# xyfJASON/ctrlora

Measured on AMD Instinct MI355X. Metric: 512x512 LoRA-finetune images/sec, higher is better.
Workload: dtype bf16; 1 GPU; ctrlora_finetune_sd15_rank128.yaml, canny-style latent hint, 512x512 (latent 64x64), per-GPU batch 8, bf16 storage / fp32 accumulate, synthetic latents + random-init weights, LoRA+zero-conv+norm trainables, fused AdamW; global_batch=8, parallelism=dp1, lora_rank=128, launch=hipGraph replay, gemm_launch_table_entries=215

## Files before the change

ctrlora_amd/build.py:

```python
from __future__ import annotations

import os
import subprocess
import sys
from concurrent.futures import ThreadPoolExecutor

HERE = os.path.dirname(os.path.abspath(__file__))
ROOT = os.path.dirname(HERE)
CSRC = os.path.join(HERE, "csrc")
OBJ = os.path.join(ROOT, "build", "obj")
LIB = os.path.join(HERE, "libctrlora_hip.so")
SOURCES = ["gemm.hip", "gemm_xs.hip", "gemm_w4.hip", "wgrad.hip", "norm.hip", "norm_coop.hip", "elementwise.hip", "attention_fwd.hip", "attention_bwd.hip", "attention_tr.hip", "attention_fwd40.hip", "attention_causal.hip", "capi.hip"]
FLAGS = ["--offload-arch=gfx950", "-O3", "-std=c++17", "-fPIC", "-Wno-unused-value"]


def _headers_mtime() -> float:
    hs = [os.path.join(CSRC, f) for f in os.listdir(CSRC) if f.endswith(".h")]
    hs.append(os.path.join(ROOT, "include", "ctrlora_hip.h"))
    return max(os.path.getmtime(h) for h in hs)


def _compile(src: str, force: bool) -> str:
    obj = os.path.join(OBJ, src.replace(".hip", ".o"))
    spath = os.path.join(CSRC, src)
    if (not force and os.path.exists(obj)
            and os.path.getmtime(obj) >= max(os.path.getmtime(spath), _headers_mtime())):
        return obj
    cmd = ["hipcc", *FLAGS, "-c", spath, "-o", obj]
    r = subprocess.run(cmd, capture_output=True, text=True)
    if r.returncode != 0:
        raise RuntimeError(f"hipcc failed for {src}:\n{r.stderr[-4000:]}")
    return obj


def build(force: bool = False, verbose: bool = True) -> str:
    os.makedirs(OBJ, exist_ok=True)
    with ThreadPoolExecutor(max_workers=6) as ex:
        objs = list(ex.map(lambda s: _compile(s, force), SOURCES))
    if force or not os.path.exists(LIB) or os.path.getmtime(LIB) < max(os.path.getmtime(o) for o in objs):
        r = subprocess.run(["hipcc", "--offload-arch=gfx950", "-shared", "-fPIC", *objs, "-o", LIB],
                           capture_output=True, text=True)
        if r.returncode != 0:
            raise RuntimeError(f"link failed:\n{r.stderr[-4000:]}")
        if verbose:
            print(f"[ctrlora_amd.build] linked {LIB}")
    elif verbose:
        print(f"[ctrlora_amd.build] up to date: {LIB}")
    return LIB


if __name__ == "__main__":
    build(force="--force" in sys.argv)
```

ctrlora_amd/csrc/attention.h:

```cpp
#pragma once
#include "common.h"

namespace cl {

struct AttnFwdArgs {
  const void* Q; long ldq;
  const void* K; long ldk;
  const void* Vt; int nkv_pad;
  void* O; long ldo;
  float* LSE; int lse_stride;
  int B, H, N, Nkv, DH;
  float scale;
  int q_prescaled;
};

struct AttnIpArgs {
  const void* K2; long ldk2;
  const void* V2; long ldv2;
  int Nip;
  float ip_scale;
};

struct AttnBwdArgs {
  const void* Q; long ldq; const void* K; long ldk; const void* V; long ldv;
  const void* O; long ldo; const void* dO; long lddo;
  const void* Qt; const void* dOt; int n_pad;
  const void* Kt; int nkv_pad;
  const float* LSE; float* Delta; int lse_stride;
  void* dQ; long lddq; void* dK; long lddk; void* dV; long lddv;
  int B, H, N, Nkv, DH;
  float scale;
  int q_prescaled;
  void* row_ws;
};

int attn_fwd(const AttnFwdArgs& a, int dtype, hipStream_t st);
int attn_bwd(const AttnBwdArgs& a, int dtype, hipStream_t st);
int attn_fwd_tr(const AttnFwdArgs& a, const void* V, long ldv, hipStream_t st);
int attn_fwd_ip(const AttnFwdArgs& a, const AttnIpArgs& ip, int dtype, hipStream_t st);
int attn_fwd_tr_ip(const AttnFwdArgs& a, const void* V, long ldv, const AttnIpArgs& ip, hipStream_t st);
int attn_bwd_tr(const AttnBwdArgs& a, hipStream_t st);
extern int g_attn_fuse_delta;
extern int g_attn_variant_dkv4;
extern int g_attn_variant;
bool attn_fwd40_applies(const AttnFwdArgs& a);
int attn_fwd40(const AttnFwdArgs& a, const void* V, long ldv, hipStream_t st);
int attn_delta(const AttnBwdArgs& a, hipStream_t st);
int attn_causal_fwd(int dtype, const void* Q, long ldq, const void* K, long ldk, const void* V, long ldv, void* O, long ldo, int B, int H,
                    int N, int dh, float scale, hipStream_t st);

enum { ATTN_FAM_TR = 1, ATTN_FAM_TR_IP = 2, ATTN_FAM_HYB = 3, ATTN_FAM_FWD40 = 4, ATTN_FAM_FOLD = 5, ATTN_FAM_TRANSPOSED = 6,
       ATTN_FAM_CAUSAL = 7 };
enum { ATTN_BIT_TAIL = 1, ATTN_BIT_TQ = 2, ATTN_BIT_TK = 4, ATTN_BIT_PRIO = 8 };
struct AttnLaunchRec {
  int kind;
  int family;
  int dtype, dh;
  int fwd_frags, dq_frags, dkv_frags;
  int bits;
  int lookahead, remap;
  int delta_launch, dkv_ran;
  int grid_fwd, grid_dq, grid_dkv;
  int tile;
};
extern AttnLaunchRec g_attn_last;
inline void attn_rec_begin() { g_attn_last = AttnLaunchRec{}; }
inline void attn_rec(int kind, int family, int dtype, int dh) {
  g_attn_last.kind = kind; g_attn_last.family = family; g_attn_last.dtype = dtype; g_attn_last.dh = dh; g_attn_last.tile = 64;
}

}
```

ctrlora_amd/csrc/attention_tr.hip:

```cpp
#include <type_traits>
#include "attn_common.h"
#include "attn_tr_util.h"

#ifndef ATTN_BWD_ABL
#define ATTN_BWD_ABL 0
#endif
#if ATTN_BWD_ABL == 2
#define BWD_MMA(a, b, c) asm volatile("" ::"v"(a), "v"(b))
#else
#define BWD_MMA(a, b, c) Mma<bf16_t>::run(a, b, c)
#endif
#if ATTN_BWD_ABL == 3
#define BWD_RD128 abl_rd128
#define BWD_TRF abl_trf
#else
#define BWD_RD128 lds_read_b128_off
#define BWD_TRF tr_frag_off
#endif
#if ATTN_BWD_ABL == 5
#define BWD_PACK(p) abl_pack(p)
#else
#define BWD_PACK(p) PFrag<bf16_t>::make(p)
#endif
#if ATTN_BWD_ABL == 1
#define BWD_EXP2(x) (x)
#else
#define BWD_EXP2(x) __builtin_amdgcn_exp2f(x)
#endif

namespace cl {
#if ATTN_BWD_ABL == 3
template <int OFF> __device__ __forceinline__ u32x4_t abl_rd128(uint32_t a) { u32x4_t v = {0x3c003c00u, 0x3c003c00u, 0x3c003c00u, 0x3c003c00u}; asm volatile("" : "+v"(v) : "v"(a)); return v; }
template <int ROWB, int STEP, int OFF> __device__ __forceinline__ u32x4_t abl_trf(uint32_t a) { u32x4_t v = {0x3c003c00u, 0x3c003c00u, 0x3c003c00u, 0x3c003c00u}; asm volatile("" : "+v"(v) : "v"(a)); return v; }
#endif
#if ATTN_BWD_ABL == 5
__device__ __forceinline__ u32x4_t abl_pack(const f32x4_t* p) {
  return u32x4_t{__float_as_uint(p[0][0]), __float_as_uint(p[0][2]), __float_as_uint(p[1][0]), __float_as_uint(p[1][2])};
}
#endif

namespace {

template <int DH> struct TileDma {
  static constexpr int TI = Geo<DH>::TI, NJ = (TI + 3) / 4, CPR = Geo<DH>::CPR, CPRP = Geo<DH>::CPRP;
  int r[NJ], cc16[NJ];
  bool real[NJ];
  __device__ __forceinline__ void init(int wave, int lane) {
#pragma unroll
    for (int j = 0; j < NJ; ++j) {
      const int c = (wave + 4 * j) * 64 + lane;
      r[j] = c / CPRP;
      const int col = c - r[j] * CPRP;
      real[j] = col < CPR;
      cc16[j] = (real[j] ? col : 0) * 16;
    }
  }
  __device__ __forceinline__ void offsets(long ld_bytes, int (&off)[NJ]) const {
#pragma unroll
    for (int j = 0; j < NJ; ++j) off[j] = r[j] * (int)ld_bytes + cc16[j];
  }
  __device__ __forceinline__ void issue_with_pad(const char* base, long ld_bytes, const int (&off)[NJ], int row0, char* dst,
                                                 int wave, const char* pad, int pad_stride) const {
    const char* tb = base + (long)row0 * ld_bytes;
    const char* pb = pad + (long)row0 * pad_stride;
#pragma unroll
    for (int j = 0; j < NJ; ++j)
      if (wave + 4 * j < TI) {
        const char* src = real[j] ? tb + off[j] : pb + r[j] * pad_stride;
        glds16(src, dst + (wave + 4 * j) * 1024);
      }
  }
  __device__ __forceinline__ void issue(const char* base, long ld_bytes, const int (&off)[NJ], int row0, int nrows,
                                        char* dst, int wave) const {
    const char* tb = base + (long)row0 * ld_bytes;
    if (row0 + 64 <= nrows) {
#pragma unroll
      for (int j = 0; j < NJ; ++j)
        if (wave + 4 * j < TI && real[j]) glds16(tb + off[j], dst + (wave + 4 * j) * 1024);
    } else {
#pragma unroll
      for (int j = 0; j < NJ; ++j)
        if (wave + 4 * j < TI && real[j]) {
          const int rr = min(row0 + r[j], nrows - 1);
          glds16(base + (long)rr * ld_bytes + cc16[j], dst + (wave + 4 * j) * 1024);
        }
    }
  }
};

__device__ __forceinline__ void split3_bf16(float x, uint32_t& w0, uint32_t& w1) {
  const uint32_t hi = pack2bf(x, 0.f) & 0xffffu;
  const float r1 = x - __uint_as_float(hi << 16);
  const uint32_t mid = pack2bf(r1, 0.f) & 0xffffu;
  const float r2 = r1 - __uint_as_float(mid << 16);
  const uint32_t lo = pack2bf(r2, 0.f) & 0xffffu;
  w0 = hi | (mid << 16); w1 = lo;
}
__device__ __forceinline__ u32x4_t ones3_chunk() { return u32x4_t{0x3F803F80u, 0x00003F80u, 0u, 0u}; }
template <int DH> __device__ __forceinline__ void init_pads_ones3(char* tiles, int ntile, int tid, int nthreads) {
  using G = Geo<DH>;
  for (int i = tid; i < ntile * 64; i += nthreads)
    *reinterpret_cast<uint4*>(tiles + (long)i * G::ROWB + G::CPR * 16) = make_uint4(0x3F803F80u, 0x00003F80u, 0u, 0u);
}

}

template <int DH, int QW, bool TAIL>
__global__ __launch_bounds__(256, 2) void attn_fwd_tr_kernel(AttnFwdArgs p, const void* __restrict__ V, long ldv) {
  using G = Geo<DH>;
  constexpr int CPR = G::CPR, KSTEPS = G::KSTEPS, DN = G::DN, ROWB = G::ROWB, TILE = G::TILE;
  constexpr int STAGE = 2 * TILE;
  extern __shared__ __attribute__((aligned(16))) char smem[];

  const int tid = threadIdx.x, lane = tid & 63;
  const int wave = __builtin_amdgcn_readfirstlane(tid >> 6);
  const int g = lane >> 4, lq = lane & 15;
  const int b = blockIdx.z, h = blockIdx.y;
  const int q0 = blockIdx.x * (64 * QW) + wave * (16 * QW);
  const float sl2 = p.q_prescaled ? 1.0f : p.scale * 1.4426950408889634f;

  u32x4_t qf[QW][KSTEPS];
#pragma unroll
  for (int f = 0; f < QW; ++f) {
    const int row = min(q0 + f * 16 + lq, p.N - 1);
    const char* qp = (const char*)p.Q + (((long)b * p.N + row) * p.ldq + (long)h * DH) * 2;
#pragma unroll
    for (int ks = 0; ks < KSTEPS; ++ks) {
      const int c = 4 * ks + g;
      qf[f][ks] = (c < CPR) ? *reinterpret_cast<const u32x4_t*>(qp + c * 16) : u32x4_t{0u, 0u, 0u, 0u};
    }
  }
  const char* kbase = (const char*)p.K + ((long)b * p.Nkv * p.ldk + (long)h * DH) * 2;
  const char* vbase = (const char*)V + ((long)b * p.Nkv * ldv + (long)h * DH) * 2;

  f32x4_t ot[DN][QW];
#pragma unroll
  for (int i = 0; i < DN; ++i)
#pragma unroll
    for (int f = 0; f < QW; ++f) ot[i][f] = f32x4_t{0.f, 0.f, 0.f, 0.f};
  float m_run[QW], l_run[QW];
#pragma unroll
  for (int f = 0; f < QW; ++f) { m_run[f] = -1e30f; l_run[f] = 0.f; }

  const uint32_t lds0 = (uint32_t)(uintptr_t)smem;
  uint32_t krow[KSTEPS];
#pragma unroll
  for (int ks = 0; ks < KSTEPS; ++ks) krow[ks] = lq * ROWB + min(4 * ks + g, CPR - 1) * 16;
  const uint32_t troff = (4 * g + ((lane >> 2) & 3)) * ROWB + (lane & 3) * 8;
  const int ntiles = (p.Nkv + 63) / 64;
  TileDma<DH> dma; dma.init(wave, lane);
  int koff[TileDma<DH>::NJ], voff[TileDma<DH>::NJ];
  dma.offsets(p.ldk * 2, koff); dma.offsets(ldv * 2, voff);
  init_pads<DH>(smem, 4, 0u, 0u, tid, 256);
  dma.issue(kbase, p.ldk * 2, koff, 0, p.Nkv, smem, wave);
  dma.issue(vbase, ldv * 2, voff, 0, p.Nkv, smem + TILE, wave);
  for (int t = 0; t < ntiles; ++t) {
    const int buf = t & 1;
    asm volatile("s_waitcnt vmcnt(0)" ::: "memory");
    __syncthreads();
    if (t + 1 < ntiles) {
      dma.issue(kbase, p.ldk * 2, koff, (t + 1) * 64, p.Nkv, smem + (buf ^ 1) * STAGE, wave);
      dma.issue(vbase, ldv * 2, voff, (t + 1) * 64, p.Nkv, smem + (buf ^ 1) * STAGE + TILE, wave);
    }
    const uint32_t kt = lds0 + buf * STAGE, vt = kt + TILE;

    f32x4_t st[4][QW];
    uint32_t kr[KSTEPS];
#pragma unroll
    for (int ks = 0; ks < KSTEPS; ++ks) kr[ks] = kt + krow[ks];
    static_for<0, 4>([&](auto KF_) {
      constexpr int kf = decltype(KF_)::value;
      u32x4_t ka[KSTEPS];
#pragma unroll
      for (int ks = 0; ks < KSTEPS; ++ks) ka[ks] = lds_read_b128_off<kf * 16 * ROWB>(kr[ks]);
      lds_wait();
#pragma unroll
      for (int f = 0; f < QW; ++f) {
        st[kf][f] = f32x4_t{0.f, 0.f, 0.f, 0.f};
#pragma unroll
        for (int ks = 0; ks < KSTEPS; ++ks) Mma<bf16_t>::run(ka[ks], qf[f][ks], st[kf][f]);
      }
    });
    const int kv0 = t * 64;
    {
#pragma unroll
      for (int f = 0; f < QW; ++f) {
        float mx = -INFINITY;
#pragma unroll
        for (int kf = 0; kf < 4; ++kf)
#pragma unroll
          for (int r = 0; r < 4; ++r) {
            if constexpr (TAIL) { if (kv0 + kf * 16 + 4 * g + r >= p.Nkv) st[kf][f][r] = -INFINITY; }
            mx = fmaxf(mx, st[kf][f][r]);
          }
        mx = fmaxf(mx, __shfl_xor(mx, 16, 64));
        mx = fmaxf(mx, __shfl_xor(mx, 32, 64));
        const float m_new = fmaxf(m_run[f], mx * sl2);
        const float alpha = __builtin_amdgcn_exp2f(m_run[f] - m_new);
        m_run[f] = m_new;
        float ls = 0.f;
#pragma unroll
        for (int kf = 0; kf < 4; ++kf)
#pragma unroll
          for (int r = 0; r < 4; ++r) {
            const float e = __builtin_amdgcn_exp2f(__builtin_fmaf(st[kf][f][r], sl2, -m_new));
            st[kf][f][r] = e;
            ls += e;
          }
        l_run[f] = l_run[f] * alpha + ls;
#pragma unroll
        for (int i = 0; i < DN; ++i) ot[i][f] *= alpha;
      }
    }
    u32x4_t pb[2][QW];
#pragma unroll
    for (int s = 0; s < 2; ++s)
#pragma unroll
      for (int f = 0; f < QW; ++f) {
        f32x4_t tmp[2] = {st[2 * s][f], st[2 * s + 1][f]};
        pb[s][f] = PFrag<bf16_t>::make(tmp);
      }
    const uint32_t tb = vt + troff;
    static_for<0, DN>([&](auto I_) {
      constexpr int i = decltype(I_)::value;
      u32x4_t va[2];
      va[0] = tr_frag_off<ROWB, 0, i * 32>(tb);
      va[1] = tr_frag_off<ROWB, 1, i * 32>(tb);
      lds_wait();
#pragma unroll
      for (int s = 0; s < 2; ++s)
#pragma unroll
        for (int f = 0; f < QW; ++f) Mma<bf16_t>::run(va[s], pb[s][f], ot[i][f]);
    });
  }

#pragma unroll
  for (int f = 0; f < QW; ++f) {
    float l = l_run[f];
    l += __shfl_xor(l, 16, 64);
    l += __shfl_xor(l, 32, 64);
    const float inv = 1.0f / l;
    const int row = q0 + f * 16 + lq;
    if (row < p.N) {
      bf16_t* op = reinterpret_cast<bf16_t*>(p.O) + ((long)b * p.N + row) * p.ldo + (long)h * DH;
#pragma unroll
      for (int i = 0; i < DN; ++i) {
        const int d0 = i * 16 + 4 * g;
        if (d0 < DH) {
          float v[4] = {ot[i][f][0] * inv, ot[i][f][1] * inv, ot[i][f][2] * inv, ot[i][f][3] * inv};
          store4(op + d0, v);
        }
      }
      if (p.LSE && g == 0) p.LSE[((long)b * p.H + h) * p.lse_stride + row] = m_run[f] + __builtin_amdgcn_logf(l);
    }
  }
}

template <int DH, int QW>
__global__ __launch_bounds__(256, 2) void attn_fwd_tr_ip_kernel(AttnFwdArgs p, const void* __restrict__ V, long ldv,
                                                                AttnIpArgs ip) {
  using G = Geo<DH>;
  constexpr int CPR = G::CPR, KSTEPS = G::KSTEPS, DN = G::DN, ROWB = G::ROWB, TILE = G::TILE;
  constexpr int STAGE = 2 * TILE;
  extern __shared__ __attribute__((aligned(16))) char smem[];

  const int tid = threadIdx.x, lane = tid & 63;
  const int wave = __builtin_amdgcn_readfirstlane(tid >> 6);
  const int g = lane >> 4, lq = lane & 15;
  const int b = blockIdx.z, h = blockIdx.y;
  const int q0 = blockIdx.x * (64 * QW) + wave * (16 * QW);
  const float sl2 = p.q_prescaled ? 1.0f : p.scale * 1.4426950408889634f;

  u32x4_t qf[QW][KSTEPS];
#pragma unroll
  for (int f = 0; f < QW; ++f) {
    const int row = min(q0 + f * 16 + lq, p.N - 1);
    const char* qp = (const char*)p.Q + (((long)b * p.N + row) * p.ldq + (long)h * DH) * 2;
#pragma unroll
    for (int ks = 0; ks < KSTEPS; ++ks) {
      const int c = 4 * ks + g;
      qf[f][ks] = (c < CPR) ? *reinterpret_cast<const u32x4_t*>(qp + c * 16) : u32x4_t{0u, 0u, 0u, 0u};
    }
  }
  const char* kbase = (const char*)p.K + ((long)b * p.Nkv * p.ldk + (long)h * DH) * 2;
  const char* vbase = (const char*)V + ((long)b * p.Nkv * ldv + (long)h * DH) * 2;

  f32x4_t ot[DN][QW];
#pragma unroll
  for (int i = 0; i < DN; ++i)
#pragma unroll
    for (int f = 0; f < QW; ++f) ot[i][f] = f32x4_t{0.f, 0.f, 0.f, 0.f};
  float m_run[QW], l_run[QW];
#pragma unroll
  for (int f = 0; f < QW; ++f) { m_run[f] = -1e30f; l_run[f] = 0.f; }

  const uint32_t lds0 = (uint32_t)(uintptr_t)smem;
  uint32_t krow[KSTEPS];
#pragma unroll
  for (int ks = 0; ks < KSTEPS; ++ks) krow[ks] = lq * ROWB + min(4 * ks + g, CPR - 1) * 16;
  const uint32_t troff = (4 * g + ((lane >> 2) & 3)) * ROWB + (lane & 3) * 8;
  auto qk = [&](uint32_t kt, f32x4_t (&st)[4][QW]) {
    static_for<0, 4>([&](auto KF_) {
      constexpr int kf = decltype(KF_)::value;
      u32x4_t ka[KSTEPS];
#pragma unroll
      for (int ks = 0; ks < KSTEPS; ++ks) ka[ks] = lds_read_b128_off<kf * 16 * ROWB>(kt + krow[ks]);
      lds_wait();
#pragma unroll
      for (int f = 0; f < QW; ++f) {
        st[kf][f] = f32x4_t{0.f, 0.f, 0.f, 0.f};
#pragma unroll
        for (int ks = 0; ks < KSTEPS; ++ks) Mma<bf16_t>::run(ka[ks], qf[f][ks], st[kf][f]);
      }
    });
  };
  auto pv = [&](uint32_t vt, f32x4_t (&st)[4][QW]) {
    u32x4_t pb[2][QW];
#pragma unroll
    for (int s = 0; s < 2; ++s)
#pragma unroll
      for (int f = 0; f < QW; ++f) {
        f32x4_t tmp[2] = {st[2 * s][f], st[2 * s + 1][f]};
        pb[s][f] = PFrag<bf16_t>::make(tmp);
      }
    const uint32_t tb = vt + troff;
    static_for<0, DN>([&](auto I_) {
      constexpr int i = decltype(I_)::value;
      u32x4_t va[2];
      va[0] = tr_frag_off<ROWB, 0, i * 32>(tb);
      va[1] = tr_frag_off<ROWB, 1, i * 32>(tb);
      lds_wait();
#pragma unroll
      for (int s = 0; s < 2; ++s)
#pragma unroll
        for (int f = 0; f < QW; ++f) Mma<bf16_t>::run(va[s], pb[s][f], ot[i][f]);
    });
  };

  const int ntiles = (p.Nkv + 63) / 64;
  TileDma<DH> dma; dma.init(wave, lane);
  int koff[TileDma<DH>::NJ], voff[TileDma<DH>::NJ];
  dma.offsets(p.ldk * 2, koff); dma.offsets(ldv * 2, voff);
  init_pads<DH>(smem, 4, 0u, 0u, tid, 256);
  dma.issue(kbase, p.ldk * 2, koff, 0, p.Nkv, smem, wave);
  dma.issue(vbase, ldv * 2, voff, 0, p.Nkv, smem + TILE, wave);
  for (int t = 0; t < ntiles; ++t) {
    const int buf = t & 1;
    asm volatile("s_waitcnt vmcnt(0)" ::: "memory");
    __syncthreads();
    if (t + 1 < ntiles) {
      dma.issue(kbase, p.ldk * 2, koff, (t + 1) * 64, p.Nkv, smem + (buf ^ 1) * STAGE, wave);
      dma.issue(vbase, ldv * 2, voff, (t + 1) * 64, p.Nkv, smem + (buf ^ 1) * STAGE + TILE, wave);
    } else {
      const char* k2 = (const char*)ip.K2 + ((long)b * ip.Nip * ip.ldk2 + (long)h * DH) * 2;
      const char* v2 = (const char*)ip.V2 + ((long)b * ip.Nip * ip.ldv2 + (long)h * DH) * 2;
      dma.offsets(ip.ldk2 * 2, koff); dma.offsets(ip.ldv2 * 2, voff);
      dma.issue(k2, ip.ldk2 * 2, koff, 0, ip.Nip, smem + (buf ^ 1) * STAGE, wave);
      dma.issue(v2, ip.ldv2 * 2, voff, 0, ip.Nip, smem + (buf ^ 1) * STAGE + TILE, wave);
    }
    const uint32_t kt = lds0 + buf * STAGE, vt = kt + TILE;
    f32x4_t st[4][QW];
    qk(kt, st);
    const int kv0 = t * 64;
#pragma unroll
    for (int f = 0; f < QW; ++f) {
      float mx = -INFINITY;
#pragma unroll
      for (int kf = 0; kf < 4; ++kf)
#pragma unroll
        for (int r = 0; r < 4; ++r) {
          if (kv0 + kf * 16 + 4 * g + r >= p.Nkv) st[kf][f][r] = -INFINITY;
          mx = fmaxf(mx, st[kf][f][r]);
        }
      mx = fmaxf(mx, __shfl_xor(mx, 16, 64));
      mx = fmaxf(mx, __shfl_xor(mx, 32, 64));
      const float m_new = fmaxf(m_run[f], mx * sl2);
      const float alpha = __builtin_amdgcn_exp2f(m_run[f] - m_new);
      m_run[f] = m_new;
      float ls = 0.f;
#pragma unroll
      for (int kf = 0; kf < 4; ++kf)
#pragma unroll
        for (int r = 0; r < 4; ++r) {
          const float e = __builtin_amdgcn_exp2f(__builtin_fmaf(st[kf][f][r], sl2, -m_new));
          st[kf][f][r] = e;
          ls += e;
        }
      l_run[f] = l_run[f] * alpha + ls;
#pragma unroll
      for (int i = 0; i < DN; ++i) ot[i][f] *= alpha;
    }
    pv(vt, st);
  }

#pragma unroll
  for (int f = 0; f < QW; ++f) {
    float l = l_run[f];
    l += __shfl_xor(l, 16, 64);
    l += __shfl_xor(l, 32, 64);
    const float inv = 1.0f / l;
#pragma unroll
    for (int i = 0; i < DN; ++i) ot[i][f] *= inv;
  }
  asm volatile("s_waitcnt vmcnt(0)" ::: "memory");
  __syncthreads();
  {
    const uint32_t kt = lds0 + (ntiles & 1) * STAGE, vt = kt + TILE;
    f32x4_t st[4][QW];
    qk(kt, st);
#pragma unroll
    for (int f = 0; f < QW; ++f) {
      float mx = -INFINITY;
#pragma unroll
      for (int kf = 0; kf < 4; ++kf)
#pragma unroll
        for (int r = 0; r < 4; ++r) {
          if (kf * 16 + 4 * g + r >= ip.Nip) st[kf][f][r] = -INFINITY;
          mx = fmaxf(mx, st[kf][f][r]);
        }
      mx = fmaxf(mx, __shfl_xor(mx, 16, 64));
      mx = fmaxf(mx, __shfl_xor(mx, 32, 64));
      const float m2 = mx * sl2;
      float ls = 0.f;
#pragma unroll
      for (int kf = 0; kf < 4; ++kf)
#pragma unroll
        for (int r = 0; r < 4; ++r) {
          const float e = __builtin_amdgcn_exp2f(__builtin_fmaf(st[kf][f][r], sl2, -m2));
          st[kf][f][r] = e;
          ls += e;
        }
      ls += __shfl_xor(ls, 16, 64);
      ls += __shfl_xor(ls, 32, 64);
      const float c = ip.ip_scale / ls;
#pragma unroll
      for (int kf = 0; kf < 4; ++kf) st[kf][f] *= c;
    }
    pv(vt, st);
  }

#pragma unroll
  for (int f = 0; f < QW; ++f) {
    const int row = q0 + f * 16 + lq;
    if (row < p.N) {
      bf16_t* op = reinterpret_cast<bf16_t*>(p.O) + ((long)b * p.N + row) * p.ldo + (long)h * DH;
#pragma unroll
      for (int i = 0; i < DN; ++i) {
        const int d0 = i * 16 + 4 * g;
        if (d0 < DH) {
          float v[4] = {ot[i][f][0], ot[i][f][1], ot[i][f][2], ot[i][f][3]};
          store4(op + d0, v);
        }
      }
    }
  }
}



template <int DH, int LA = 3>
__global__ __launch_bounds__(512, 2) void attn_fwd_hyb_kernel(AttnFwdArgs p, const void* __restrict__ V, long ldv,
                                                              int nqb, int remap) {
  using G = Geo<DH>;
  constexpr int CPR = G::CPR, DN = G::DN, ROWB = G::ROWB, TILE = G::TILE;
  constexpr int STAGE = 2 * TILE, QW = 2;
  constexpr int NK = (DH + 15) / 16;
  constexpr bool ONES = (DH % 16) != 0;
  constexpr bool PADONES = ONES && G::CPRP > G::CPR;
  static_assert(!ONES || PADONES, "spare V^T rows come from the padded LDS pitch");
  static_assert(2 * NK <= G::CPRP, "K fragment reads stay inside the LDS row");
  constexpr int LROW = DH % 16;
  constexpr float RESCALE_THR = 6.0f;
  extern __shared__ __attribute__((aligned(16))) char smem[];

  const int tid = threadIdx.x, lane = tid & 63;
  const int wave = __builtin_amdgcn_readfirstlane(tid >> 6);
  const int grp = wave >> 2;
  const int g = lane >> 4, lq = lane & 15, l31 = lane & 31, hi = lane >> 5;
  int bh, qb;
  {
    const int id = blockIdx.x;
    if (remap) { const int xcd = id & 7, slot = id >> 3; bh = xcd + 8 * (slot / nqb); qb = slot - (slot / nqb) * nqb; }
    else { bh = id / nqb; qb = id - bh * nqb; }
  }
  const int b = bh / p.H, h = bh - b * p.H;
  const int q0 = qb * 256 + wave * 32;
  const float sl2 = p.q_prescaled ? 1.0f : p.scale * 1.4426950408889634f;

  for (int i = tid; i < (16 * ROWB + 64) / 4; i += 512) reinterpret_cast<uint32_t*>(smem + 3 * STAGE)[i] = 0u;
  init_pads<DH>(smem, 6, 0u, 0x3F803F80u, tid, 512);

  u32x4_t qh[NK];
  {
    const char* qp = (const char*)p.Q + (((long)b * p.N + q0 + l31) * p.ldq + (long)h * DH) * 2;
#pragma unroll
    for (int j = 0; j < NK; ++j) {
      const int c = 2 * j + hi;
      qh[j] = (c < CPR) ? *reinterpret_cast<const u32x4_t*>(qp + c * 16) : u32x4_t{0u, 0u, 0u, 0u};
    }
  }
  const char* kbase = (const char*)p.K + ((long)b * p.Nkv * p.ldk + (long)h * DH) * 2;
  const char* vbase = (const char*)V + ((long)b * p.Nkv * ldv + (long)h * DH) * 2;

  f32x4_t ot[DN][QW];
#pragma unroll
  for (int i = 0; i < DN; ++i)
#pragma unroll
    for (int f = 0; f < QW; ++f) ot[i][f] = f32x4_t{0.f, 0.f, 0.f, 0.f};
  float m_run = -1e30f, l_run = 0.f;
  f32x16_t st[2];
  u32x4_t pb[2][QW];

  constexpr int CPRP = G::CPRP, NJ = (CPRP + 7) / 8;
  int koff[NJ], voff[NJ];
  bool real[NJ];
#pragma unroll
  for (int j = 0; j < NJ; ++j) {
    const int c = (wave + 8 * j) * 64 + lane, r = c / CPRP, col = c - r * CPRP;
    real[j] = col < CPR;
    const int cc = (real[j] ? col : 0) * 16;
    koff[j] = r * (int)(p.ldk * 2) + cc;
    voff[j] = r * (int)(ldv * 2) + cc;
  }
  auto issue = [&](int t, int stage) {
    const char* kb = kbase + (long)t * 64 * p.ldk * 2;
    const char* vb = vbase + (long)t * 64 * ldv * 2;
    char* dst = smem + stage * STAGE;
#pragma unroll
    for (int j = 0; j < NJ; ++j)
      if (wave + 8 * j < CPRP && real[j]) {
        glds16(kb + koff[j], dst + (wave + 8 * j) * 1024);
        glds16(vb + voff[j], dst + TILE + (wave + 8 * j) * 1024);
      }
  };

  const uint32_t lds0 = (uint32_t)(uintptr_t)smem;
  const int kr = (l31 & 19) | ((l31 & 4) << 1) | ((l31 & 8) >> 1);
  const uint32_t krow = kr * ROWB + hi * 16;
  const uint32_t troff = (4 * g + ((lane >> 2) & 3)) * ROWB + (lane & 3) * 8;
  const int nt = p.Nkv / 64;

  auto phaseM = [&](auto PREVc, uint32_t kt, uint32_t vt) {
    constexpr bool PREV = decltype(PREVc)::value;
    constexpr int NV = PREV ? DN : 0, NG = NV + 2;
    u32x4_t va[LA][2], ka[LA][NK];
    auto cnt_of = [](int j) constexpr { return j < NV ? 4 : NK; };
    auto read_group = [&](auto Jc) {
      constexpr int J = decltype(Jc)::value;
      if constexpr (J < NV) {
        va[J % LA][0] = tr_frag<ROWB, 0>(vt + troff + J * 32);
        va[J % LA][1] = tr_frag<ROWB, 1>(vt + troff + J * 32);
      } else if constexpr (J < NG) {
        constexpr int s = J - NV;
        static_for<0, NK>([&](auto Kc) {
          constexpr int j = decltype(Kc)::value;
          ka[s % LA][j] = lds_read_b128_off<s * 32 * ROWB + j * 32>(kt + krow);
        });
      }
    };
    static_for<0, LA - 1>([&](auto Jc) { read_group(Jc); });
    __builtin_amdgcn_s_setprio(1);
    static_for<0, NG>([&](auto Jc) {
      constexpr int J = decltype(Jc)::value;
      read_group(std::integral_constant<int, J + LA - 1>{});
      constexpr int pending = [&]() constexpr { int n = 0; for (int k = J + 1; k < J + LA && k < NG; ++k) n += cnt_of(k); return n; }();
      lgkm_wait<(pending > 15 ? 15 : pending)>();
      if constexpr (J < NV) {
        pin(va[J % LA][0]); pin(va[J % LA][1]);
#pragma unroll
        for (int f = 0; f < QW; ++f) Mma<bf16_t>::run(va[J % LA][0], pb[0][f], ot[J][f]);
#pragma unroll
        for (int f = 0; f < QW; ++f) Mma<bf16_t>::run(va[J % LA][1], pb[1][f], ot[J][f]);
      } else {
        constexpr int s = J - NV;
#pragma unroll
        for (int j = 0; j < NK; ++j) pin(ka[s % LA][j]);
        f32x16_t acc = {0.f, 0.f, 0.f, 0.f, 0.f, 0.f, 0.f, 0.f, 0.f, 0.f, 0.f, 0.f, 0.f, 0.f, 0.f, 0.f};
#pragma unroll
        for (int j = 0; j < NK; ++j)
          acc = __builtin_amdgcn_mfma_f32_32x32x16_bf16(__builtin_bit_cast(bf16x8_t, ka[s % LA][j]),
                                                        __builtin_bit_cast(bf16x8_t, qh[j]), acc, 0, 0, 0);
        st[s] = acc;
      }
      __builtin_amdgcn_sched_barrier(0);
    });
    __builtin_amdgcn_s_setprio(0);
  };

  auto phaseV = [&]() {
    float mx = st[0][0];
#pragma unroll
    for (int s = 0; s < 2; ++s)
#pragma unroll
      for (int r = 0; r < 16; ++r) mx = fmaxf(mx, st[s][r]);
    const bool need = mx * sl2 > m_run + RESCALE_THR;
    if (__any(need)) {
      mx = fmaxf(mx, __shfl_xor(mx, 32, 64));
      const float m_new = fmaxf(m_run, mx * sl2);
      const float alpha = __builtin_amdgcn_exp2f(m_run - m_new);
      m_run = m_new;
      l_run *= alpha;
#pragma unroll
      for (int f = 0; f < QW; ++f) {
        const float af = __shfl(alpha, 16 * f + lq, 64);
#pragma unroll
        for (int i = 0; i < DN; ++i) ot[i][f] *= af;
      }
    }
    float ls = 0.f;
#pragma unroll
    for (int s = 0; s < 2; ++s) {
      uint32_t pk[8];
#pragma unroll
      for (int k = 0; k < 8; ++k) {
        const f32x2_t x = f32x2_t{st[s][2 * k], st[s][2 * k + 1]} * sl2 - m_run;
        const float e0 = __builtin_amdgcn_exp2f(x.x), e1 = __builtin_amdgcn_exp2f(x.y);
        if constexpr (!ONES) ls += e0 + e1;
        pk[k] = pack2bf(e0, e1);
      }
      const auto s0 = __builtin_amdgcn_permlane16_swap(pk[0], pk[2], false, false);
      const auto s1 = __builtin_amdgcn_permlane16_swap(pk[1], pk[3], false, false);
      const auto s2 = __builtin_amdgcn_permlane16_swap(pk[4], pk[6], false, false);
      const auto s3 = __builtin_amdgcn_permlane16_swap(pk[5], pk[7], false, false);
      pb[s][0] = u32x4_t{s0[0], s1[0], s2[0], s3[0]};
      pb[s][1] = u32x4_t{s0[1], s1[1], s2[1], s3[1]};
    }
    if constexpr (!ONES) l_run += ls;
  };

  issue(0, 0);
  issue(1, 1);
  asm volatile("s_waitcnt vmcnt(0)" ::: "memory");
  __syncthreads();
  int sk = 0;
  if (grp == 1) __builtin_amdgcn_s_setprio(1);
  auto pv_tail = [&](uint32_t vt) {
    u32x4_t va[2];
#pragma unroll
    for (int i = 0; i < DN; ++i) {
      va[0] = tr_frag<ROWB, 0>(vt + troff + i * 32); va[1] = tr_frag<ROWB, 1>(vt + troff + i * 32);
      lds_wait();
#pragma unroll
      for (int s = 0; s < 2; ++s)
#pragma unroll
        for (int f = 0; f < QW; ++f) Mma<bf16_t>::run(va[s], pb[s][f], ot[i][f]);
    }
  };
  if (grp == 0) {
    int sp = 2;
    for (int u = 0; u < nt; ++u) {
      const int sn = (sk == 2) ? 0 : sk + 1;
      if (u >= 1 && u + 1 < nt) issue(u + 1, sn);
      if (u == 0) phaseM(std::false_type{}, lds0 + sk * STAGE, 0u);
      else phaseM(std::true_type{}, lds0 + sk * STAGE, lds0 + sp * STAGE + TILE);
      __builtin_amdgcn_s_barrier();
      phaseV();
      asm volatile("s_waitcnt vmcnt(0)" ::: "memory");
      __builtin_amdgcn_s_barrier();
      sp = sk; sk = sn;
    }
    pv_tail(lds0 + sp * STAGE + TILE);
    __builtin_amdgcn_s_barrier();
  } else {
    int sp = 2;
    __builtin_amdgcn_s_barrier();
    for (int u = 0; u < nt; ++u) {
      const int sn = (sk == 2) ? 0 : sk + 1, sn2 = (sn == 2) ? 0 : sn + 1;
      if (u == 0) phaseM(std::false_type{}, lds0 + sk * STAGE, 0u);
      else phaseM(std::true_type{}, lds0 + sk * STAGE, lds0 + sp * STAGE + TILE);
      __builtin_amdgcn_s_setprio(1);
      asm volatile("s_waitcnt vmcnt(0)" ::: "memory");
      __builtin_amdgcn_s_barrier();
      if (u + 2 < nt) issue(u + 2, sn2);
      phaseV();
      __builtin_amdgcn_s_barrier();
      sp = sk; sk = sn;
    }
    pv_tail(lds0 + sp * STAGE + TILE);
  }

  float l_full = l_run;
  if constexpr (!ONES) l_full += __shfl_xor(l_full, 32, 64);
#pragma unroll
  for (int f = 0; f < QW; ++f) {
    float l;
    if constexpr (ONES) l = __shfl(ot[DN - 1][f][LROW & 3], lq + 16 * (LROW >> 2), 64);
    else l = __shfl(l_full, 16 * f + lq, 64);
    const float m = __shfl(m_run, 16 * f + lq, 64);
    const float inv = 1.0f / l;
    const int row = q0 + f * 16 + lq;
    bf16_t* op = reinterpret_cast<bf16_t*>(p.O) + ((long)b * p.N + row) * p.ldo + (long)h * DH;
#pragma unroll
    for (int i = 0; i < DN; ++i) {
      const int d0 = i * 16 + 4 * g;
      if (d0 < DH) {
        float v[4] = {ot[i][f][0] * inv, ot[i][f][1] * inv, ot[i][f][2] * inv, ot[i][f][3] * inv};
        store4(op + d0, v);
      }
    }
    if (p.LSE && g == 0) p.LSE[((long)b * p.H + h) * p.lse_stride + row] = m + __builtin_amdgcn_logf(l);
  }
}

template <int DH, int KF, bool TAIL, bool PRIO = false, bool FOLD = false>
__global__ __launch_bounds__(256, (DH <= 80 && KF <= 2 ? 2 : 1)) void attn_bwd_dkv_tr_kernel(AttnBwdArgs p) {
  using G = Geo<DH>;
  constexpr int CPR = G::CPR, KSTEPS = G::KSTEPS, DN = G::DN, ROWB = G::ROWB, TILE = G::TILE, TI = G::TI;
  static_assert(!FOLD || (DH == 40 && !TAIL), "the fold uses the pad chunk of the 96-byte pitch, whole tiles only");
  constexpr int CIN = FOLD ? G::CPRP : CPR;
  constexpr bool PIPE = FOLD;
  constexpr int STAGE = 2 * TILE + 512;
  extern __shared__ __attribute__((aligned(16))) char smem[];

  const int tid = threadIdx.x, lane = tid & 63;
  const int wave = __builtin_amdgcn_readfirstlane(tid >> 6);
  const int g = lane >> 4, lq = lane & 15;
  const int b = blockIdx.z, h = blockIdx.y;
  const int kv_w = blockIdx.x * (64 * KF) + wave * (16 * KF);
  const float sl2 = p.q_prescaled ? 1.0f : p.scale * 1.4426950408889634f;
  const float kscale = p.q_prescaled ? 0.6931471805599453f : p.scale;

  u32x4_t kb[KF][KSTEPS], vb[KF][KSTEPS];
#pragma unroll
  for (int kf = 0; kf < KF; ++kf) {
    const int kr = min(kv_w + kf * 16 + lq, p.Nkv - 1);
    const char* kp = (const char*)p.K + (((long)b * p.Nkv + kr) * p.ldk + (long)h * DH) * 2;
    const char* vp = (const char*)p.V + (((long)b * p.Nkv + kr) * p.ldv + (long)h * DH) * 2;
#pragma unroll
    for (int ks = 0; ks < KSTEPS; ++ks) {
      const int c = 4 * ks + g;
      kb[kf][ks] = (c < CPR) ? *reinterpret_cast<const u32x4_t*>(kp + c * 16) : u32x4_t{0u, 0u, 0u, 0u};
      vb[kf][ks] = (c < CPR) ? *reinterpret_cast<const u32x4_t*>(vp + c * 16) : u32x4_t{0u, 0u, 0u, 0u};
      if constexpr (FOLD) {
        if (c == CPR) { kb[kf][ks] = ones3_chunk(); vb[kf][ks] = ones3_chunk(); }
      }
    }
  }
  const char* qbase = (const char*)p.Q + ((long)b * p.N * p.ldq + (long)h * DH) * 2;
  const char* dobase = (const char*)p.dO + ((long)b * p.N * p.lddo + (long)h * DH) * 2;
  const float* lse = p.LSE + ((long)b * p.H + h) * p.lse_stride;
  const float* dlt = p.Delta + ((long)b * p.H + h) * p.lse_stride;

  f32x4_t dvt[KF][DN], dkt[KF][DN];
#pragma unroll
  for (int kf = 0; kf < KF; ++kf)
#pragma unroll
    for (int i = 0; i < DN; ++i) { dvt[kf][i] = f32x4_t{0.f, 0.f, 0.f, 0.f}; dkt[kf][i] = f32x4_t{0.f, 0.f, 0.f, 0.f}; }

  TileDma<DH> dma; dma.init(wave, lane);
  int qoff[TileDma<DH>::NJ], dooff[TileDma<DH>::NJ];
  dma.offsets(p.ldq * 2, qoff); dma.offsets(p.lddo * 2, dooff);
  const char* rowpad = FOLD ? (const char*)p.row_ws + ((long)b * p.H + h) * p.lse_stride * 32 : nullptr;
  auto issue = [&](int t, int buf) {
    char* base = smem + buf * STAGE;
    if constexpr (FOLD) {
      dma.issue_with_pad(qbase, p.ldq * 2, qoff, t * 64, base, wave, rowpad, 32);
      dma.issue_with_pad(dobase, p.lddo * 2, dooff, t * 64, base + TILE, wave, rowpad + 16, 32);
      return;
    }
    dma.issue(qbase, p.ldq * 2, qoff, t * 64, p.N, base, wave);
    dma.issue(dobase, p.lddo * 2, dooff, t * 64, p.N, base + TILE, wave);
    if (wave == (TI & 3) && lane < 32) {
      const float* src = lane < 16 ? lse + t * 64 + lane * 4 : dlt + t * 64 + (lane - 16) * 4;
      glds16(src, base + 2 * TILE);
    }
  };

  const uint32_t lds0 = (uint32_t)(uintptr_t)smem;
  uint32_t rrow[KSTEPS];
#pragma unroll
  for (int ks = 0; ks < KSTEPS; ++ks) rrow[ks] = lq * ROWB + min(4 * ks + g, CIN - 1) * 16;
  const uint32_t troff = (4 * g + ((lane >> 2) & 3)) * ROWB + (lane & 3) * 8;
  const int ntiles = (p.N + 63) / 64;
  if constexpr (!FOLD) {
    init_pads<DH>(smem, 2, 0u, 0u, tid, 256);
    init_pads<DH>(smem + STAGE, 2, 0u, 0u, tid, 256);
  }
  const int dma_per_tile = 2 * ((TI - wave + 3) / 4);
  issue(0, 0);
  if constexpr (PIPE) { if (ntiles > 1) issue(1, 1); }
  int buf = 0;
  for (int t = 0; t < ntiles; ++t) {
#if ATTN_BWD_ABL == 4
    if constexpr (!PIPE) { asm volatile("s_waitcnt vmcnt(0)" ::: "memory"); __syncthreads(); }
#else
    if constexpr (PIPE) {
      if (t + 1 >= ntiles) asm volatile("s_waitcnt vmcnt(0)" ::: "memory");
      else if (dma_per_tile == 4) asm volatile("s_waitcnt vmcnt(4)" ::: "memory");
      else asm volatile("s_waitcnt vmcnt(2)" ::: "memory");
    } else {
      asm volatile("s_waitcnt vmcnt(0)" ::: "memory");
    }
    __syncthreads();
#endif
    const uint32_t aQ = lds0 + buf * STAGE, adO = aQ + TILE, aL = adO + TILE;
    const int q0 = t * 64;
    uint32_t rb[KSTEPS];
#pragma unroll
    for (int ks = 0; ks < KSTEPS; ++ks) rb[ks] = aQ + rrow[ks];
    const uint32_t tb = aQ + troff;
    u32x4_t qa[2][KSTEPS], da[2][KSTEPS];
    if constexpr (PIPE) {
#pragma unroll
      for (int ks = 0; ks < KSTEPS; ++ks) { qa[0][ks] = BWD_RD128<0>(rb[ks]); da[0][ks] = BWD_RD128<TILE>(rb[ks]); }
    }
    if constexpr (PIPE) {
      if (t + 2 < ntiles) issue(t + 2, buf == 0 ? 2 : buf - 1);
    } else {
      if (t + 1 < ntiles) issue(t + 1, buf ^ 1);
    }

    f32x4_t ps[KF][4], ds[KF][4];
    u32x4_t oa[2][2], qt[2][2];
    static_for<0, 4>([&](auto QF_) {
      constexpr int qf = decltype(QF_)::value;
      constexpr int cur = PIPE ? (qf & 1) : 0;
      u32x4_t l4 = {0u, 0u, 0u, 0u}, d4 = {0u, 0u, 0u, 0u};
      if constexpr (PIPE) {
        if constexpr (qf + 1 < 4) {
#pragma unroll
          for (int ks = 0; ks < KSTEPS; ++ks) {
            qa[cur ^ 1][ks] = BWD_RD128<(qf + 1) * 16 * ROWB>(rb[ks]);
            da[cur ^ 1][ks] = BWD_RD128<TILE + (qf + 1) * 16 * ROWB>(rb[ks]);
          }
          lgkm_wait<2 * KSTEPS>();
        } else {
          oa[0][0] = BWD_TRF<ROWB, 0, TILE>(tb); oa[0][1] = BWD_TRF<ROWB, 1, TILE>(tb);
          qt[0][0] = BWD_TRF<ROWB, 0, 0>(tb); qt[0][1] = BWD_TRF<ROWB, 1, 0>(tb);
          lgkm_wait<8>();
        }
      } else {
#pragma unroll
        for (int ks = 0; ks < KSTEPS; ++ks) {
          qa[0][ks] = BWD_RD128<qf * 16 * ROWB>(rb[ks]);
          da[0][ks] = BWD_RD128<TILE + qf * 16 * ROWB>(rb[ks]);
        }
        if constexpr (!FOLD) {
          l4 = lds_read_b128(aL + (qf * 16 + 4 * g) * 4);
          d4 = lds_read_b128(aL + 256 + (qf * 16 + 4 * g) * 4);
        }
        lds_wait();
      }
      const float lv[4] = {__uint_as_float(l4.x), __uint_as_float(l4.y), __uint_as_float(l4.z), __uint_as_float(l4.w)};
      const float dv[4] = {__uint_as_float(d4.x), __uint_as_float(d4.y), __uint_as_float(d4.z), __uint_as_float(d4.w)};
      const int qrow = q0 + qf * 16 + 4 * g;
#pragma unroll
      for (int kf = 0; kf < KF; ++kf) {
        f32x4_t sc = {0.f, 0.f, 0.f, 0.f}, dp = {0.f, 0.f, 0.f, 0.f};
        if constexpr (PRIO) __builtin_amdgcn_s_setprio(1);
#pragma unroll
        for (int ks = 0; ks < KSTEPS; ++ks) { BWD_MMA(qa[cur][ks], kb[kf][ks], sc); BWD_MMA(da[cur][ks], vb[kf][ks], dp); }
        if constexpr (PRIO) __builtin_amdgcn_s_setprio(0);
#pragma unroll
        for (int h2 = 0; h2 < 2; ++h2) {
          f32x2_t pr, dsv;
          if constexpr (FOLD) {
            pr = f32x2_t{BWD_EXP2(sc[2 * h2]), BWD_EXP2(sc[2 * h2 + 1])};
            dsv = pr * f32x2_t{dp[2 * h2], dp[2 * h2 + 1]};
          } else {
            const f32x2_t s2 = {sc[2 * h2], sc[2 * h2 + 1]}, l2 = {lv[2 * h2], lv[2 * h2 + 1]};
            const f32x2_t x = s2 * sl2 - l2;
            pr = f32x2_t{__builtin_amdgcn_exp2f(x.x), __builtin_amdgcn_exp2f(x.y)};
            const f32x2_t dd = f32x2_t{dp[2 * h2], dp[2 * h2 + 1]} - f32x2_t{dv[2 * h2], dv[2 * h2 + 1]};
            dsv = pr * dd;
          }
          if constexpr (TAIL) {
            if (qrow + 2 * h2 >= p.N) { pr.x = 0.f; dsv.x = 0.f; }
            if (qrow + 2 * h2 + 1 >= p.N) { pr.y = 0.f; dsv.y = 0.f; }
          }
          ps[kf][qf][2 * h2] = pr.x; ps[kf][qf][2 * h2 + 1] = pr.y;
          ds[kf][qf][2 * h2] = dsv.x; ds[kf][qf][2 * h2 + 1] = dsv.y;
        }
      }
    });
    u32x4_t pb[KF][2], sb[KF][2];
#pragma unroll
    for (int kf = 0; kf < KF; ++kf)
#pragma unroll
      for (int s2 = 0; s2 < 2; ++s2) { pb[kf][s2] = BWD_PACK(&ps[kf][2 * s2]); sb[kf][s2] = BWD_PACK(&ds[kf][2 * s2]); }
    static_for<0, DN>([&](auto I_) {
      constexpr int i = decltype(I_)::value;
      constexpr int cur = PIPE ? (i & 1) : 0;
      if constexpr (PIPE) {
        if constexpr (i + 1 < DN) {
          oa[cur ^ 1][0] = BWD_TRF<ROWB, 0, TILE + (i + 1) * 32>(tb); oa[cur ^ 1][1] = BWD_TRF<ROWB, 1, TILE + (i + 1) * 32>(tb);
          lgkm_wait<4>();
          qt[cur ^ 1][0] = BWD_TRF<ROWB, 0, (i + 1) * 32>(tb); qt[cur ^ 1][1] = BWD_TRF<ROWB, 1, (i + 1) * 32>(tb);
        } else {
          lgkm_wait<0>();
        }
      } else {
        oa[0][0] = BWD_TRF<ROWB, 0, TILE + i * 32>(tb); oa[0][1] = BWD_TRF<ROWB, 1, TILE + i * 32>(tb);
        qt[0][0] = BWD_TRF<ROWB, 0, i * 32>(tb); qt[0][1] = BWD_TRF<ROWB, 1, i * 32>(tb);
        lds_wait();
      }
      if constexpr (PRIO) __builtin_amdgcn_s_setprio(1);
#pragma unroll
      for (int kf = 0; kf < KF; ++kf)
#pragma unroll
        for (int s2 = 0; s2 < 2; ++s2) { BWD_MMA(oa[cur][s2], pb[kf][s2], dvt[kf][i]); BWD_MMA(qt[cur][s2], sb[kf][s2], dkt[kf][i]); }
      if constexpr (PRIO) __builtin_amdgcn_s_setprio(0);
    });
    if constexpr (PIPE) buf = buf == 2 ? 0 : buf + 1;
    else buf ^= 1;
  }
#pragma unroll
  for (int kf = 0; kf < KF; ++kf) {
    const int kr = kv_w + kf * 16 + lq;
    if (kr < p.Nkv) {
      bf16_t* dkp = reinterpret_cast<bf16_t*>(p.dK) + ((long)b * p.Nkv + kr) * p.lddk + (long)h * DH;
      bf16_t* dvp = reinterpret_cast<bf16_t*>(p.dV) + ((long)b * p.Nkv + kr) * p.lddv + (long)h * DH;
#pragma unroll
      for (int i = 0; i < DN; ++i) {
        const int d0 = i * 16 + 4 * g;
        if (d0 < DH) {
          float a[4] = {dkt[kf][i][0] * kscale, dkt[kf][i][1] * kscale, dkt[kf][i][2] * kscale, dkt[kf][i][3] * kscale};
          float c[4] = {dvt[kf][i][0], dvt[kf][i][1], dvt[kf][i][2], dvt[kf][i][3]};
          store4(dkp + d0, a);
          store4(dvp + d0, c);
        }
      }
    }
  }
}

template <int DH, int QF, bool TAIL, bool DELTA = false, bool PRIO = false, bool FOLD = false>
__global__ __launch_bounds__(256, 2) void attn_bwd_dq_tr_kernel(AttnBwdArgs p) {
  using G = Geo<DH>;
  constexpr int CPR = G::CPR, KSTEPS = G::KSTEPS, DN = G::DN, ROWB = G::ROWB, TILE = G::TILE;
  static_assert(!FOLD || (DH == 40 && !TAIL && DELTA), "fold: d_head 40, whole key tiles, fused delta");
  constexpr int CIN = FOLD ? G::CPRP : CPR;
  constexpr bool PIPE = FOLD;
  constexpr int STAGE = 2 * TILE;
  extern __shared__ __attribute__((aligned(16))) char smem[];

  const int tid = threadIdx.x, lane = tid & 63;
  const int wave = __builtin_amdgcn_readfirstlane(tid >> 6);
  const int g = lane >> 4, lq = lane & 15;
  const int b = blockIdx.z, h = blockIdx.y;
  const int q_w = blockIdx.x * (64 * QF) + wave * (16 * QF);
  const float sl2 = p.q_prescaled ? 1.0f : p.scale * 1.4426950408889634f;

  u32x4_t qb[QF][KSTEPS], ob[QF][KSTEPS];
  float lse_q[QF], dlt_q[QF];
#pragma unroll
  for (int f = 0; f < QF; ++f) {
    const int qr = min(q_w + f * 16 + lq, p.N - 1);
    const char* qp = (const char*)p.Q + (((long)b * p.N + qr) * p.ldq + (long)h * DH) * 2;
    const char* op = (const char*)p.dO + (((long)b * p.N + qr) * p.lddo + (long)h * DH) * 2;
#pragma unroll
    for (int ks = 0; ks < KSTEPS; ++ks) {
      const int c = 4 * ks + g;
      qb[f][ks] = (c < CPR) ? *reinterpret_cast<const u32x4_t*>(qp + c * 16) : u32x4_t{0u, 0u, 0u, 0u};
      ob[f][ks] = (c < CPR) ? *reinterpret_cast<const u32x4_t*>(op + c * 16) : u32x4_t{0u, 0u, 0u, 0u};
    }
    lse_q[f] = p.LSE[((long)b * p.H + h) * p.lse_stride + qr];
    if constexpr (DELTA) {
      const char* orow = (const char*)p.O + (((long)b * p.N + qr) * p.ldo + (long)h * DH) * 2;
      float acc = 0.f;
#pragma unroll
      for (int ks = 0; ks < KSTEPS; ++ks) {
        const int c = 4 * ks + g;
        if (c < CPR) {
          const u32x4_t ov = *reinterpret_cast<const u32x4_t*>(orow + c * 16);
          const u32x4_t dv = ob[f][ks];
#pragma unroll
          for (int j = 0; j < 4; ++j) {
            acc += __uint_as_float(ov[j] << 16) * __uint_as_float(dv[j] << 16);
            acc += __uint_as_float(ov[j] & 0xffff0000u) * __uint_as_float(dv[j] & 0xffff0000u);
          }
        }
      }
      acc += __shfl_xor(acc, 16, 64);
      acc += __shfl_xor(acc, 32, 64);
      dlt_q[f] = acc;
      if (g == 0 && q_w + f * 16 + lq < p.N) p.Delta[((long)b * p.H + h) * p.lse_stride + qr] = acc;
    } else {
      dlt_q[f] = p.Delta[((long)b * p.H + h) * p.lse_stride + qr];
    }
    if constexpr (FOLD) {
      uint32_t l0, l1, d0, d1;
      split3_bf16(-lse_q[f], l0, l1);
      split3_bf16(-dlt_q[f], d0, d1);
      if (g == 1) {
        qb[f][1] = u32x4_t{l0, l1, 0u, 0u};
        ob[f][1] = u32x4_t{d0, d1, 0u, 0u};
      }
      if (g == 0 && q_w + f * 16 + lq < p.N) {
        uint4* rp = reinterpret_cast<uint4*>((char*)p.row_ws + (((long)b * p.H + h) * p.lse_stride + qr) * 32);
        rp[0] = make_uint4(l0, l1, 0u, 0u);
        rp[1] = make_uint4(d0, d1, 0u, 0u);
      }
    }
  }
  const char* kbase = (const char*)p.K + ((long)b * p.Nkv * p.ldk + (long)h * DH) * 2;
  const char* vbase = (const char*)p.V + ((long)b * p.Nkv * p.ldv + (long)h * DH) * 2;

  f32x4_t dqt[QF][DN];
#pragma unroll
  for (int f = 0; f < QF; ++f)
#pragma unroll
    for (int i = 0; i < DN; ++i) dqt[f][i] = f32x4_t{0.f, 0.f, 0.f, 0.f};

  const uint32_t lds0 = (uint32_t)(uintptr_t)smem;
  uint32_t rrow[KSTEPS];
#pragma unroll
  for (int ks = 0; ks < KSTEPS; ++ks) rrow[ks] = lq * ROWB + min(4 * ks + g, CIN - 1) * 16;
  const uint32_t troff = (4 * g + ((lane >> 2) & 3)) * ROWB + (lane & 3) * 8;
  const int ntiles = (p.Nkv + 63) / 64;
  TileDma<DH> dma; dma.init(wave, lane);
  int koff[TileDma<DH>::NJ], voff[TileDma<DH>::NJ];
  dma.offsets(p.ldk * 2, koff); dma.offsets(p.ldv * 2, voff);
  if constexpr (FOLD) init_pads_ones3<DH>(smem, 6, tid, 256);
  else init_pads<DH>(smem, 4, 0u, 0u, tid, 256);
  constexpr int TI = G::TI;
  const int dma_per_tile = 2 * ((TI - wave + 3) / 4);
  auto issue_kv = [&](int t, int st_) {
    dma.issue(kbase, p.ldk * 2, koff, t * 64, p.Nkv, smem + st_ * STAGE, wave);
    dma.issue(vbase, p.ldv * 2, voff, t * 64, p.Nkv, smem + st_ * STAGE + TILE, wave);
  };
  issue_kv(0, 0);
  if constexpr (PIPE) { if (ntiles > 1) issue_kv(1, 1); }
  int buf = 0;
  for (int t = 0; t < ntiles; ++t) {
#if ATTN_BWD_ABL == 4
    if constexpr (!PIPE) { asm volatile("s_waitcnt vmcnt(0)" ::: "memory"); __syncthreads(); }
#else
    if constexpr (PIPE) {
      if (t + 1 >= ntiles) asm volatile("s_waitcnt vmcnt(0)" ::: "memory");
      else if (dma_per_tile == 4) asm volatile("s_waitcnt vmcnt(4)" ::: "memory");
      else asm volatile("s_waitcnt vmcnt(2)" ::: "memory");
    } else {
      asm volatile("s_waitcnt vmcnt(0)" ::: "memory");
    }
    __syncthreads();
#endif
    const uint32_t aK = lds0 + buf * STAGE, aV = aK + TILE;
    const int kv0 = t * 64;
    uint32_t rb[KSTEPS];
#pragma unroll
    for (int ks = 0; ks < KSTEPS; ++ks) rb[ks] = aK + rrow[ks];
    const uint32_t tb = aK + troff;
    u32x4_t ka[2][KSTEPS], va[2][KSTEPS], kc[2][2];
    if constexpr (PIPE) {
#pragma unroll
      for (int ks = 0; ks < KSTEPS; ++ks) { ka[0][ks] = BWD_RD128<0>(rb[ks]); va[0][ks] = BWD_RD128<TILE>(rb[ks]); }
    }
    if constexpr (PIPE) {
      if (t + 2 < ntiles) issue_kv(t + 2, buf == 0 ? 2 : buf - 1);
    } else {
      if (t + 1 < ntiles) issue_kv(t + 1, buf ^ 1);
    }

    f32x4_t dst[QF][4];
    static_for<0, 4>([&](auto KF_) {
      constexpr int kf = decltype(KF_)::value;
      constexpr int cur = PIPE ? (kf & 1) : 0;
      if constexpr (PIPE) {
        if constexpr (kf + 1 < 4) {
#pragma unroll
          for (int ks = 0; ks < KSTEPS; ++ks) {
            ka[cur ^ 1][ks] = BWD_RD128<(kf + 1) * 16 * ROWB>(rb[ks]);
            va[cur ^ 1][ks] = BWD_RD128<TILE + (kf + 1) * 16 * ROWB>(rb[ks]);
          }
          lgkm_wait<2 * KSTEPS>();
        } else {
          kc[0][0] = BWD_TRF<ROWB, 0, 0>(tb); kc[0][1] = BWD_TRF<ROWB, 1, 0>(tb);
          lgkm_wait<4>();
        }
      } else {
#pragma unroll
        for (int ks = 0; ks < KSTEPS; ++ks) {
          ka[0][ks] = BWD_RD128<kf * 16 * ROWB>(rb[ks]);
          va[0][ks] = BWD_RD128<TILE + kf * 16 * ROWB>(rb[ks]);
        }
        lds_wait();
      }
#pragma unroll
      for (int f = 0; f < QF; ++f) {
        f32x4_t sc = {0.f, 0.f, 0.f, 0.f}, dp = {0.f, 0.f, 0.f, 0.f};
        if constexpr (PRIO) __builtin_amdgcn_s_setprio(1);
#pragma unroll
        for (int ks = 0; ks < KSTEPS; ++ks) { BWD_MMA(ka[cur][ks], qb[f][ks], sc); BWD_MMA(va[cur][ks], ob[f][ks], dp); }
        if constexpr (PRIO) __builtin_amdgcn_s_setprio(0);
#pragma unroll
        for (int h2 = 0; h2 < 2; ++h2) {
          f32x2_t dsv;
          if constexpr (FOLD) {
            const f32x2_t pr = {BWD_EXP2(sc[2 * h2]), BWD_EXP2(sc[2 * h2 + 1])};
            dsv = pr * f32x2_t{dp[2 * h2], dp[2 * h2 + 1]};
          } else {
            const f32x2_t x = f32x2_t{sc[2 * h2], sc[2 * h2 + 1]} * sl2 - lse_q[f];
            const f32x2_t pr = {__builtin_amdgcn_exp2f(x.x), __builtin_amdgcn_exp2f(x.y)};
            dsv = pr * (f32x2_t{dp[2 * h2], dp[2 * h2 + 1]} - dlt_q[f]);
          }
          if constexpr (TAIL) {
            if (kv0 + kf * 16 + 4 * g + 2 * h2 >= p.Nkv) dsv.x = 0.f;
            if (kv0 + kf * 16 + 4 * g + 2 * h2 + 1 >= p.Nkv) dsv.y = 0.f;
          }
          dst[f][kf][2 * h2] = dsv.x; dst[f][kf][2 * h2 + 1] = dsv.y;
        }
      }
    });
    u32x4_t sb[QF][2];
#pragma unroll
    for (int f = 0; f < QF; ++f)
#pragma unroll
      for (int s2 = 0; s2 < 2; ++s2) sb[f][s2] = BWD_PACK(&dst[f][2 * s2]);
    static_for<0, DN>([&](auto I_) {
      constexpr int i = decltype(I_)::value;
      constexpr int cur = PIPE ? (i & 1) : 0;
      if constexpr (PIPE) {
        if constexpr (i + 1 < DN) {
          kc[cur ^ 1][0] = BWD_TRF<ROWB, 0, (i + 1) * 32>(tb); kc[cur ^ 1][1] = BWD_TRF<ROWB, 1, (i + 1) * 32>(tb);
          lgkm_wait<4>();
        } else {
          lgkm_wait<0>();
        }
      } else {
        kc[0][0] = BWD_TRF<ROWB, 0, i * 32>(tb); kc[0][1] = BWD_TRF<ROWB, 1, i * 32>(tb);
        lds_wait();
      }
      if constexpr (PRIO) __builtin_amdgcn_s_setprio(1);
#pragma unroll
      for (int f = 0; f < QF; ++f)
#pragma unroll
        for (int s2 = 0; s2 < 2; ++s2) BWD_MMA(kc[cur][s2], sb[f][s2], dqt[f][i]);
      if constexpr (PRIO) __builtin_amdgcn_s_setprio(0);
    });
    if constexpr (PIPE) buf = buf == 2 ? 0 : buf + 1;
    else buf ^= 1;
  }
#pragma unroll
  for (int f = 0; f < QF; ++f) {
    const int qrow = q_w + f * 16 + lq;
    if (qrow < p.N) {
      bf16_t* dqp = reinterpret_cast<bf16_t*>(p.dQ) + ((long)b * p.N + qrow) * p.lddq + (long)h * DH;
#pragma unroll
      for (int i = 0; i < DN; ++i) {
        const int d0 = i * 16 + 4 * g;
        if (d0 < DH) {
          float a[4] = {dqt[f][i][0] * p.scale, dqt[f][i][1] * p.scale, dqt[f][i][2] * p.scale, dqt[f][i][3] * p.scale};
          store4(dqp + d0, a);
        }
      }
    }
  }
}

template <typename K>
static int set_lds(K kern, int bytes) {
  if (bytes > 65536 &&
      hipFuncSetAttribute(reinterpret_cast<const void*>(kern), hipFuncAttributeMaxDynamicSharedMemorySize, bytes) != hipSuccess)
    return CL_ELAUNCH;
  return CL_OK;
}

AttnLaunchRec g_attn_last{};
int g_attn_variant_dkv4 = 0;
int g_attn_variant = 0;

template <int DH, int LA>
static int launch_fwd_hyb_t(const AttnFwdArgs& a, const void* V, long ldv, hipStream_t st) {
  constexpr int LDS = 3 * 2 * Geo<DH>::TILE + 16 * Geo<DH>::ROWB + 64;
  static bool done = false;
  if (!done) {
    if (set_lds(&attn_fwd_hyb_kernel<DH, LA>, LDS)) return CL_ELAUNCH;
    done = true;
  }
  const int nqb = a.N / 256;
  const long grid = (long)nqb * a.H * a.B;
  const int remap = ((a.B * a.H) % 8 == 0) ? 1 : 0;
  hipLaunchKernelGGL((attn_fwd_hyb_kernel<DH, LA>), dim3((unsigned)grid), dim3(512), LDS, st, a, V, ldv, nqb, remap);
  attn_rec(1, ATTN_FAM_HYB, CL_BF16, DH);
  g_attn_last.fwd_frags = 4; g_attn_last.lookahead = LA; g_attn_last.remap = remap; g_attn_last.grid_fwd = (int)grid;
  CL_CHECK_LAUNCH();
  return CL_OK;
}

template <int DH>
static bool launch_fwd_pp(const AttnFwdArgs& a, const void* V, long ldv, hipStream_t st, int* rc) {
  if constexpr (DH == 40 || DH == 80) {
    const long grid = (long)(a.N / 256) * a.H * a.B;
    if (g_attn_variant == 1 || a.N % 256 || a.Nkv % 64 || a.Nkv < 128 || grid < 256) return false;
    *rc = g_attn_variant == 13 ? launch_fwd_hyb_t<DH, 3>(a, V, ldv, st) : launch_fwd_hyb_t<DH, 2>(a, V, ldv, st);
    return true;
  }
  return false;
}

template <int DH, bool TAIL>
static int launch_fwd_tr(const AttnFwdArgs& a, const void* V, long ldv, hipStream_t st) {
  constexpr int LDS = 2 * 2 * Geo<DH>::TILE + 64 + 16 * Geo<DH>::ROWB;
  constexpr int QW = DH <= 80 ? 2 : 1;
  static bool done = false;
  if (!done) {
    if (set_lds(&attn_fwd_tr_kernel<DH, QW, TAIL>, LDS) || set_lds(&attn_fwd_tr_kernel<DH, 1, TAIL>, LDS)) return CL_ELAUNCH;
    done = true;
  }
  const long blocks128 = (long)((a.N + 127) / 128) * a.H * a.B;
  if (QW == 2 && blocks128 >= 512) {
    dim3 grid((a.N + 127) / 128, a.H, a.B);
    hipLaunchKernelGGL((attn_fwd_tr_kernel<DH, QW, TAIL>), grid, dim3(256), LDS, st, a, V, ldv);
    g_attn_last.fwd_frags = QW; g_attn_last.grid_fwd = (int)(grid.x * grid.y * grid.z);
  } else {
    dim3 grid((a.N + 63) / 64, a.H, a.B);
    hipLaunchKernelGGL((attn_fwd_tr_kernel<DH, 1, TAIL>), grid, dim3(256), LDS, st, a, V, ldv);
    g_attn_last.fwd_frags = 1; g_attn_last.grid_fwd = (int)(grid.x * grid.y * grid.z);
  }
  attn_rec(1, ATTN_FAM_TR, CL_BF16, DH);
  g_attn_last.bits = TAIL ? ATTN_BIT_TAIL : 0;
  CL_CHECK_LAUNCH();
  return CL_OK;
}

template <int DH>
static int launch_fwd_tr_t(const AttnFwdArgs& a, const void* V, long ldv, hipStream_t st) {
  int rc = CL_OK;
  if (launch_fwd_pp<DH>(a, V, ldv, st, &rc)) return rc;
  return (a.Nkv % 64) ? launch_fwd_tr<DH, true>(a, V, ldv, st) : launch_fwd_tr<DH, false>(a, V, ldv, st);
}

int attn_fwd_tr(const AttnFwdArgs& a, const void* V, long ldv, hipStream_t st) {
  attn_rec_begin();
  if ((a.ldq * 2) % 16 || (a.ldk * 2) % 16 || (ldv * 2) % 16 || (a.ldo * 2) % 16 || a.Nkv < 1 || a.N < 1) return CL_EINVAL;
  if (a.LSE && (a.lse_stride % 64 || a.lse_stride < a.N)) return CL_EINVAL;
  if (g_attn_variant == 0 && attn_fwd40_applies(a)) return attn_fwd40(a, V, ldv, st);
  switch (a.DH) {
    case 8: return launch_fwd_tr_t<8>(a, V, ldv, st);
    case 16: return launch_fwd_tr_t<16>(a, V, ldv, st);
    case 32: return launch_fwd_tr_t<32>(a, V, ldv, st);
    case 40: return launch_fwd_tr_t<40>(a, V, ldv, st);
    case 80: return launch_fwd_tr_t<80>(a, V, ldv, st);
    case 160: return launch_fwd_tr_t<160>(a, V, ldv, st);
    default: return CL_EINVAL;
  }
}

template <int DH>
static int launch_fwd_tr_ip(const AttnFwdArgs& a, const void* V, long ldv, const AttnIpArgs& ip, hipStream_t st) {
  constexpr int LDS = 2 * 2 * Geo<DH>::TILE + 64 + 16 * Geo<DH>::ROWB;
  constexpr int QW = DH <= 80 ? 2 : 1;
  static bool done = false;
  if (!done) {
    if (set_lds(&attn_fwd_tr_ip_kernel<DH, QW>, LDS) || set_lds(&attn_fwd_tr_ip_kernel<DH, 1>, LDS)) return CL_ELAUNCH;
    done = true;
  }
  const long blocks128 = (long)((a.N + 127) / 128) * a.H * a.B;
  if (QW == 2 && blocks128 >= 512) {
    dim3 grid((a.N + 127) / 128, a.H, a.B);
    hipLaunchKernelGGL((attn_fwd_tr_ip_kernel<DH, QW>), grid, dim3(256), LDS, st, a, V, ldv, ip);
    g_attn_last.fwd_frags = QW; g_attn_last.grid_fwd = (int)(grid.x * grid.y * grid.z);
  } else {
    dim3 grid((a.N + 63) / 64, a.H, a.B);
    hipLaunchKernelGGL((attn_fwd_tr_ip_kernel<DH, 1>), grid, dim3(256), LDS, st, a, V, ldv, ip);
    g_attn_last.fwd_frags = 1; g_attn_last.grid_fwd = (int)(grid.x * grid.y * grid.z);
  }
  attn_rec(1, ATTN_FAM_TR_IP, CL_BF16, DH);
  CL_CHECK_LAUNCH();
  return CL_OK;
}

int attn_fwd_tr_ip(const AttnFwdArgs& a, const void* V, long ldv, const AttnIpArgs& ip, hipStream_t st) {
  attn_rec_begin();
  if ((a.ldq * 2) % 16 || (a.ldk * 2) % 16 || (ldv * 2) % 16 || (a.ldo * 2) % 16 || a.Nkv < 1 || a.N < 1) return CL_EINVAL;
  if ((ip.ldk2 * 2) % 16 || (ip.ldv2 * 2) % 16 || ip.Nip < 1 || ip.Nip > 64 || !ip.K2 || !ip.V2 || a.LSE) return CL_EINVAL;
  switch (a.DH) {
    case 8: return launch_fwd_tr_ip<8>(a, V, ldv, ip, st);
    case 16: return launch_fwd_tr_ip<16>(a, V, ldv, ip, st);
    case 32: return launch_fwd_tr_ip<32>(a, V, ldv, ip, st);
    case 40: return launch_fwd_tr_ip<40>(a, V, ldv, ip, st);
    case 80: return launch_fwd_tr_ip<80>(a, V, ldv, ip, st);
    case 160: return launch_fwd_tr_ip<160>(a, V, ldv, ip, st);
    default: return CL_EINVAL;
  }
}

int g_attn_fuse_delta = 1;

template <int DH, bool TQ, bool TK>
static int launch_bwd_tr(const AttnBwdArgs& a, hipStream_t st) {
  constexpr int KF = DH <= 40 ? 2 : 1;
  constexpr int LDS_DKV = 2 * (2 * Geo<DH>::TILE + 512) + 64 + 16 * Geo<DH>::ROWB;
  constexpr int LDS_DQ = 2 * 2 * Geo<DH>::TILE + 64 + 16 * Geo<DH>::ROWB;
  constexpr int LDS_DKV3 = 3 * (2 * Geo<DH>::TILE + 512) + 64 + 16 * Geo<DH>::ROWB;
  constexpr int LDS_DQ3 = 3 * 2 * Geo<DH>::TILE + 64 + 16 * Geo<DH>::ROWB;
  static bool done = false;
  if (!done) {
    if (set_lds(&attn_bwd_dkv_tr_kernel<DH, KF, TQ>, LDS_DKV) || set_lds(&attn_bwd_dkv_tr_kernel<DH, 1, TQ>, LDS_DKV) ||
        set_lds(&attn_bwd_dq_tr_kernel<DH, KF, TK>, LDS_DQ) || set_lds(&attn_bwd_dq_tr_kernel<DH, 1, TK>, LDS_DQ) ||
        set_lds(&attn_bwd_dq_tr_kernel<DH, KF, TK, true>, LDS_DQ) || set_lds(&attn_bwd_dq_tr_kernel<DH, 1, TK, true>, LDS_DQ) ||
        set_lds(&attn_bwd_dq_tr_kernel<DH, KF, TK, true, true>, LDS_DQ) || set_lds(&attn_bwd_dkv_tr_kernel<DH, KF, TQ, true>, LDS_DKV))
      return CL_ELAUNCH;
    done = true;
  }
  const bool fused_delta = g_attn_fuse_delta != 0;
  if (!fused_delta) {
    const int rc = attn_delta(a, st);
    if (rc) return rc;
  }
  const bool prio = g_attn_variant == 11;
  attn_rec(2, ATTN_FAM_TR, CL_BF16, DH);
  g_attn_last.bits = (TQ ? ATTN_BIT_TQ : 0) | (TK ? ATTN_BIT_TK : 0);
  g_attn_last.delta_launch = fused_delta ? 0 : 1;
  if constexpr (DH == 40 && !TQ && !TK) {
    const long qb2 = (long)(a.N / 128) * a.H * a.B, kb2 = (long)(a.Nkv / 128) * a.H * a.B;
    if (a.q_prescaled && a.row_ws && fused_delta && g_attn_variant == 0 && a.N % 128 == 0 && a.Nkv % 128 == 0 &&
        qb2 >= 512 && (!a.dK || kb2 >= 512)) {
      static bool done_f = false;
      if (!done_f) {
        if (set_lds(&attn_bwd_dq_tr_kernel<DH, KF, TK, true, false, true>, LDS_DQ3) ||
            set_lds(&attn_bwd_dkv_tr_kernel<DH, KF, TQ, false, true>, LDS_DKV3))
          return CL_ELAUNCH;
        done_f = true;
      }
      hipLaunchKernelGGL((attn_bwd_dq_tr_kernel<DH, KF, TK, true, false, true>), dim3(a.N / 128, a.H, a.B), dim3(256), LDS_DQ3, st, a);
      g_attn_last.family = ATTN_FAM_FOLD; g_attn_last.dq_frags = KF; g_attn_last.grid_dq = (int)qb2;
      if (a.dK) {
        if (g_attn_variant_dkv4 && a.Nkv % 256 == 0) {
          static bool done4 = false;
          if (!done4) { if (set_lds(&attn_bwd_dkv_tr_kernel<DH, 4, TQ, false, true>, LDS_DKV3)) return CL_ELAUNCH; done4 = true; }
          hipLaunchKernelGGL((attn_bwd_dkv_tr_kernel<DH, 4, TQ, false, true>), dim3(a.Nkv / 256, a.H, a.B), dim3(256), LDS_DKV3, st, a);
          g_attn_last.dkv_frags = 4; g_attn_last.grid_dkv = (a.Nkv / 256) * a.H * a.B;
        } else {
          hipLaunchKernelGGL((attn_bwd_dkv_tr_kernel<DH, KF, TQ, false, true>), dim3(a.Nkv / 128, a.H, a.B), dim3(256), LDS_DKV3, st, a);
          g_attn_last.dkv_frags = KF; g_attn_last.grid_dkv = (int)kb2;
        }
        g_attn_last.dkv_ran = 1;
      }
      CL_CHECK_LAUNCH();
      return CL_OK;
    }
  }
  auto launch_dq = [&]() {
    const long qb2 = (long)((a.N + 64 * KF - 1) / (64 * KF)) * a.H * a.B;
    if (KF == 2 && qb2 >= 512) {
      dim3 grid((a.N + 127) / 128, a.H, a.B);
      if (fused_delta && prio) hipLaunchKernelGGL((attn_bwd_dq_tr_kernel<DH, KF, TK, true, true>), grid, dim3(256), LDS_DQ, st, a);
      else if (fused_delta) hipLaunchKernelGGL((attn_bwd_dq_tr_kernel<DH, KF, TK, true>), grid, dim3(256), LDS_DQ, st, a);
      else hipLaunchKernelGGL((attn_bwd_dq_tr_kernel<DH, KF, TK>), grid, dim3(256), LDS_DQ, st, a);
      g_attn_last.dq_frags = KF; g_attn_last.grid_dq = (int)(grid.x * grid.y * grid.z);
      if (fused_delta && prio) g_attn_last.bits |= ATTN_BIT_PRIO;
    } else {
      dim3 grid((a.N + 63) / 64, a.H, a.B);
      if (fused_delta) hipLaunchKernelGGL((attn_bwd_dq_tr_kernel<DH, 1, TK, true>), grid, dim3(256), LDS_DQ, st, a);
      else hipLaunchKernelGGL((attn_bwd_dq_tr_kernel<DH, 1, TK>), grid, dim3(256), LDS_DQ, st, a);
      g_attn_last.dq_frags = 1; g_attn_last.grid_dq = (int)(grid.x * grid.y * grid.z);
    }
  };
  if (fused_delta) launch_dq();
  if (a.dK) {
    const long blocks2 = (long)((a.Nkv + 64 * KF - 1) / (64 * KF)) * a.H * a.B;
    if (KF == 2 && blocks2 >= 512) {
      dim3 grid((a.Nkv + 127) / 128, a.H, a.B);
      if (prio) hipLaunchKernelGGL((attn_bwd_dkv_tr_kernel<DH, KF, TQ, true>), grid, dim3(256), LDS_DKV, st, a);
      else hipLaunchKernelGGL((attn_bwd_dkv_tr_kernel<DH, KF, TQ>), grid, dim3(256), LDS_DKV, st, a);
      g_attn_last.dkv_frags = KF; g_attn_last.grid_dkv = (int)(grid.x * grid.y * grid.z);
      if (prio) g_attn_last.bits |= ATTN_BIT_PRIO;
    } else {
      dim3 grid((a.Nkv + 63) / 64, a.H, a.B);
      hipLaunchKernelGGL((attn_bwd_dkv_tr_kernel<DH, 1, TQ>), grid, dim3(256), LDS_DKV, st, a);
      g_attn_last.dkv_frags = 1; g_attn_last.grid_dkv = (int)(grid.x * grid.y * grid.z);
    }
    g_attn_last.dkv_ran = 1;
  }
  if (!fused_delta) launch_dq();
  CL_CHECK_LAUNCH();
  return CL_OK;
}

template <int DH>
static int launch_bwd_tr_t(const AttnBwdArgs& a, hipStream_t st) {
  const bool tq = a.N % 64, tk = a.Nkv % 64;
  if (tq) return tk ? launch_bwd_tr<DH, true, true>(a, st) : launch_bwd_tr<DH, true, false>(a, st);
  return tk ? launch_bwd_tr<DH, false, true>(a, st) : launch_bwd_tr<DH, false, false>(a, st);
}

int attn_bwd_tr(const AttnBwdArgs& a, hipStream_t st) {
  attn_rec_begin();
  if ((a.ldq * 2) % 16 || (a.ldk * 2) % 16 || (a.ldv * 2) % 16 || (a.lddo * 2) % 16 || (a.ldo * 2) % 16) return CL_EINVAL;
  if ((a.lddq * 2) % 16 || a.lse_stride % 64 || a.lse_stride < a.N) return CL_EINVAL;
  if ((a.dK == nullptr) != (a.dV == nullptr)) return CL_EINVAL;
  if (a.row_ws && (reinterpret_cast<uintptr_t>(a.row_ws) & 15)) return CL_EINVAL;
  if (a.dK && ((a.lddk * 2) % 16 || (a.lddv * 2) % 16)) return CL_EINVAL;
  switch (a.DH) {
    case 8: return launch_bwd_tr_t<8>(a, st);
    case 16: return launch_bwd_tr_t<16>(a, st);
    case 32: return launch_bwd_tr_t<32>(a, st);
    case 40: return launch_bwd_tr_t<40>(a, st);
    case 80: return launch_bwd_tr_t<80>(a, st);
    case 160: return launch_bwd_tr_t<160>(a, st);
    default: return CL_EINVAL;
  }
}

}
```

ctrlora_amd/csrc/capi.hip:

```cpp
#define CTRLORA_HIP_INTERNAL
#include "../../include/ctrlora_hip.h"
#include "attention.h"
#include "debug_hooks.h"
#include "elementwise.h"
#include "gemm.h"
#include "norm.h"

using namespace cl;

static inline hipStream_t S(void* s) { (void)hipGetLastError(); return reinterpret_cast<hipStream_t>(s); }

static GemmParams base_params() {
  GemmParams g{};
  g.alpha = 1.f; g.beta = 0.f; g.splitk = 1; g.mode = GEMM_LINEAR;
  return g;
}

extern "C" {

int cl_abi_version(void) { return CL_ABI_VERSION; }
int cl_last_hip_error(void) { return g_last_hip_error; }
const char* cl_last_hip_error_string(void) { return hipGetErrorString((hipError_t)g_last_hip_error); }

int cl_set_workspace(void* ptr, long bytes) {
  if (bytes < 0 || (bytes > 0 && !ptr) || (reinterpret_cast<uintptr_t>(ptr) & 15)) return CL_EINVAL;
  gemm_set_workspace(ptr, bytes);
  return CL_OK;
}
int cl_set_stream_workspace(void* stream, void* ptr, long bytes) {
  if (bytes <= 0 || !ptr || (reinterpret_cast<uintptr_t>(ptr) & 15)) return CL_EINVAL;
  return gemm_set_stream_workspace(S(stream), ptr, bytes);
}
int cl_gemm_force_config(int cfg) { g_gemm_force_cfg = cfg; return CL_OK; }
int cl_gemm_force_splitk(int splitk) { g_gemm_force_splitk = splitk < 0 ? 0 : splitk; return CL_OK; }
int cl_gemm_tune_set(int dtype, int mode, int M, int N, int K1, int K2, int geglu, int cfg, int splitk) {
  return gemm_tune_set(dtype, mode, M, N, K1, K2, geglu, cfg, splitk);
}
int cl_gemm_tune_clear(void) { gemm_tune_clear(); return CL_OK; }
int cl_gemm_tune_size(void) { return gemm_tune_size(); }
int cl_debug_attention_variant(int v) {
  switch (v) {
    case 0: case 1: case 11: case 13: case 14:
      g_attn_variant = v; g_attn_variant_dkv4 = 0; return CL_OK;
    case 21:
      g_attn_variant = 0; g_attn_variant_dkv4 = 1; return CL_OK;
    default: return CL_EINVAL;
  }
}
int cl_debug_attention_fuse_delta(int on) { g_attn_fuse_delta = on ? 1 : 0; return CL_OK; }
int cl_debug_attention_last_launch(int* out16) {
  static_assert(sizeof(AttnLaunchRec) == 16 * sizeof(int), "cl_debug_attention_last_launch: sixteen ints");
  if (!out16) return CL_EINVAL;
  const int* rec = reinterpret_cast<const int*>(&g_attn_last);
  for (int i = 0; i < 16; ++i) out16[i] = rec[i];
  return CL_OK;
}
int cl_debug_groupnorm_form(int three_pass, int one_pass) {
  g_gn_three_pass = three_pass ? 1 : 0; g_gn_one_pass = one_pass ? 1 : 0; return CL_OK;
}
int cl_debug_groupnorm_group(int mode) {
  if (mode != 0 && mode != 1 && mode != 2 && mode != 5 && mode != 6) return CL_EINVAL;
  g_gn_group = mode; return CL_OK;
}
int cl_debug_norm_last_launch(int* out12) {
  static_assert(sizeof(NormLaunchRec) == 12 * sizeof(int), "cl_debug_norm_last_launch: twelve ints");
  if (!out12) return CL_EINVAL;
  const int* rec = reinterpret_cast<const int*>(&g_norm_last);
  for (int i = 0; i < 12; ++i) out12[i] = rec[i];
  return CL_OK;
}

int cl_debug_groupnorm_coop(int on) { g_gn_coop = on ? 1 : 0; return CL_OK; }
int cl_debug_groupnorm_coop_timeouts(void) { return (int)gnc_timeouts(); }

int cl_debug_wgrad_ring(int slots) { if (slots != 3 && slots != 4 && slots != 6) return CL_EINVAL; g_wgrad_ring = slots; return CL_OK; }
int cl_debug_wgrad_last_launch(int* out32) {
  static_assert(sizeof(WgradLaunchRec) == 32 * sizeof(int), "cl_debug_wgrad_last_launch: thirty-two ints");
  if (!out32) return CL_EINVAL;
  const int* rec = reinterpret_cast<const int*>(&g_wgrad_last);
  for (int i = 0; i < 32; ++i) out32[i] = rec[i];
  return CL_OK;
}
int cl_debug_wgrad_last_problem(int i, long* out12) {
  static_assert(sizeof(WgradProbRec) == 12 * sizeof(long), "cl_debug_wgrad_last_problem: twelve longs");
  return wgrad_rec_problem(i, out12);
}
int cl_debug_ew_last_launch(int* out8) {
  static_assert(sizeof(EwLaunchRec) == 8 * sizeof(int), "cl_debug_ew_last_launch: eight ints");
  if (!out8) return CL_EINVAL;
  const int* rec = reinterpret_cast<const int*>(&g_ew_last);
  for (int i = 0; i < 8; ++i) out8[i] = rec[i];
  return CL_OK;
}
int cl_debug_gemm_xs_rules(int on) { g_gemm_xs_rules = on ? 1 : 0; return CL_OK; }
int cl_debug_gemm_tag(int on) { g_gemm_tag_on = on ? 1 : 0; return CL_OK; }
int cl_debug_gemm_tag_count(void) { return gemm_tag_count(); }
int cl_debug_gemm_tag_clear(void) { gemm_tag_clear(); return CL_OK; }
int cl_debug_gemm_config(int cfg, int* out10) { return gemm_config_get(cfg, out10); }
int cl_debug_gemm_tag_get(int i, long* out12) { return out12 ? gemm_tag_get(i, out12) : CL_EINVAL; }

int cl_gemm(const cl_gemm_params* p, int dtype, void* stream) {
  if (!p) return CL_EINVAL;
  GemmParams g{};
  g.A1 = p->A1; g.lda1 = p->lda1; g.K1 = p->K1; g.W1 = p->W1; g.ldw1 = p->ldw1;
  g.A2 = p->A2; g.lda2 = p->lda2; g.K2 = p->K2; g.W2 = p->W2; g.ldw2 = p->ldw2;
  g.M = p->M; g.N = p->N; g.mode = p->mode;
  g.B = p->B; g.Hin = p->Hin; g.Win = p->Win; g.Hout = p->Hout; g.Wout = p->Wout;
  g.zero_page = p->zero_page; g.bias = p->bias;
  g.rowbias = p->rowbias; g.ldrb = p->ldrb; g.rows_per_batch = p->rows_per_batch;
  g.residual = p->residual; g.ldr = p->ldr; g.alpha = p->alpha; g.beta = p->beta; g.act = p->act;
  g.C = p->C; g.ldc = p->ldc; g.out_f32 = p->out_f32; g.atomic = p->atomic; g.splitk = p->splitk < 1 ? 1 : p->splitk;
  g.a1_group_n = p->a1_group_n; g.a2_group_n = p->a2_group_n; g.alpha_n = p->alpha_n;
  g.ln_gamma = p->ln_gamma; g.ln_beta = p->ln_beta; g.ln_eps = p->ln_eps; g.ln_stats = p->ln_stats;
  return launch_gemm(g, dtype, S(stream));
}

int cl_lora_down(int dtype, const void* x, long ldx, const void* A, int r, void* t, long ldt, int M, int K,
                 void* stream) {
  GemmParams g = base_params();
  g.A1 = x; g.lda1 = ldx; g.K1 = K; g.W1 = A; g.ldw1 = K; g.M = M; g.N = r; g.C = t; g.ldc = ldt;
  return launch_gemm(g, dtype, S(stream));
}

int cl_lora_linear_fwd(int dtype, const void* x, long ldx, const void* W, const float* bias, const void* t,
                       long ldt, const void* Bup, int r, const void* residual, long ldr, int act, void* y,
                       long ldy, int M, int N, int K, void* stream) {
  GemmParams g = base_params();
  g.A1 = x; g.lda1 = ldx; g.K1 = K; g.W1 = W; g.ldw1 = K;
  if (r > 0) { g.A2 = t; g.lda2 = ldt; g.K2 = r; g.W2 = Bup; g.ldw2 = r; }
  g.M = M; g.N = N; g.bias = bias; g.act = act;
  if (residual) { g.residual = residual; g.ldr = ldr; g.beta = 1.f; }
  g.C = y; g.ldc = ldy;
  return launch_gemm(g, dtype, S(stream));
}

int cl_lora_linear_bwd_data(int dtype, const void* dy, long lddy, const void* Wt, const void* At, const void* Bt,
                            int r, void* u, long ldu, const void* accum, long ldacc, void* dx, long lddx, int M,
                            int N, int K, void* stream) {
  if (r > 0) {
    GemmParams g = base_params();
    g.A1 = dy; g.lda1 = lddy; g.K1 = N; g.W1 = Bt; g.ldw1 = N; g.M = M; g.N = r; g.C = u; g.ldc = ldu;
    const int rc = launch_gemm(g, dtype, S(stream));
    if (rc) return rc;
  }
  GemmParams g = base_params();
  g.A1 = dy; g.lda1 = lddy; g.K1 = N; g.W1 = Wt; g.ldw1 = N;
  if (r > 0) { g.A2 = u; g.lda2 = ldu; g.K2 = r; g.W2 = At; g.ldw2 = r; }
  g.M = M; g.N = K;
  if (accum) { g.residual = accum; g.ldr = ldacc; g.beta = 1.f; }
  g.C = dx; g.ldc = lddx;
  return launch_gemm(g, dtype, S(stream));
}

int cl_weight_grad(int dtype, const void* dyT, long lddyt, const void* xT, long ldxt, float* dW, long lddw, int N,
                   int K, int Mp, float scale, void* stream) {
  GemmParams g = base_params();
  g.A1 = dyT; g.lda1 = lddyt; g.K1 = Mp; g.W1 = xT; g.ldw1 = ldxt; g.M = N; g.N = K;
  g.alpha = scale; g.C = dW; g.ldc = lddw; g.out_f32 = 1; g.atomic = 1;
  const int kpb = dtype == CL_BF16 ? 32 : 16;
  const long tiles = (long)((N + 63) / 64) * ((K + 63) / 64);
  int sk = (int)(512 / (tiles > 0 ? tiles : 1));
  const int ksteps = Mp / kpb;
  if (sk > ksteps / 4) sk = ksteps / 4;
  if (sk < 1) sk = 1;
  if (sk > 64) sk = 64;
  g.splitk = sk;
  return launch_gemm(g, dtype, S(stream));
}

int cl_weight_grad_tn(int dtype, const void* dy, long lddy, const void* x, long ldx, float* dW, long lddw, int M,
                      int N, int K, float scale, const void* zero_page, void* stream) {
  wgrad_rec_begin();
  if (dtype != CL_BF16) return CL_EINVAL;
  return launch_wgrad_tn(dy, lddy, x, ldx, dW, lddw, M, N, K, scale, zero_page, S(stream));
}

int cl_weight_grad_tn_group(int dtype, int n, const cl_wgrad_desc* descs, const void* zero_page, void* stream) {
  wgrad_rec_begin();
  if (dtype != CL_BF16) return CL_EINVAL;
  if (n <= 0) return CL_OK;
  if (!descs || n > 4096) return CL_EINVAL;
  static_assert(sizeof(cl_wgrad_desc) == sizeof(WgradDesc), "descriptor layout");
  return launch_wgrad_tn_group(reinterpret_cast<const WgradDesc*>(descs), n, zero_page, S(stream));
}

int cl_conv3x3_fwd(int dtype, int mode, const void* x, long ldx, const void* Wp, const float* bias, const void* emb,
                   long ldemb, const void* residual, long ldr, void* y, long ldy, int B, int Hin, int Win, int Cin,
                   int Cout, const void* zero_page, void* stream) {
  GemmParams g = base_params();
  int Hout = Hin, Wout = Win;
  if (mode == GEMM_CONV_S2 || mode == GEMM_CONV_S2A) { Hout = Hin / 2; Wout = Win / 2; }
  else if (mode == GEMM_CONV_UP2 || mode == GEMM_CONV_T2) { Hout = 2 * Hin; Wout = 2 * Win; }
  else if (mode != GEMM_CONV_S1) return CL_EINVAL;
  g.mode = mode; g.A1 = x; g.lda1 = ldx; g.K1 = Cin; g.W1 = Wp; g.ldw1 = 9L * Cin;
  g.M = B * Hout * Wout; g.N = Cout; g.B = B; g.Hin = Hin; g.Win = Win; g.Hout = Hout; g.Wout = Wout;
  g.zero_page = zero_page; g.bias = bias;
  if (emb) { g.rowbias = emb; g.ldrb = ldemb; g.rows_per_batch = Hout * Wout; }
  if (residual) { g.residual = residual; g.ldr = ldr; g.beta = 1.f; }
  g.C = y; g.ldc = ldy;
  return launch_gemm(g, dtype, S(stream));
}

int cl_conv3x3_bwd_data(int dtype, int mode, const void* dy, long lddy, const void* Wd, const void* accum,
                        long ldacc, void* dx, long lddx, int B, int Hdy, int Wdy, int Cout, int Cin,
                        const void* zero_page, void* stream) {
  return cl_conv3x3_fwd(dtype, mode, dy, lddy, Wd, nullptr, nullptr, 0, accum, ldacc, dx, lddx, B, Hdy, Wdy, Cout,
                        Cin, zero_page, stream);
}

int cl_conv1x1_fwd(int dtype, const void* x, long ldx, const void* W, const float* bias, float scale,
                   const void* residual, long ldr, float beta, void* y, long ldy, int M, int Cin, int Cout,
                   void* stream) {
  GemmParams g = base_params();
  g.A1 = x; g.lda1 = ldx; g.K1 = Cin; g.W1 = W; g.ldw1 = Cin; g.M = M; g.N = Cout; g.bias = bias; g.alpha = scale;
  if (residual) { g.residual = residual; g.ldr = ldr; g.beta = beta; }
  g.C = y; g.ldc = ldy;
  return launch_gemm(g, dtype, S(stream));
}

long cl_groupnorm_ws_floats(int B, int HW, int C) { return gn_ws_floats(B, HW, C); }

int cl_groupnorm_silu_fwd(int dtype, const void* x, long ldx, void* y, long ldy, const float* gamma,
                          const float* beta, int B, int HW, int C, int groups, float eps, int silu, float* stats,
                          float* ws, void* stream) {
  GnArgs a{}; a.x = x; a.ldx = ldx; a.y = y; a.ldy = ldy; a.gamma = gamma; a.beta = beta; a.B = B; a.HW = HW; a.C = C;
  a.G = groups; a.eps = eps; a.silu = silu; a.stats = stats; a.ws = ws;
  return gn_fwd(a, dtype, S(stream));
}

int cl_groupnorm_silu_bwd(int dtype, const void* x, long ldx, const void* dy, long lddy, const void* accum,
                          long ldacc, void* dx, long lddx, const float* gamma, const float* beta, const float* stats,
                          int B, int HW, int C, int groups, int silu, float* dgamma, float* dbeta, float* ws,
                          void* stream) {
  GnBwdArgs a{}; a.x = x; a.ldx = ldx; a.dy = dy; a.lddy = lddy; a.accum = accum; a.ldacc = ldacc; a.dx = dx; a.lddx = lddx;
  a.gamma = gamma; a.beta = beta; a.stats = stats; a.B = B; a.HW = HW; a.C = C; a.G = groups; a.silu = silu;
  a.dgamma = dgamma; a.dbeta = dbeta; a.ws = ws;
  return gn_bwd(a, dtype, S(stream));
}

int cl_layernorm_fwd(int dtype, const void* x, long ldx, void* y, long ldy, const float* gamma, const float* beta,
                     int M, int D, float eps, float* stats, void* stream) {
  LnArgs a{}; a.x = x; a.ldx = ldx; a.y = y; a.ldy = ldy; a.gamma = gamma; a.beta = beta; a.M = M; a.D = D; a.eps = eps;
  a.stats = stats;
  return ln_fwd(a, dtype, S(stream));
}

int cl_layernorm_bwd(int dtype, const void* x, long ldx, const void* dy, long lddy, const void* accum, long ldacc,
                     void* dx, long lddx, const float* gamma, const float* stats, int M, int D, float* dgamma,
                     float* dbeta, void* stream) {
  LnBwdArgs a{}; a.x = x; a.ldx = ldx; a.dy = dy; a.lddy = lddy; a.accum = accum; a.ldacc = ldacc; a.dx = dx; a.lddx = lddx;
  a.gamma = gamma; a.stats = stats; a.M = M; a.D = D; a.dgamma = dgamma; a.dbeta = dbeta;
  return ln_bwd(a, dtype, S(stream));
}

int cl_attention_fwd(int dtype, const void* Q, long ldq, const void* K, long ldk, const void* Vt, int nkv_pad,
                     void* O, long ldo, float* LSE, int lse_stride, int B, int H, int N, int Nkv, int dh, float scale,
                     void* stream) {
  attn_rec_begin();
  AttnFwdArgs a{}; a.Q = Q; a.ldq = ldq; a.K = K; a.ldk = ldk; a.Vt = Vt; a.nkv_pad = nkv_pad; a.O = O; a.ldo = ldo;
  a.LSE = LSE; a.lse_stride = lse_stride; a.B = B; a.H = H; a.N = N; a.Nkv = Nkv; a.DH = dh; a.scale = scale;
  return attn_fwd(a, dtype, S(stream));
}

int cl_attention_bwd(int dtype, const void* Q, long ldq, const void* K, long ldk, const void* V, long ldv,
                     const void* O, long ldo, const void* dO, long lddo, const void* Qt, const void* dOt, int n_pad,
                     const void* Kt, int nkv_pad, const float* LSE, float* Delta, int lse_stride, void* dQ, long lddq,
                     void* dK, long lddk, void* dV, long lddv, int B, int H, int N, int Nkv, int dh, float scale,
                     void* stream) {
  attn_rec_begin();
  AttnBwdArgs a{}; a.Q = Q; a.ldq = ldq; a.K = K; a.ldk = ldk; a.V = V; a.ldv = ldv; a.O = O; a.ldo = ldo;
  a.dO = dO; a.lddo = lddo; a.Qt = Qt; a.dOt = dOt; a.n_pad = n_pad; a.Kt = Kt; a.nkv_pad = nkv_pad; a.LSE = LSE;
  a.Delta = Delta; a.lse_stride = lse_stride; a.dQ = dQ; a.lddq = lddq; a.dK = dK; a.lddk = lddk; a.dV = dV; a.lddv = lddv;
  a.B = B; a.H = H; a.N = N; a.Nkv = Nkv; a.DH = dh; a.scale = scale;
  return attn_bwd(a, dtype, S(stream));
}

int cl_attention_fwd_v2(int dtype, const void* Q, long ldq, const void* K, long ldk, const void* V, long ldv, void* O,
                        long ldo, float* LSE, int lse_stride, int B, int H, int N, int Nkv, int dh, float scale,
                        int flags, void* stream) {
  attn_rec_begin();
  if (dtype != CL_BF16 || (flags & ~CL_ATTN_Q_PRESCALED)) return CL_EINVAL;
  AttnFwdArgs a{}; a.Q = Q; a.ldq = ldq; a.K = K; a.ldk = ldk; a.O = O; a.ldo = ldo;
  a.LSE = LSE; a.lse_stride = lse_stride; a.B = B; a.H = H; a.N = N; a.Nkv = Nkv; a.DH = dh; a.scale = scale;
  a.q_prescaled = (flags & CL_ATTN_Q_PRESCALED) ? 1 : 0;
  return attn_fwd_tr(a, V, ldv, S(stream));
}

int cl_attention_fwd_ip(int dtype, const void* Q, long ldq, const void* K, long ldk, const void* V, long ldv,
                        const void* Kip, long ldkip, const void* Vip, long ldvip, void* O, long ldo, int B, int H, int N,
                        int Nkv, int Nip, int dh, float scale, float ip_scale, int flags, void* stream) {
  attn_rec_begin();
  if (flags & ~CL_ATTN_Q_PRESCALED) return CL_EINVAL;
  AttnFwdArgs a{}; a.Q = Q; a.ldq = ldq; a.K = K; a.ldk = ldk; a.O = O; a.ldo = ldo;
  a.B = B; a.H = H; a.N = N; a.Nkv = Nkv; a.DH = dh; a.scale = scale;
  a.q_prescaled = (flags & CL_ATTN_Q_PRESCALED) ? 1 : 0;
  AttnIpArgs ip{}; ip.K2 = Kip; ip.ldk2 = ldkip; ip.V2 = Vip; ip.ldv2 = ldvip; ip.Nip = Nip; ip.ip_scale = ip_scale;
  if (dtype == CL_BF16) return attn_fwd_tr_ip(a, V, ldv, ip, S(stream));
  if (ldv < 1 || ldv > 0x7fffffffL) return CL_EINVAL;
  a.Vt = V; a.nkv_pad = (int)ldv;
  return attn_fwd_ip(a, ip, dtype, S(stream));
}

int cl_attention_causal_fwd(int dtype, const void* Q, long ldq, const void* K, long ldk, const void* V, long ldv, void* O,
                            long ldo, int B, int H, int N, int dh, float scale, void* stream) {
  attn_rec_begin();
  return attn_causal_fwd(dtype, Q, ldq, K, ldk, V, ldv, O, ldo, B, H, N, dh, scale, S(stream));
}

int cl_attention_bwd_v2(int dtype, const void* Q, long ldq, const void* K, long ldk, const void* V, long ldv,
                        const void* O, long ldo, const void* dO, long lddo, const float* LSE, float* Delta,
                        int lse_stride, void* dQ, long lddq, void* dK, long lddk, void* dV, long lddv, int B, int H,
                        int N, int Nkv, int dh, float scale, int flags, void* row_ws, void* stream) {
  attn_rec_begin();
  if (dtype != CL_BF16 || (flags & ~CL_ATTN_Q_PRESCALED)) return CL_EINVAL;
  AttnBwdArgs a{}; a.Q = Q; a.ldq = ldq; a.K = K; a.ldk = ldk; a.V = V; a.ldv = ldv; a.O = O; a.ldo = ldo;
  a.dO = dO; a.lddo = lddo; a.LSE = LSE; a.Delta = Delta; a.lse_stride = lse_stride; a.dQ = dQ; a.lddq = lddq;
  a.dK = dK; a.lddk = lddk; a.dV = dV; a.lddv = lddv; a.B = B; a.H = H; a.N = N; a.Nkv = Nkv; a.DH = dh; a.scale = scale;
  a.q_prescaled = (flags & CL_ATTN_Q_PRESCALED) ? 1 : 0;
  a.row_ws = row_ws;
  return attn_bwd_tr(a, S(stream));
}

int cl_geglu_fwd(int dtype, const void* h, long ldh, void* out, long ldo, long M, int F, void* stream) { return geglu_fwd(dtype, h, ldh, out, ldo, M, F, S(stream)); }
int cl_geglu_bwd(int dtype, const void* h, long ldh, const void* dout, long lddo, void* dh, long lddh, long M, int F, void* stream) { return geglu_bwd(dtype, h, ldh, dout, lddo, dh, lddh, M, F, S(stream)); }
int cl_silu_fwd(int dtype, const void* x, void* y, long n, void* stream) { return silu_fwd(dtype, x, y, n, S(stream)); }
int cl_silu_bwd(int dtype, const void* x, const void* dy, void* dx, long n, void* stream) { return silu_bwd(dtype, x, dy, dx, n, S(stream)); }
int cl_axpby(int dtype, const void* x, long ldx, void* y, long ldy, long M, int C, float a, float b, void* stream) { return axpby(dtype, x, ldx, y, ldy, M, C, a, b, S(stream)); }
int cl_transpose(int in_dtype, int out_dtype, const void* in, long ldi, long bsi, void* out, long ldo, long bso, int Bt, int R, int C, int Rpad, void* stream) { return transpose(in_dtype, out_dtype, in, ldi, bsi, out, ldo, bso, Bt, R, C, Rpad, S(stream)); }
int cl_nchw_to_tok(int dtype, const float* in, void* out, long ldo, int B, int Cin, int Cpad, int HW, void* stream) { return nchw_to_tok(dtype, in, out, ldo, B, Cin, Cpad, HW, S(stream)); }
int cl_tok_to_nchw(int dtype, const void* in, long ldi, float* out, int B, int C, int HW, float alpha, float beta, void* stream) { return tok_to_nchw(dtype, in, ldi, out, B, C, HW, alpha, beta, S(stream)); }
int cl_colsum(int dtype, const void* in, long ldi, float* out, long ldo, int B, int HW, int C, float scale, void* stream) { return colsum(dtype, in, ldi, out, ldo, B, HW, C, scale, S(stream)); }
int cl_pool2x2(int dtype, const void* in, long ldi, void* out, long ldo, int B, int H, int W, int C, int accumulate, void* stream) { return pool2x2(dtype, in, ldi, out, ldo, B, H, W, C, accumulate, S(stream)); }
int cl_pack2d(int dtype, const float* in, long ldi, void* out, long ldo, long R, int C, int Cpad, void* stream) { return pack2d(dtype, in, ldi, out, ldo, R, C, Cpad, S(stream)); }
int cl_vit_patch_rows(int dtype, const float* pixels, void* out, long ldo, int B, int C, int S_, int P, int Kpad, void* stream) { return vit_patch_rows(dtype, pixels, out, ldo, B, C, S_, P, Kpad, S(stream)); }
int cl_vit_tokens(int dtype, const void* patch, long ldp, const float* cls, const float* pos, void* out, long ldo, int B, int T, int D, void* stream) { return vit_tokens(dtype, patch, ldp, cls, pos, out, ldo, B, T, D, S(stream)); }
int cl_clip_text_embed(int dtype, const long* ids, const float* tok, const float* pos, void* out, long ldo, int B, int T, int D, int vocab, void* stream) { return clip_text_embed(dtype, ids, tok, pos, out, ldo, B, T, D, vocab, S(stream)); }
int cl_gather_rows(int dtype, const void* src, long lds_, const long* rows, void* dst, long ldd, int R, int D, int nsrc, void* stream) { return gather_rows(dtype, src, lds_, rows, dst, ldd, R, D, nsrc, S(stream)); }
int cl_repack(int dtype, const float* flat, const long* desc, const int* tile_prefix, int ndesc, int total_tiles, void* stream) { return repack(dtype, flat, desc, tile_prefix, ndesc, total_tiles, S(stream)); }
int cl_timestep_embedding(int dtype, const long* t, const float* freqs, void* out, long ldo, int B, int half, void* stream) { return timestep_embed(dtype, t, freqs, out, ldo, B, half, S(stream)); }
int cl_qsample(const float* z, const float* noise, const long* t, const float* sqrt_ac, const float* sqrt_1mac, float* out, int B, long per_sample, void* stream) { return qsample(z, noise, t, sqrt_ac, sqrt_1mac, out, B, per_sample, S(stream)); }
int cl_qsample_blend(const float* x0, const float* noise, const long* t, const float* sqrt_ac, const float* sqrt_1mac, int T, const float* mask, int mask_per_batch, int mask_per_channel, const float* x, float* out, int B, int C, long HW, void* stream) { return qsample_blend(x0, noise, t, sqrt_ac, sqrt_1mac, T, mask, mask_per_batch, mask_per_channel, x, out, B, C, HW, S(stream)); }
int cl_posterior_sample_pair(const float* mom_a, const float* e_a, float* out_a, const float* mom_b, const float* e_b, float* out_b, int B, long per_sample, float scale, void* stream) { return posterior_sample_pair(mom_a, e_a, out_a, mom_b, e_b, out_b, B, per_sample, scale, S(stream)); }
int cl_mse_loss(const float* eps, const float* target, float* d_eps, float* loss, long n, float gscale, void* stream) { return mse_loss(eps, target, d_eps, loss, n, gscale, S(stream)); }
int cl_ddim_step(const float* x, const float* e_c, const float* e_u, const float* noise, const float* coef, int index, float scale, float* x_prev, float* pred_x0, long n, void* stream) { return ddim_step(x, e_c, e_u, noise, coef, index, scale, x_prev, pred_x0, n, S(stream)); }
int cl_adamw(float* p, const float* g, float* m, float* v, long n, float lr, float beta1, float beta2, float eps, float weight_decay, int step, float grad_scale, void* stream) { return adamw(p, g, m, v, n, lr, beta1, beta2, eps, weight_decay, step, grad_scale, S(stream)); }

int cl_p_losses_mse(const float* eps, const float* target, float* d_eps, const long* t, const float* lvlb, float* out, float* per_sample, float* scratch, int B, long per_sample_elems, float gscale, float w_simple, float w_elbo, void* stream) { return plosses_mse(eps, target, d_eps, t, lvlb, out, per_sample, scratch, B, per_sample_elems, gscale, w_simple, w_elbo, S(stream)); }
int cl_conv_tap_gather(int dtype, const void* x, long ldx, void* out, long ldo, int B, int Hin, int Win, int Hout, int Wout, int C, int tap, int stride, int pad, void* stream) { return conv_tap_gather(dtype, x, ldx, out, ldo, B, Hin, Win, Hout, Wout, C, tap, stride, pad, S(stream)); }
int cl_softmax_rows(int dtype, const float* Sm, long lds_, void* P, long ldp, long M, int N, float scale, void* stream) { return softmax_rows(dtype, Sm, lds_, P, ldp, M, N, scale, S(stream)); }
int cl_zero(void* p, long nbytes, void* stream) { return zero_bytes(p, nbytes, S(stream)); }
int cl_tick(int* counter, void* stream) { return tick(counter, S(stream)); }
int cl_adamw_dev(float* p, const float* g, float* m, float* v, long n, const float* hyper, int* step, void* stream) { return adamw_dev(p, g, m, v, n, hyper, step, S(stream)); }
long cl_grad_norm_scratch_floats(int nbuf) { return grad_norm_scratch_floats(nbuf); }
int cl_grad_norm(const float* const* bufs, const long* counts, int nbuf, const float* hyper, const float* max_norm, float* out, float* scratch, void* stream) { return grad_norm(bufs, counts, nbuf, hyper, max_norm, out, scratch, S(stream)); }
int cl_adamw_dev_clip(float* p, const float* g, float* m, float* v, long n, const float* hyper, int* step, const float* clip, void* stream) { return adamw_dev_clip(p, g, m, v, n, hyper, step, clip, S(stream)); }
int cl_ddim_set_t(const long* table, const int* cursor, int S_, long* ts, int n, void* stream) { return ddim_set_t(table, cursor, S_, ts, n, S(stream)); }
int cl_ddim_step_dev(const float* x, const float* e_c, const float* e_u, const float* noise, const float* coef, const int* cursor, int S_, float scale, float* x_prev, float* pred_x0, long n, void* stream) { return ddim_step_dev(x, e_c, e_u, noise, coef, cursor, S_, scale, x_prev, pred_x0, n, S(stream)); }
int cl_timestep_embedding_f(int dtype, const float* t, const float* freqs, void* out, long ldo, int B, int half, void* stream) { return timestep_embed_f(dtype, t, freqs, out, ldo, B, half, S(stream)); }
int cl_dpmpp_step(const float* x, const float* e_c, const float* e_u, const float* coef, int index, int S_, float scale, float* hist, float* x_next, float* pred_x0, long n, void* stream) { return dpmpp_step(x, e_c, e_u, coef, index, S_, scale, hist, x_next, pred_x0, n, S(stream)); }
int cl_dpmpp_step_dev(const float* x, const float* e_c, const float* e_u, const float* coef, const int* cursor, int S_, float scale, float* hist, float* x_next, float* pred_x0, long n, void* stream) { return dpmpp_step_dev(x, e_c, e_u, coef, cursor, S_, scale, hist, x_next, pred_x0, n, S(stream)); }
int cl_dpm_set_t(const float* coef, const int* cursor, int S_, float* ts, int n, void* stream) { return dpm_set_t(coef, cursor, S_, ts, n, S(stream)); }
int cl_plms_step(const float* x, const float* e_c, const float* e_u, const float* coef, int iter, int S_, int phase, float scale, float* hist, float* x_out, float* pred_x0, long n, void* stream) { return plms_step(x, e_c, e_u, coef, iter, S_, phase, scale, hist, x_out, pred_x0, n, S(stream)); }
int cl_plms_step_dev(const float* x, const float* e_c, const float* e_u, const float* coef, const int* cursor, int S_, float scale, float* hist, float* x_out, float* pred_x0, long n, void* stream) { return plms_step_dev(x, e_c, e_u, coef, cursor, S_, scale, hist, x_out, pred_x0, n, S(stream)); }

}
```

ctrlora_amd/csrc/debug_hooks.h:

```cpp
#pragma once
#ifdef __cplusplus
extern "C" {
#endif
int cl_debug_attention_variant(int variant);
int cl_debug_attention_fuse_delta(int on);
int cl_debug_attention_last_launch(int* out16);
int cl_debug_groupnorm_form(int three_pass, int one_pass);
int cl_debug_groupnorm_group(int mode);
int cl_debug_norm_last_launch(int* out12);
int cl_debug_wgrad_last_launch(int* out32);
int cl_debug_wgrad_last_problem(int i, long* out12);
int cl_debug_ew_last_launch(int* out8);
int cl_debug_groupnorm_coop(int on);
int cl_debug_groupnorm_coop_timeouts(void);
int cl_debug_gemm_tag(int on);
int cl_debug_gemm_xs_rules(int on);
int cl_debug_wgrad_ring(int slots);
int cl_debug_gemm_tag_count(void);
int cl_debug_gemm_tag_clear(void);
int cl_debug_gemm_tag_get(int i, long* out12);
int cl_debug_gemm_config(int cfg, int* out10);
#ifdef __cplusplus
}
#endif
```

ctrlora_amd/hip.py:

```python
from __future__ import annotations

import ctypes as C
import os
from typing import Optional

import torch

_HERE = os.path.dirname(os.path.abspath(__file__))
LIB_PATH = os.environ.get("CTRLORA_LIB") or os.path.join(_HERE, "libctrlora_hip.so")

BF16, F32 = 0, 1
LINEAR, CONV_S1, CONV_S2, CONV_UP2, CONV_T2, CONV_S2A, CONV_UP2P, CONV_T2P, CONV_S2K4 = 0, 1, 2, 3, 4, 5, 6, 7, 8
ACT_NONE, ACT_SILU, ACT_GEGLU, ACT_GEGLU_SPLIT, ACT_GELU = 0, 1, 2, 3, 4


class HipError(RuntimeError):
    pass


class WgradDesc(C.Structure):
    _fields_ = [("dy", C.c_void_p), ("lddy", C.c_long), ("x", C.c_void_p), ("ldx", C.c_long),
                ("dW", C.c_void_p), ("lddw", C.c_long), ("M", C.c_int), ("N", C.c_int), ("K", C.c_int),
                ("scale", C.c_float), ("tap", C.c_int), ("Hin", C.c_int), ("Win", C.c_int), ("Hout", C.c_int),
                ("Wout", C.c_int), ("stride", C.c_int), ("pad", C.c_int), ("reserved", C.c_int)]


class GemmParams(C.Structure):
    _fields_ = [
        ("A1", C.c_void_p), ("lda1", C.c_long), ("K1", C.c_int),
        ("W1", C.c_void_p), ("ldw1", C.c_long),
        ("A2", C.c_void_p), ("lda2", C.c_long), ("K2", C.c_int),
        ("W2", C.c_void_p), ("ldw2", C.c_long),
        ("M", C.c_int), ("N", C.c_int), ("mode", C.c_int),
        ("B", C.c_int), ("Hin", C.c_int), ("Win", C.c_int), ("Hout", C.c_int), ("Wout", C.c_int),
        ("zero_page", C.c_void_p), ("bias", C.c_void_p),
        ("rowbias", C.c_void_p), ("ldrb", C.c_long), ("rows_per_batch", C.c_int),
        ("residual", C.c_void_p), ("ldr", C.c_long),
        ("alpha", C.c_float), ("beta", C.c_float), ("act", C.c_int),
        ("C", C.c_void_p), ("ldc", C.c_long),
        ("out_f32", C.c_int), ("atomic", C.c_int), ("splitk", C.c_int),
        ("a1_group_n", C.c_int), ("a2_group_n", C.c_int), ("alpha_n", C.c_int),
        ("ln_gamma", C.c_void_p), ("ln_beta", C.c_void_p), ("ln_eps", C.c_float), ("ln_stats", C.c_void_p),
    ]


_lib = None

_P, _L, _I, _F = C.c_void_p, C.c_long, C.c_int, C.c_float
_SIGS = {
    "cl_abi_version": [],
    "cl_last_hip_error": [],
    "cl_set_workspace": [_P, _L],
    "cl_set_stream_workspace": [_P, _P, _L],
    "cl_gemm_force_config": [_I],
    "cl_gemm_force_splitk": [_I],
    "cl_gemm_tune_set": [_I] * 9,
    "cl_gemm_tune_clear": [],
    "cl_gemm_tune_size": [],
    "cl_gemm": [C.POINTER(GemmParams), _I, _P],
    "cl_lora_down": [_I, _P, _L, _P, _I, _P, _L, _I, _I, _P],
    "cl_lora_linear_fwd": [_I, _P, _L, _P, _P, _P, _L, _P, _I, _P, _L, _I, _P, _L, _I, _I, _I, _P],
    "cl_lora_linear_bwd_data": [_I, _P, _L, _P, _P, _P, _I, _P, _L, _P, _L, _P, _L, _I, _I, _I, _P],
    "cl_weight_grad": [_I, _P, _L, _P, _L, _P, _L, _I, _I, _I, _F, _P],
    "cl_weight_grad_tn_group": [_I, _I, _P, _P, _P],
    "cl_weight_grad_tn": [_I, _P, _L, _P, _L, _P, _L, _I, _I, _I, _F, _P, _P],
    "cl_conv3x3_fwd": [_I, _I, _P, _L, _P, _P, _P, _L, _P, _L, _P, _L, _I, _I, _I, _I, _I, _P, _P],
    "cl_conv3x3_bwd_data": [_I, _I, _P, _L, _P, _P, _L, _P, _L, _I, _I, _I, _I, _I, _P, _P],
    "cl_conv1x1_fwd": [_I, _P, _L, _P, _P, _F, _P, _L, _F, _P, _L, _I, _I, _I, _P],
    "cl_groupnorm_ws_floats": [_I, _I, _I],
    "cl_groupnorm_silu_fwd": [_I, _P, _L, _P, _L, _P, _P, _I, _I, _I, _I, _F, _I, _P, _P, _P],
    "cl_groupnorm_silu_bwd": [_I, _P, _L, _P, _L, _P, _L, _P, _L, _P, _P, _P, _I, _I, _I, _I, _I, _P, _P, _P, _P],
    "cl_layernorm_fwd": [_I, _P, _L, _P, _L, _P, _P, _I, _I, _F, _P, _P],
    "cl_layernorm_bwd": [_I, _P, _L, _P, _L, _P, _L, _P, _L, _P, _P, _I, _I, _P, _P, _P],
    "cl_attention_fwd": [_I, _P, _L, _P, _L, _P, _I, _P, _L, _P, _I, _I, _I, _I, _I, _I, _F, _P],
    "cl_attention_bwd": [_I, _P, _L, _P, _L, _P, _L, _P, _L, _P, _L, _P, _P, _I, _P, _I, _P, _P, _I, _P, _L, _P, _L,
                         _P, _L, _I, _I, _I, _I, _I, _F, _P],
    "cl_attention_fwd_v2": [_I, _P, _L, _P, _L, _P, _L, _P, _L, _P, _I, _I, _I, _I, _I, _I, _F, _I, _P],
    "cl_attention_fwd_ip": [_I, _P, _L, _P, _L, _P, _L, _P, _L, _P, _L, _P, _L, _I, _I, _I, _I, _I, _I, _F, _F, _I, _P],
    "cl_attention_bwd_v2": [_I, _P, _L, _P, _L, _P, _L, _P, _L, _P, _L, _P, _P, _I, _P, _L, _P, _L, _P, _L,
                            _I, _I, _I, _I, _I, _F, _I, _P, _P],
    "cl_attention_causal_fwd": [_I, _P, _L, _P, _L, _P, _L, _P, _L, _I, _I, _I, _I, _F, _P],
    "cl_geglu_fwd": [_I, _P, _L, _P, _L, _L, _I, _P],
    "cl_geglu_bwd": [_I, _P, _L, _P, _L, _P, _L, _L, _I, _P],
    "cl_silu_fwd": [_I, _P, _P, _L, _P],
    "cl_silu_bwd": [_I, _P, _P, _P, _L, _P],
    "cl_axpby": [_I, _P, _L, _P, _L, _L, _I, _F, _F, _P],
    "cl_transpose": [_I, _I, _P, _L, _L, _P, _L, _L, _I, _I, _I, _I, _P],
    "cl_nchw_to_tok": [_I, _P, _P, _L, _I, _I, _I, _I, _P],
    "cl_tok_to_nchw": [_I, _P, _L, _P, _I, _I, _I, _F, _F, _P],
    "cl_colsum": [_I, _P, _L, _P, _L, _I, _I, _I, _F, _P],
    "cl_pool2x2": [_I, _P, _L, _P, _L, _I, _I, _I, _I, _I, _P],
    "cl_pack2d": [_I, _P, _L, _P, _L, _L, _I, _I, _P],
    "cl_vit_patch_rows": [_I, _P, _P, _L, _I, _I, _I, _I, _I, _P],
    "cl_vit_tokens": [_I, _P, _L, _P, _P, _P, _L, _I, _I, _I, _P],
    "cl_clip_text_embed": [_I, _P, _P, _P, _P, _L, _I, _I, _I, _I, _P],
    "cl_gather_rows": [_I, _P, _L, _P, _P, _L, _I, _I, _I, _P],
    "cl_repack": [_I, _P, _P, _P, _I, _I, _P],
    "cl_timestep_embedding": [_I, _P, _P, _P, _L, _I, _I, _P],
    "cl_qsample": [_P, _P, _P, _P, _P, _P, _I, _L, _P],
    "cl_mse_loss": [_P, _P, _P, _P, _L, _F, _P],
    "cl_p_losses_mse": [_P, _P, _P, _P, _P, _P, _P, _P, _I, _L, _F, _F, _F, _P],
    "cl_zero": [_P, _L, _P],
    "cl_softmax_rows": [_I, _P, _L, _P, _L, _L, _I, _F, _P],
    "cl_conv_tap_gather": [_I, _P, _L, _P, _L, _I, _I, _I, _I, _I, _I, _I, _I, _I, _P],
    "cl_ddim_step": [_P, _P, _P, _P, _P, _I, _F, _P, _P, _L, _P],
    "cl_tick": [_P, _P],
    "cl_adamw_dev": [_P, _P, _P, _P, _L, _P, _P, _P],
    "cl_ddim_set_t": [_P, _P, _I, _P, _I, _P],
    "cl_ddim_step_dev": [_P, _P, _P, _P, _P, _P, _I, _F, _P, _P, _L, _P],
    "cl_adamw": [_P, _P, _P, _P, _L, _F, _F, _F, _F, _F, _I, _F, _P],
    "cl_timestep_embedding_f": [_I, _P, _P, _P, _L, _I, _I, _P],
    "cl_dpmpp_step": [_P, _P, _P, _P, _I, _I, _F, _P, _P, _P, _L, _P],
    "cl_dpmpp_step_dev": [_P, _P, _P, _P, _P, _I, _F, _P, _P, _P, _L, _P],
    "cl_dpm_set_t": [_P, _P, _I, _P, _I, _P],
    "cl_posterior_sample_pair": [_P, _P, _P, _P, _P, _P, _I, _L, _F, _P],
    "cl_plms_step": [_P, _P, _P, _P, _I, _I, _I, _F, _P, _P, _P, _L, _P],
    "cl_plms_step_dev": [_P, _P, _P, _P, _P, _I, _F, _P, _P, _P, _L, _P],
    "cl_qsample_blend": [_P, _P, _P, _P, _P, _I, _P, _I, _I, _P, _P, _I, _I, _L, _P],
    "cl_grad_norm_scratch_floats": [_I],
    "cl_grad_norm": [_P, _P, _I, _P, _P, _P, _P, _P],
    "cl_adamw_dev_clip": [_P, _P, _P, _P, _L, _P, _P, _P, _P],
}
_LONG_RESULT = ("cl_groupnorm_ws_floats", "cl_grad_norm_scratch_floats")
EXPORTED = tuple(_SIGS.keys())
_DEBUG_SIGS = {
    "cl_debug_attention_variant": [_I],
    "cl_debug_attention_fuse_delta": [_I],
    "cl_debug_attention_last_launch": [_P],
    "cl_debug_groupnorm_form": [_I, _I],
    "cl_debug_groupnorm_group": [_I],
    "cl_debug_norm_last_launch": [_P],
    "cl_debug_groupnorm_coop": [_I],
    "cl_debug_groupnorm_coop_timeouts": [],
    "cl_debug_gemm_tag": [_I],
    "cl_debug_gemm_xs_rules": [_I],
    "cl_debug_wgrad_ring": [_I],
    "cl_debug_wgrad_last_launch": [_P],
    "cl_debug_wgrad_last_problem": [_I, _P],
    "cl_debug_ew_last_launch": [_P],
    "cl_debug_gemm_tag_count": [],
    "cl_debug_gemm_tag_clear": [],
    "cl_debug_gemm_tag_get": [_I, _P],
    "cl_debug_gemm_config": [_I, _P],
}


def lib():
    global _lib
    if _lib is None:
        if not os.path.exists(LIB_PATH):
            raise HipError(f"{LIB_PATH} not found -- run `python -m ctrlora_amd.build` "
                           "(the CtrLoRA engine has no non-HIP fallback)")
        L = C.CDLL(LIB_PATH)
        for name, args in {**_SIGS, **_DEBUG_SIGS}.items():
            fn = getattr(L, name)
            fn.argtypes = args
            fn.restype = C.c_long if name in _LONG_RESULT else C.c_int
        _lib = L
        if os.environ.get("CTRLORA_ATTN_FUSE_DELTA", "1") == "0":
            L.cl_debug_attention_fuse_delta(0)
        gn3 = os.environ.get("CTRLORA_GN_THREE_PASS", "0") == "1"
        gn1 = os.environ.get("CTRLORA_GN_ONE_PASS", "1") != "0"
        if gn3 or not gn1:
            L.cl_debug_groupnorm_form(int(gn3), int(gn1))
        if os.environ.get("CTRLORA_GN_GROUP", "1") == "0":
            L.cl_debug_groupnorm_group(0)
        if os.environ.get("CTRLORA_GN_COOP", "0") == "1":
            L.cl_debug_groupnorm_coop(1)
        L.cl_debug_gemm_xs_rules(int(XS_ENABLED))
        if os.environ.get("CTRLORA_WGRAD_RING"):
            L.cl_debug_wgrad_ring(int(os.environ["CTRLORA_WGRAD_RING"]))
        if os.environ.get("CTRLORA_GEMM_TUNED", "1") != "0":
            load_gemm_table(os.environ.get("CTRLORA_GEMM_TABLE", GEMM_TABLE_PATH))
            if "CTRLORA_GEMM_TABLE" not in os.environ:
                if XS_ENABLED:
                    load_gemm_table(GEMM_XS_TABLE_PATH, clear=False)
                if R06_ENABLED and os.path.exists(GEMM_R06_TABLE_PATH):
                    load_gemm_table(GEMM_R06_TABLE_PATH, clear=False)
    return _lib


GEMM_TABLE_PATH = os.path.join(os.path.dirname(os.path.abspath(__file__)), "gemm_tuned_gfx950.json")
GEMM_XS_TABLE_PATH = os.path.join(os.path.dirname(os.path.abspath(__file__)), "gemm_tuned_gfx950_xs.json")
GEMM_R06_TABLE_PATH = os.path.join(os.path.dirname(os.path.abspath(__file__)), "gemm_tuned_gfx950_r06.json")
R06_ENABLED = os.environ.get("CTRLORA_GEMM_R06", "1") != "0"
XS_ENABLED = os.environ.get("CTRLORA_GEMM_XS", "1") != "0"


LN_PROLOGUE = os.environ.get("CTRLORA_LN_PROLOGUE", "1") != "0"


def xs_ln_ok(M: int, N: int, K: int, act: int = 0) -> bool:
    if not (XS_ENABLED and LN_PROLOGUE) or K not in (320, 640) or M < 128:
        return False
    if act == ACT_GEGLU_SPLIT:
        return N % 64 == 0 and xs_geglu_ok(M, K, 0)
    return act == ACT_NONE and N % 32 == 0


def gemm_tags():
    L = lib()
    out = []
    buf = (C.c_long * 12)()
    for i in range(int(L.cl_debug_gemm_tag_count())):
        _chk(L.cl_debug_gemm_tag_get(i, C.cast(buf, C.c_void_p)), "cl_debug_gemm_tag_get")
        v = list(buf)
        out.append(dict(dtype=v[0], mode=v[1], M=v[2], N=v[3], K1=v[4], K2=v[5], act=v[6], residual=v[7], tag=v[8],
                        workgroups=v[9], wg_size=v[10], launches=v[11]))
    return out


def xs_geglu_ok(M: int, K: int, r: int) -> bool:
    if not XS_ENABLED or r not in (0, 128):
        return False
    return (K == 320 and M >= 128) or (K == 640 and M >= 8192)


def load_gemm_table(path: str, clear: bool = True) -> int:
    import json
    L = lib()
    if clear:
        L.cl_gemm_tune_clear()
    if not path or not os.path.exists(path):
        return 0
    with open(path) as f:
        tab = json.load(f)
    for row in tab.get("entries", []):
        _chk(L.cl_gemm_tune_set(*[int(v) for v in row[:9]]), "cl_gemm_tune_set")
    return int(L.cl_gemm_tune_size())


def _chk(rc: int, what: str):
    if rc != 0:
        detail = "unsupported shape/alignment"
        if rc != 1:
            L = lib()
            L.cl_last_hip_error_string.restype = C.c_char_p
            detail = f"HIP launch error {L.cl_last_hip_error()}: {L.cl_last_hip_error_string().decode()}"
        raise HipError(f"{what} failed with code {rc} ({detail})")


def dt(t: torch.Tensor) -> int:
    if t.dtype == torch.bfloat16:
        return BF16
    if t.dtype == torch.float32:
        return F32
    raise HipError(f"unsupported dtype {t.dtype}")


def dt_of(dtype: torch.dtype) -> int:
    return BF16 if dtype == torch.bfloat16 else F32


def stream() -> int:
    return torch.cuda.current_stream().cuda_stream


def ptr(t: Optional[torch.Tensor]):
    return None if t is None else t.data_ptr()


def ld(t: Optional[torch.Tensor]) -> int:
    if t is None:
        return 0
    assert t.dim() == 2 and t.stride(1) == 1, (t.shape, t.stride())
    return t.stride(0)


ZERO_PAGE_BYTES = 16384
_zero_pages = {}
_workspace = None
WORKSPACE_BYTES = 64 << 20


_stream_ws = {}


def bind_stream_workspace(stream: "torch.cuda.Stream", nbytes: int = 32 << 20) -> None:
    key = stream.cuda_stream
    if key not in _stream_ws:
        buf = torch.empty(nbytes, dtype=torch.uint8, device=stream.device)
        _chk(lib().cl_set_stream_workspace(key, buf.data_ptr(), nbytes), "cl_set_stream_workspace")
        _stream_ws[key] = buf


_side_streams = {}


def side_stream(device) -> "torch.cuda.Stream":
    key = str(device)
    st = _side_streams.get(key)
    if st is None:
        st = torch.cuda.Stream(device=device)
        bind_stream_workspace(st)
        _side_streams[key] = st
    return st


def ensure_workspace(device) -> None:
    global _workspace
    if _workspace is None:
        _workspace = torch.empty(WORKSPACE_BYTES, dtype=torch.uint8, device=device)
        _chk(lib().cl_set_workspace(_workspace.data_ptr(), WORKSPACE_BYTES), "cl_set_workspace")


def zero_page(device) -> torch.Tensor:
    k = str(device)
    if k not in _zero_pages:
        _zero_pages[k] = torch.zeros(ZERO_PAGE_BYTES, dtype=torch.uint8, device=device)
    return _zero_pages[k]



def gemm(a1, w1, out, *, a2=None, w2=None, bias=None, rowbias=None, rows_per_batch=0, residual=None,
         alpha=1.0, beta=0.0, act=ACT_NONE, mode=LINEAR, conv=None, k1=None, out_f32=False, atomic=False,
         splitk=1, M=None, N=None, dtype=None, a1_group_n=0, a2_group_n=0, alpha_n=0, ln=None):
    p = GemmParams()
    if _workspace is None:
        ensure_workspace(a1.device)
    dty = dt(a1) if dtype is None else dtype
    p.A1 = a1.data_ptr(); p.lda1 = ld(a1); p.K1 = a1.shape[1] if k1 is None else k1
    p.W1 = w1.data_ptr(); p.ldw1 = ld(w1)
    if a2 is not None:
        p.A2 = a2.data_ptr(); p.lda2 = ld(a2); p.W2 = w2.data_ptr(); p.ldw2 = ld(w2)
        p.K2 = w2.shape[1] if a2_group_n else a2.shape[1]
    p.M = out.shape[0] if M is None else M
    p.N = out.shape[1] if N is None else N
    p.mode = mode
    if conv is not None:
        p.B, p.Hin, p.Win, p.Hout, p.Wout = conv
        p.zero_page = zero_page(a1.device).data_ptr()
    p.bias = ptr(bias)
    if rowbias is not None:
        p.rowbias = rowbias.data_ptr(); p.ldrb = ld(rowbias); p.rows_per_batch = rows_per_batch
    if residual is not None:
        p.residual = residual.data_ptr(); p.ldr = ld(residual)
    p.alpha = alpha; p.beta = beta; p.act = act
    p.C = out.data_ptr(); p.ldc = ld(out)
    p.out_f32 = int(out_f32); p.atomic = int(atomic); p.splitk = splitk
    p.a1_group_n = a1_group_n; p.a2_group_n = a2_group_n; p.alpha_n = alpha_n
    if ln is not None:
        p.ln_gamma = ln[0].data_ptr(); p.ln_beta = ln[1].data_ptr(); p.ln_eps = ln[2]; p.ln_stats = ptr(ln[3])
    _chk(lib().cl_gemm(C.byref(p), dty, stream()), "cl_gemm")
    return out


WGRAD_F32_DETERMINISTIC = os.environ.get("CTRLORA_WGRAD_F32_DETERMINISTIC", "0") == "1"


def weight_grad(dyT, xT, dW, scale=1.0):
    if WGRAD_F32_DETERMINISTIC and dyT.dtype == torch.float32:
        if dW.data_ptr() % 16 or ld(dW) % 8 or dW.shape[1] % 8:
            raise HipError(f"deterministic fp32 weight gradient: dW must be 16-byte aligned with a row stride and a width that are "
                           f"multiples of 8 (got offset {dW.data_ptr() % 16}, ld {ld(dW)}, width {dW.shape[1]})")
        gemm(dyT, xT, dW, residual=dW, alpha=scale, beta=1.0, out_f32=True)
        return
    _chk(lib().cl_weight_grad(dt(dyT), dyT.data_ptr(), ld(dyT), xT.data_ptr(), ld(xT), dW.data_ptr(), ld(dW),
                              dyT.shape[0], xT.shape[0], dyT.shape[1], scale, stream()), "cl_weight_grad")


def weight_grad_tn_group(problems):
    n = len(problems)
    if n == 0:
        return
    if _workspace is None:
        ensure_workspace(problems[0][0].device)
    arr = (WgradDesc * n)()
    for d, prob in zip(arr, problems):
        dy, x, dW, scale = prob[:4]
        d.dy = dy.data_ptr(); d.lddy = ld(dy); d.x = x.data_ptr(); d.ldx = ld(x)
        d.dW = dW.data_ptr(); d.lddw = ld(dW); d.M = dy.shape[0]; d.N = dy.shape[1]; d.K = x.shape[1]
        d.scale = scale
        d.tap = -1
        if len(prob) > 4 and prob[4] is not None:
            d.tap, d.Hin, d.Win, d.Hout, d.Wout, d.stride, d.pad = prob[4]
    _chk(lib().cl_weight_grad_tn_group(BF16, n, C.cast(arr, C.c_void_p), zero_page(problems[0][0].device).data_ptr(),
                                       stream()), "cl_weight_grad_tn_group")


def repack(dtype, flat, desc, tile_prefix, ndesc, total_tiles):
    _chk(lib().cl_repack(dt_of(dtype), flat.data_ptr(), desc.data_ptr(), tile_prefix.data_ptr(), ndesc, total_tiles,
                         stream()), "cl_repack")


def weight_grad_tn(dy, x, dW, scale=1.0):
    if _workspace is None:
        ensure_workspace(dy.device)
    _chk(lib().cl_weight_grad_tn(dt(dy), dy.data_ptr(), ld(dy), x.data_ptr(), ld(x), dW.data_ptr(), ld(dW),
                                 dy.shape[0], dy.shape[1], x.shape[1], scale, zero_page(dy.device).data_ptr(),
                                 stream()), "cl_weight_grad_tn")



def groupnorm_ws(B, HW, C_) -> int:
    return int(lib().cl_groupnorm_ws_floats(B, HW, C_))


def groupnorm_fwd(x, y, gamma, beta, B, HW, eps, silu, stats, ws, groups=32):
    _chk(lib().cl_groupnorm_silu_fwd(dt(x), x.data_ptr(), ld(x), y.data_ptr(), ld(y), gamma.data_ptr(),
                                     beta.data_ptr(), B, HW, x.shape[1], groups, eps, int(silu), stats.data_ptr(),
                                     ws.data_ptr(), stream()), "cl_groupnorm_silu_fwd")
    return y


def groupnorm_bwd(x, dy, dx, gamma, beta, stats, B, HW, silu, ws, accum=None, dgamma=None, dbeta=None, groups=32):
    _chk(lib().cl_groupnorm_silu_bwd(dt(x), x.data_ptr(), ld(x), dy.data_ptr(), ld(dy), ptr(accum), ld(accum),
                                     dx.data_ptr(), ld(dx), gamma.data_ptr(), beta.data_ptr(), stats.data_ptr(), B, HW,
                                     x.shape[1], groups, int(silu), ptr(dgamma), ptr(dbeta), ws.data_ptr(), stream()),
         "cl_groupnorm_silu_bwd")
    return dx


def layernorm_fwd(x, y, gamma, beta, eps=1e-5, stats=None):
    _chk(lib().cl_layernorm_fwd(dt(x), x.data_ptr(), ld(x), y.data_ptr(), ld(y), gamma.data_ptr(), beta.data_ptr(),
                                x.shape[0], x.shape[1], eps, ptr(stats), stream()), "cl_layernorm_fwd")
    return y


def layernorm_bwd(x, dy, dx, gamma, stats, accum=None, dgamma=None, dbeta=None):
    _chk(lib().cl_layernorm_bwd(dt(x), x.data_ptr(), ld(x), dy.data_ptr(), ld(dy), ptr(accum), ld(accum),
                                dx.data_ptr(), ld(dx), gamma.data_ptr(), stats.data_ptr(), x.shape[0], x.shape[1],
                                ptr(dgamma), ptr(dbeta), stream()), "cl_layernorm_bwd")
    return dx



def attention_fwd(q, k, vt, o, lse, B, H, N, Nkv, dh, scale):
    _chk(lib().cl_attention_fwd(dt(q), q.data_ptr(), ld(q), k.data_ptr(), ld(k), vt.data_ptr(), vt.shape[-1],
                                o.data_ptr(), ld(o), ptr(lse), 0 if lse is None else lse.shape[-1], B, H, N, Nkv, dh,
                                scale, stream()), "cl_attention_fwd")
    return o


def attention_bwd(q, k, v, o, do, qt, dot, kt, lse, delta, dq, dk, dv, B, H, N, Nkv, dh, scale):
    _chk(lib().cl_attention_bwd(dt(q), q.data_ptr(), ld(q), k.data_ptr(), ld(k), v.data_ptr(), ld(v), o.data_ptr(),
                                ld(o), do.data_ptr(), ld(do), qt.data_ptr(), dot.data_ptr(), qt.shape[-1],
                                kt.data_ptr(), kt.shape[-1], lse.data_ptr(), delta.data_ptr(), lse.shape[-1],
                                dq.data_ptr(), ld(dq), ptr(dk), ld(dk), ptr(dv), ld(dv), B, H, N, Nkv, dh, scale,
                                stream()), "cl_attention_bwd")


ATTN_Q_PRESCALED = 1


def attention_fwd_v2(q, k, v, o, lse, B, H, N, Nkv, dh, scale, q_prescaled=False):
    _chk(lib().cl_attention_fwd_v2(dt(q), q.data_ptr(), ld(q), k.data_ptr(), ld(k), v.data_ptr(), ld(v), o.data_ptr(),
                                   ld(o), ptr(lse), 0 if lse is None else lse.shape[-1], B, H, N, Nkv, dh, scale,
                                   ATTN_Q_PRESCALED if q_prescaled else 0, stream()), "cl_attention_fwd_v2")
    return o


def attention_fwd_ip(q, k, v, k_ip, v_ip, o, B, H, N, Nkv, Nip, dh, scale, ip_scale, q_prescaled=False):
    if dt(q) == BF16:
        lv, lvi = ld(v), ld(v_ip)
    else:
        lv, lvi = v.shape[-1], v_ip.shape[-1]
    _chk(lib().cl_attention_fwd_ip(dt(q), q.data_ptr(), ld(q), k.data_ptr(), ld(k), v.data_ptr(), lv, k_ip.data_ptr(),
                                   ld(k_ip), v_ip.data_ptr(), lvi, o.data_ptr(), ld(o), B, H, N, Nkv, Nip, dh, scale,
                                   ip_scale, ATTN_Q_PRESCALED if q_prescaled else 0, stream()), "cl_attention_fwd_ip")
    return o


def attention_bwd_v2(q, k, v, o, do, lse, delta, dq, dk, dv, B, H, N, Nkv, dh, scale, q_prescaled=False, row_ws=None):
    assert row_ws is None or row_ws.numel() * row_ws.element_size() >= B * H * lse.shape[-1] * 32
    _chk(lib().cl_attention_bwd_v2(dt(q), q.data_ptr(), ld(q), k.data_ptr(), ld(k), v.data_ptr(), ld(v), o.data_ptr(),
                                   ld(o), do.data_ptr(), ld(do), lse.data_ptr(), delta.data_ptr(), lse.shape[-1],
                                   dq.data_ptr(), ld(dq), ptr(dk), ld(dk), ptr(dv), ld(dv), B, H, N, Nkv, dh, scale,
                                   ATTN_Q_PRESCALED if q_prescaled else 0, ptr(row_ws), stream()), "cl_attention_bwd_v2")



def _transposed(x, B, rows, inner, pad, out=None):
    if out is None:
        out = torch.empty((B, inner, pad), dtype=x.dtype, device=x.device)
    assert tuple(out.shape) == (B, inner, pad) and out.dtype == x.dtype
    return transpose(x, out, B, rows, inner, pad, ldi=x.stride(0))


def attention(q, k, v, o, lse, B, H, N, Nkv, dh, scale, *, q_prescaled=False, ip=None, vt=None):
    assert ip is None or lse is None
    if dt(q) == BF16:
        if ip is None:
            return attention_fwd_v2(q, k, v, o, lse, B, H, N, Nkv, dh, scale, q_prescaled=q_prescaled)
        k_ip, v_ip, Nip, ip_scale = ip
        return attention_fwd_ip(q, k, v, k_ip, v_ip, o, B, H, N, Nkv, Nip, dh, scale, ip_scale, q_prescaled=q_prescaled)
    assert not q_prescaled, "the fp32 kernels scale the scores themselves"
    vt = _transposed(v, B, Nkv, H * dh, (Nkv + 63) // 64 * 64, vt)
    if ip is None:
        return attention_fwd(q, k, vt, o, lse, B, H, N, Nkv, dh, scale)
    k_ip, v_ip, Nip, ip_scale = ip
    vt_ip = _transposed(v_ip, B, Nip, H * dh, 64)
    return attention_fwd_ip(q, k, vt, k_ip, vt_ip, o, B, H, N, Nkv, Nip, dh, scale, ip_scale)


def attention_causal(q, k, v, o, B, H, N, dh, scale):
    assert dt(q) == dt(k) == dt(v) == dt(o)
    _chk(lib().cl_attention_causal_fwd(dt(q), q.data_ptr(), ld(q), k.data_ptr(), ld(k), v.data_ptr(), ld(v), o.data_ptr(), ld(o),
                                       B, H, N, dh, float(scale), stream()), "cl_attention_causal_fwd")
    return o


def attention_backward(q, k, v, o, do, lse, delta, dq, dk, dv, B, H, N, Nkv, dh, scale, *, q_prescaled=False):
    if dt(q) == BF16:
        row_ws = torch.empty(lse.numel() * 8, dtype=torch.float32, device=q.device) if (q_prescaled and dh == 40) else None
        return attention_bwd_v2(q, k, v, o, do, lse, delta, dq, dk, dv, B, H, N, Nkv, dh, scale, q_prescaled=q_prescaled,
                                row_ws=row_ws)
    assert not q_prescaled, "the fp32 kernels scale the scores themselves"
    inner, npad, kpad = H * dh, (N + 63) // 64 * 64, (Nkv + 63) // 64 * 64
    qt = _transposed(q, B, N, inner, npad)
    dot = _transposed(do, B, N, inner, npad)
    kt = _transposed(k, B, Nkv, inner, kpad)
    attention_bwd(q, k, v, o, do, qt, dot, kt, lse, delta, dq, dk, dv, B, H, N, Nkv, dh, scale)



def geglu_fwd(h, out):
    _chk(lib().cl_geglu_fwd(dt(h), h.data_ptr(), ld(h), out.data_ptr(), ld(out), h.shape[0], out.shape[1], stream()),
         "cl_geglu_fwd")
    return out


def geglu_bwd(h, dout, dh):
    _chk(lib().cl_geglu_bwd(dt(h), h.data_ptr(), ld(h), dout.data_ptr(), ld(dout), dh.data_ptr(), ld(dh), h.shape[0],
                            dout.shape[1], stream()), "cl_geglu_bwd")
    return dh


def silu_fwd(x, y):
    _chk(lib().cl_silu_fwd(dt(x), x.data_ptr(), y.data_ptr(), x.numel(), stream()), "cl_silu_fwd")
    return y


def silu_bwd(x, dy, dx):
    _chk(lib().cl_silu_bwd(dt(x), x.data_ptr(), dy.data_ptr(), dx.data_ptr(), x.numel(), stream()), "cl_silu_bwd")
    return dx


def axpby(x, y, a=1.0, b=1.0):
    _chk(lib().cl_axpby(dt(x), x.data_ptr(), ld(x), y.data_ptr(), ld(y), x.shape[0], x.shape[1], a, b, stream()),
         "cl_axpby")
    return y


def transpose(src, dst, Bt, R, C_, Rpad, ldi=None, bsi=None):
    ldi = src.stride(-2) if ldi is None else ldi
    bsi = R * ldi if bsi is None else bsi
    _chk(lib().cl_transpose(dt(src), dt(dst), src.data_ptr(), ldi, bsi, dst.data_ptr(), Rpad, C_ * Rpad, Bt, R, C_,
                            Rpad, stream()), "cl_transpose")
    return dst


def nchw_to_tok(x_nchw, out, Cpad=None):
    B, Cin, H, W = x_nchw.shape
    x_nchw = x_nchw.contiguous()
    _chk(lib().cl_nchw_to_tok(dt(out), x_nchw.data_ptr(), out.data_ptr(), ld(out), B, Cin,
                              out.shape[1] if Cpad is None else Cpad, H * W, stream()), "cl_nchw_to_tok")
    return out


def tok_to_nchw(tok, out_nchw, alpha=1.0, beta=0.0):
    B, C_, H, W = out_nchw.shape
    _chk(lib().cl_tok_to_nchw(dt(tok), tok.data_ptr(), ld(tok), out_nchw.data_ptr(), B, C_, H * W, alpha, beta,
                              stream()), "cl_tok_to_nchw")
    return out_nchw


def colsum(x, out_f32, B, HW, scale=1.0):
    _chk(lib().cl_colsum(dt(x), x.data_ptr(), ld(x), out_f32.data_ptr(), ld(out_f32), B, HW, x.shape[1], scale,
                         stream()), "cl_colsum")
    return out_f32


def pool2x2(src, dst, B, H, W, accumulate=False):
    _chk(lib().cl_pool2x2(dt(src), src.data_ptr(), ld(src), dst.data_ptr(), ld(dst), B, H, W, dst.shape[1],
                          int(accumulate), stream()), "cl_pool2x2")
    return dst


def pack2d(src_f32, dst, Cpad=None):
    R, C_ = src_f32.shape
    _chk(lib().cl_pack2d(dt(dst), src_f32.data_ptr(), ld(src_f32), dst.data_ptr(), ld(dst), R, C_,
                         dst.shape[1] if Cpad is None else Cpad, stream()), "cl_pack2d")
    return dst


def vit_patch_rows(pixels, out, P):
    B, C_, S, S2 = pixels.shape
    assert S == S2 and pixels.dtype == torch.float32 and pixels.is_contiguous() and out.shape[0] == B * (S // P) ** 2
    _chk(lib().cl_vit_patch_rows(dt(out), pixels.data_ptr(), out.data_ptr(), ld(out), B, C_, S, P, out.shape[1], stream()),
         "cl_vit_patch_rows")
    return out


def clip_text_embed(ids, tok, pos, out):
    B, T = ids.shape
    vocab, D = tok.shape
    assert ids.dtype == torch.long and ids.is_contiguous() and tok.is_contiguous() and pos.is_contiguous()
    assert out.shape == (B * T, D) and pos.shape[0] >= T and pos.shape[1] == D and tok.dtype == pos.dtype == torch.float32
    if not ids.is_cuda:
        if ids.numel() and (int(ids.min()) < 0 or int(ids.max()) >= vocab):
            raise HipError(f"cl_clip_text_embed: token id outside [0, {vocab})")
        ids = ids.to(out.device)
    _chk(lib().cl_clip_text_embed(dt(out), ids.data_ptr(), tok.data_ptr(), pos.data_ptr(), out.data_ptr(), ld(out), B, T, D, vocab,
                                  stream()), "cl_clip_text_embed")
    return out


def gather_rows(src, rows, dst):
    R, D = dst.shape
    assert rows.dtype == torch.long and rows.is_cuda and rows.is_contiguous() and rows.numel() == R and src.shape[1] == D
    assert src.dtype == dst.dtype
    _chk(lib().cl_gather_rows(dt(dst), src.data_ptr(), ld(src), rows.data_ptr(), dst.data_ptr(), ld(dst), R, D, src.shape[0], stream()),
         "cl_gather_rows")
    return dst


def vit_tokens(patch, cls, pos, out, B):
    T, D = pos.shape
    assert out.shape == (B * T, D) and patch.shape == (B * (T - 1), D) and cls.is_contiguous() and pos.is_contiguous()
    _chk(lib().cl_vit_tokens(dt(out), patch.data_ptr(), ld(patch), cls.data_ptr(), pos.data_ptr(), out.data_ptr(), ld(out), B, T, D,
                             stream()), "cl_vit_tokens")
    return out


def timestep_embedding(t_long, freqs, out):
    _chk(lib().cl_timestep_embedding(dt(out), t_long.data_ptr(), freqs.data_ptr(), out.data_ptr(), ld(out),
                                     t_long.shape[0], freqs.shape[0], stream()), "cl_timestep_embedding")
    return out


def timestep_embedding_f(t_f32, freqs, out):
    assert t_f32.dtype == torch.float32 and t_f32.is_contiguous()
    _chk(lib().cl_timestep_embedding_f(dt(out), t_f32.data_ptr(), freqs.data_ptr(), out.data_ptr(), ld(out),
                                       t_f32.shape[0], freqs.shape[0], stream()), "cl_timestep_embedding_f")
    return out


def qsample(z, noise, t, sqrt_ac, sqrt_1mac, out):
    B = z.shape[0]
    _chk(lib().cl_qsample(z.data_ptr(), noise.data_ptr(), t.data_ptr(), sqrt_ac.data_ptr(), sqrt_1mac.data_ptr(),
                          out.data_ptr(), B, z.numel() // B, stream()), "cl_qsample")
    return out


def qsample_blend(x0, noise, t, sqrt_ac, sqrt_1mac, mask, x, out):
    B, Cn = x0.shape[0], x0.shape[1]
    hw = tuple(x0.shape[2:])
    if mask.dim() != x0.dim() or tuple(mask.shape[2:]) != hw or mask.shape[0] not in (1, B) or mask.shape[1] not in (1, Cn):
        raise ValueError(f"mask {tuple(mask.shape)} is none of the layouts (B | 1, C | 1, H, W) of a sample {tuple(x0.shape)}")
    for v in (x0, noise, sqrt_ac, sqrt_1mac, mask, x, out):
        assert v.dtype == torch.float32 and v.is_contiguous()
    assert t.dtype == torch.long and t.is_contiguous() and t.numel() == B
    assert noise.shape == x0.shape == x.shape == out.shape and sqrt_ac.numel() == sqrt_1mac.numel()
    HW = 1
    for d in hw:
        HW *= int(d)
    _chk(lib().cl_qsample_blend(x0.data_ptr(), noise.data_ptr(), t.data_ptr(), sqrt_ac.data_ptr(), sqrt_1mac.data_ptr(),
                                sqrt_ac.numel(), mask.data_ptr(), int(mask.shape[0] != 1), int(mask.shape[1] != 1),
                                x.data_ptr(), out.data_ptr(), B, Cn, HW, stream()), "cl_qsample_blend")
    return out


def posterior_sample_pair(mom_a, e_a, out_a, scale, mom_b=None, e_b=None, out_b=None):
    ts = [t for t in (mom_a, e_a, out_a, mom_b, e_b, out_b) if t is not None]
    assert all(t.dtype == torch.float32 and t.is_contiguous() for t in ts)
    B = e_a.shape[0]
    per = e_a.numel() // B if B else 0
    assert mom_a.numel() == 2 * e_a.numel() == 2 * out_a.numel()
    assert mom_b is None or (mom_b.numel() == mom_a.numel() and e_b.numel() == e_a.numel() and out_b.numel() == out_a.numel())
    _chk(lib().cl_posterior_sample_pair(mom_a.data_ptr(), e_a.data_ptr(), out_a.data_ptr(), ptr(mom_b), ptr(e_b), ptr(out_b),
                                        B, per, float(scale), stream()), "cl_posterior_sample_pair")
    return out_a, out_b


def mse_loss(eps, target, d_eps, loss, gscale=1.0):
    _chk(lib().cl_mse_loss(eps.data_ptr(), target.data_ptr(), ptr(d_eps), loss.data_ptr(), eps.numel(), gscale,
                           stream()), "cl_mse_loss")
    return loss


def p_losses_mse(eps, target, d_eps, t, lvlb, out3, scratch, gscale=1.0, w_simple=1.0, w_elbo=0.0, per_sample=None):
    B = eps.shape[0]
    assert scratch.numel() >= 16 * B and eps.is_contiguous() and target.is_contiguous()
    _chk(lib().cl_p_losses_mse(eps.data_ptr(), target.data_ptr(), ptr(d_eps), ptr(t), ptr(lvlb), out3.data_ptr(),
                               ptr(per_sample), scratch.data_ptr(), B, eps.numel() // B, gscale, w_simple, w_elbo,
                               stream()), "cl_p_losses_mse")
    return out3


def conv_tap_gather(x, out, B, Hin, Win, Hout, Wout, tap, stride, pad):
    _chk(lib().cl_conv_tap_gather(dt(x), x.data_ptr(), ld(x), out.data_ptr(), ld(out), B, Hin, Win, Hout, Wout, x.shape[1], tap,
                                  stride, pad, stream()), "cl_conv_tap_gather")
    return out


def softmax_rows(scores_f32, probs, scale=1.0):
    M, N = scores_f32.shape
    _chk(lib().cl_softmax_rows(dt(probs), scores_f32.data_ptr(), ld(scores_f32), probs.data_ptr(), ld(probs), M, N, scale,
                               stream()), "cl_softmax_rows")
    return probs


def zero_(t):
    assert t.is_contiguous()
    _chk(lib().cl_zero(t.data_ptr(), t.numel() * t.element_size(), stream()), "cl_zero")
    return t


def ddim_step(x, e_c, e_u, noise, coef, index, scale, x_prev, pred_x0=None):
    _chk(lib().cl_ddim_step(x.data_ptr(), e_c.data_ptr(), ptr(e_u), ptr(noise), coef.data_ptr(), index, scale,
                            x_prev.data_ptr(), ptr(pred_x0), x.numel(), stream()), "cl_ddim_step")
    return x_prev


def adamw(p, g, m, v, lr, step, beta1=0.9, beta2=0.999, eps=1e-8, weight_decay=1e-2, grad_scale=1.0):
    _chk(lib().cl_adamw(p.data_ptr(), g.data_ptr(), m.data_ptr(), v.data_ptr(), p.numel(), lr, beta1, beta2, eps,
                        weight_decay, step, grad_scale, stream()), "cl_adamw")


def tick(counter):
    _chk(lib().cl_tick(counter.data_ptr(), stream()), "cl_tick")


def adamw_dev(p, g, m, v, hyper, step):
    _chk(lib().cl_adamw_dev(p.data_ptr(), g.data_ptr(), m.data_ptr(), v.data_ptr(), p.numel(), hyper.data_ptr(),
                            step.data_ptr(), stream()), "cl_adamw_dev")


GRAD_NORM_MAX_BUFS = 16


def grad_norm_scratch_floats(nbuf=1):
    return int(lib().cl_grad_norm_scratch_floats(nbuf))


def grad_norm(bufs, hyper, max_norm, out, scratch):
    n = len(bufs)
    for b in bufs:
        assert b.dtype == torch.float32 and b.is_contiguous(), (b.dtype, b.stride())
    ptrs = (C.c_void_p * max(n, 1))(*[b.data_ptr() for b in bufs])
    counts = (C.c_long * max(n, 1))(*[b.numel() for b in bufs])
    _chk(lib().cl_grad_norm(ptrs, counts, n, hyper.data_ptr(), ptr(max_norm), out.data_ptr(), scratch.data_ptr(), stream()),
         "cl_grad_norm")
    return out


def adamw_dev_clip(p, g, m, v, hyper, step, clip):
    _chk(lib().cl_adamw_dev_clip(p.data_ptr(), g.data_ptr(), m.data_ptr(), v.data_ptr(), p.numel(), hyper.data_ptr(),
                                 step.data_ptr(), clip.data_ptr(), stream()), "cl_adamw_dev_clip")


def ddim_set_t(table, cursor, S, ts):
    _chk(lib().cl_ddim_set_t(table.data_ptr(), cursor.data_ptr(), S, ts.data_ptr(), ts.numel(), stream()), "cl_ddim_set_t")
    return ts


def ddim_step_dev(x, e_c, e_u, noise, coef, cursor, S, scale, x_prev, pred_x0=None):
    _chk(lib().cl_ddim_step_dev(x.data_ptr(), e_c.data_ptr(), ptr(e_u), ptr(noise), coef.data_ptr(), cursor.data_ptr(),
                                S, scale, x_prev.data_ptr(), ptr(pred_x0), x.numel(), stream()), "cl_ddim_step_dev")
    return x_prev


def _dpm_args(x, e_c, e_u, coef, S, hist, x_next, pred_x0):
    n = x.numel()
    assert coef.dtype == torch.float32 and coef.is_contiguous() and tuple(coef.shape) == (S, 8), tuple(coef.shape)
    assert hist.dtype == torch.float32 and hist.is_contiguous() and hist.numel() == 3 * n
    for t in (x, e_c, e_u, x_next, pred_x0):
        assert t is None or (t.dtype == torch.float32 and t.is_contiguous() and t.numel() == n)
    return n


def dpmpp_step(x, e_c, e_u, coef, index, scale, hist, x_next, pred_x0=None):
    S = coef.shape[0]
    n = _dpm_args(x, e_c, e_u, coef, S, hist, x_next, pred_x0)
    _chk(lib().cl_dpmpp_step(x.data_ptr(), e_c.data_ptr(), ptr(e_u), coef.data_ptr(), index, S, scale, hist.data_ptr(),
                             x_next.data_ptr(), ptr(pred_x0), n, stream()), "cl_dpmpp_step")
    return x_next


def dpmpp_step_dev(x, e_c, e_u, coef, cursor, S, scale, hist, x_next, pred_x0=None):
    n = _dpm_args(x, e_c, e_u, coef, S, hist, x_next, pred_x0)
    _chk(lib().cl_dpmpp_step_dev(x.data_ptr(), e_c.data_ptr(), ptr(e_u), coef.data_ptr(), cursor.data_ptr(), S, scale,
                                 hist.data_ptr(), x_next.data_ptr(), ptr(pred_x0), n, stream()), "cl_dpmpp_step_dev")
    return x_next


def dpm_set_t(coef, cursor, S, ts):
    assert ts.dtype == torch.float32 and ts.is_contiguous() and tuple(coef.shape) == (S, 8)
    _chk(lib().cl_dpm_set_t(coef.data_ptr(), cursor.data_ptr(), S, ts.data_ptr(), ts.numel(), stream()), "cl_dpm_set_t")
    return ts


PLMS_MULTISTEP, PLMS_START, PLMS_FINISH = 0, 1, 2


def _plms_args(x, e_c, e_u, coef, S, hist, x_out, pred_x0):
    n = x.numel()
    assert coef.dtype == torch.float32 and coef.is_contiguous() and tuple(coef.shape) == (S, 4), tuple(coef.shape)
    assert hist.dtype == torch.float32 and hist.is_contiguous() and hist.numel() == 4 * n
    for t in (x, e_c, e_u, x_out, pred_x0):
        assert t is None or (t.dtype == torch.float32 and t.is_contiguous() and t.numel() == n)
    return n


def plms_step(x, e_c, e_u, coef, iteration, phase, scale, hist, x_out, pred_x0=None):
    S = coef.shape[0]
    n = _plms_args(x, e_c, e_u, coef, S, hist, x_out, pred_x0)
    _chk(lib().cl_plms_step(x.data_ptr(), e_c.data_ptr(), ptr(e_u), coef.data_ptr(), iteration, S, phase, scale,
                            hist.data_ptr(), x_out.data_ptr(), ptr(pred_x0), n, stream()), "cl_plms_step")
    return x_out


def plms_step_dev(x, e_c, e_u, coef, cursor, S, scale, hist, x_out, pred_x0=None):
    n = _plms_args(x, e_c, e_u, coef, S, hist, x_out, pred_x0)
    _chk(lib().cl_plms_step_dev(x.data_ptr(), e_c.data_ptr(), ptr(e_u), coef.data_ptr(), cursor.data_ptr(), S, scale,
                                hist.data_ptr(), x_out.data_ptr(), ptr(pred_x0), n, stream()), "cl_plms_step_dev")
    return x_out
```

include/ctrlora_hip.h:

```cpp
#ifndef CTRLORA_HIP_H
#define CTRLORA_HIP_H

#ifdef __cplusplus
extern "C" {
#endif

#ifndef CTRLORA_HIP_INTERNAL
#define CL_OK 0
#define CL_EINVAL 1
#define CL_ELAUNCH 2
#define CL_BF16 0
#define CL_F32 1
#endif

#define CL_ABI_VERSION 7
int cl_abi_version(void);
int cl_last_hip_error(void);

int cl_set_workspace(void* device_ptr, long bytes);
int cl_set_stream_workspace(void* stream, void* device_ptr, long bytes);
int cl_gemm_force_config(int cfg);
int cl_gemm_force_splitk(int splitk);
int cl_gemm_tune_set(int dtype, int mode, int M, int N, int K1, int K2, int geglu, int cfg, int splitk);
int cl_gemm_tune_clear(void);
int cl_gemm_tune_size(void);

enum cl_gemm_mode {
  CL_GEMM_LINEAR = 0,
  CL_GEMM_CONV_S1 = 1,
  CL_GEMM_CONV_S2 = 2,
  CL_GEMM_CONV_UP2 = 3,
  CL_GEMM_CONV_T2 = 4,
  CL_GEMM_CONV_S2A = 5,
  CL_GEMM_CONV_UP2P = 6,
  CL_GEMM_CONV_T2P = 7,
  CL_GEMM_CONV_S2K4 = 8
};

typedef struct cl_gemm_params {
  const void* A1; long lda1; int K1;
  const void* W1; long ldw1;
  const void* A2; long lda2; int K2;
  const void* W2; long ldw2;
  int M, N;
  int mode;
  int B, Hin, Win, Hout, Wout;
  const void* zero_page;
  const float* bias;
  const void* rowbias; long ldrb; int rows_per_batch;
  const void* residual; long ldr;
  float alpha, beta;
  int act;
  void* C; long ldc;
  int out_f32;
  int atomic;
  int splitk;
  int a1_group_n, a2_group_n;
  int alpha_n;
  const float* ln_gamma; const float* ln_beta; float ln_eps; float* ln_stats;
} cl_gemm_params;

int cl_gemm(const cl_gemm_params* p, int dtype, void* stream);

int cl_lora_down(int dtype, const void* x, long ldx, const void* A, int r, void* t, long ldt,
                 int M, int K, void* stream);
int cl_lora_linear_fwd(int dtype, const void* x, long ldx, const void* W, const float* bias,
                       const void* t, long ldt, const void* Bup, int r,
                       const void* residual, long ldr, int act, void* y, long ldy,
                       int M, int N, int K, void* stream);
int cl_lora_linear_bwd_data(int dtype, const void* dy, long lddy, const void* Wt, const void* At,
                            const void* Bt, int r, void* u, long ldu, const void* accum, long ldacc,
                            void* dx, long lddx, int M, int N, int K, void* stream);
int cl_weight_grad(int dtype, const void* dyT, long lddyt, const void* xT, long ldxt, float* dW,
                   long lddw, int N, int K, int Mp, float scale, void* stream);

int cl_weight_grad_tn(int dtype, const void* dy, long lddy, const void* x, long ldx, float* dW, long lddw,
                      int M, int N, int K, float scale, const void* zero_page, void* stream);

typedef struct cl_wgrad_desc {
  const void* dy; long lddy;
  const void* x; long ldx;
  float* dW; long lddw;
  int M, N, K; float scale;
  int tap, Hin, Win, Hout, Wout, stride, pad, reserved;
} cl_wgrad_desc;
int cl_weight_grad_tn_group(int dtype, int n, const cl_wgrad_desc* descs, const void* zero_page, void* stream);

int cl_conv3x3_fwd(int dtype, int mode, const void* x, long ldx, const void* Wp, const float* bias,
                   const void* emb, long ldemb, const void* residual, long ldr, void* y, long ldy,
                   int B, int Hin, int Win, int Cin, int Cout, const void* zero_page, void* stream);
int cl_conv3x3_bwd_data(int dtype, int mode, const void* dy, long lddy, const void* Wd,
                        const void* accum, long ldacc, void* dx, long lddx,
                        int B, int Hdy, int Wdy, int Cout, int Cin, const void* zero_page, void* stream);

int cl_conv1x1_fwd(int dtype, const void* x, long ldx, const void* W, const float* bias, float scale,
                   const void* residual, long ldr, float beta, void* y, long ldy,
                   int M, int Cin, int Cout, void* stream);

long cl_groupnorm_ws_floats(int B, int HW, int C);
int cl_groupnorm_silu_fwd(int dtype, const void* x, long ldx, void* y, long ldy, const float* gamma,
                          const float* beta, int B, int HW, int C, int groups, float eps, int silu,
                          float* stats, float* ws, void* stream);
int cl_groupnorm_silu_bwd(int dtype, const void* x, long ldx, const void* dy, long lddy,
                          const void* accum, long ldacc, void* dx, long lddx, const float* gamma,
                          const float* beta, const float* stats, int B, int HW, int C, int groups,
                          int silu, float* dgamma, float* dbeta, float* ws, void* stream);
int cl_layernorm_fwd(int dtype, const void* x, long ldx, void* y, long ldy, const float* gamma,
                     const float* beta, int M, int D, float eps, float* stats, void* stream);
int cl_layernorm_bwd(int dtype, const void* x, long ldx, const void* dy, long lddy, const void* accum,
                     long ldacc, void* dx, long lddx, const float* gamma, const float* stats, int M,
                     int D, float* dgamma, float* dbeta, void* stream);

int cl_attention_fwd(int dtype, const void* Q, long ldq, const void* K, long ldk, const void* Vt,
                     int nkv_pad, void* O, long ldo, float* LSE, int lse_stride, int B, int H, int N,
                     int Nkv, int dh, float scale, void* stream);
int cl_attention_bwd(int dtype, const void* Q, long ldq, const void* K, long ldk, const void* V,
                     long ldv, const void* O, long ldo, const void* dO, long lddo, const void* Qt,
                     const void* dOt, int n_pad, const void* Kt, int nkv_pad, const float* LSE,
                     float* Delta, int lse_stride, void* dQ, long lddq, void* dK, long lddk, void* dV,
                     long lddv, int B, int H, int N, int Nkv, int dh, float scale, void* stream);

enum { CL_ATTN_Q_PRESCALED = 1 };
int cl_attention_fwd_v2(int dtype, const void* Q, long ldq, const void* K, long ldk, const void* V, long ldv,
                        void* O, long ldo, float* LSE, int lse_stride, int B, int H, int N, int Nkv, int dh,
                        float scale, int flags, void* stream);
int cl_attention_bwd_v2(int dtype, const void* Q, long ldq, const void* K, long ldk, const void* V, long ldv,
                        const void* O, long ldo, const void* dO, long lddo, const float* LSE, float* Delta,
                        int lse_stride, void* dQ, long lddq, void* dK, long lddk, void* dV, long lddv,
                        int B, int H, int N, int Nkv, int dh, float scale, int flags, void* row_ws, void* stream);
int cl_attention_fwd_ip(int dtype, const void* Q, long ldq, const void* K, long ldk, const void* V, long ldv,
                        const void* Kip, long ldkip, const void* Vip, long ldvip, void* O, long ldo, int B, int H,
                        int N, int Nkv, int Nip, int dh, float scale, float ip_scale, int flags, void* stream);
int cl_attention_causal_fwd(int dtype, const void* Q, long ldq, const void* K, long ldk, const void* V, long ldv,
                            void* O, long ldo, int B, int H, int N, int dh, float scale, void* stream);

int cl_geglu_fwd(int dtype, const void* h, long ldh, void* out, long ldo, long M, int F, void* stream);
int cl_geglu_bwd(int dtype, const void* h, long ldh, const void* dout, long lddo, void* dh, long lddh, long M, int F, void* stream);
int cl_silu_fwd(int dtype, const void* x, void* y, long n, void* stream);
int cl_silu_bwd(int dtype, const void* x, const void* dy, void* dx, long n, void* stream);
int cl_axpby(int dtype, const void* x, long ldx, void* y, long ldy, long M, int C, float a, float b, void* stream);
int cl_transpose(int in_dtype, int out_dtype, const void* in, long ldi, long bsi, void* out, long ldo,
                 long bso, int Bt, int R, int C, int Rpad, void* stream);
int cl_nchw_to_tok(int dtype, const float* in, void* out, long ldo, int B, int Cin, int Cpad, int HW, void* stream);
int cl_tok_to_nchw(int dtype, const void* in, long ldi, float* out, int B, int C, int HW, float alpha, float beta, void* stream);
int cl_colsum(int dtype, const void* in, long ldi, float* out, long ldo, int B, int HW, int C, float scale, void* stream);
int cl_pool2x2(int dtype, const void* in, long ldi, void* out, long ldo, int B, int H, int W, int C, int accumulate, void* stream);
int cl_pack2d(int dtype, const float* in, long ldi, void* out, long ldo, long R, int C, int Cpad, void* stream);
int cl_vit_patch_rows(int dtype, const float* pixels, void* out, long ldo, int B, int C, int S, int P, int Kpad, void* stream);
int cl_vit_tokens(int dtype, const void* patch, long ldp, const float* cls, const float* pos, void* out, long ldo, int B, int T,
                  int D, void* stream);
int cl_clip_text_embed(int dtype, const long* ids, const float* tok, const float* pos, void* out, long ldo, int B, int T, int D,
                       int vocab, void* stream);
int cl_gather_rows(int dtype, const void* src, long lds, const long* rows, void* dst, long ldd, int R, int D, int nsrc, void* stream);
int cl_repack(int dtype, const float* flat, const long* desc, const int* tile_prefix, int ndesc,
              int total_tiles, void* stream);
int cl_timestep_embedding(int dtype, const long* t, const float* freqs, void* out, long ldo, int B, int half, void* stream);
int cl_timestep_embedding_f(int dtype, const float* t, const float* freqs, void* out, long ldo, int B, int half, void* stream);

int cl_conv_tap_gather(int dtype, const void* x, long ldx, void* out, long ldo, int B, int Hin, int Win, int Hout,
                       int Wout, int C, int tap, int stride, int pad, void* stream);
int cl_softmax_rows(int dtype, const float* S, long lds, void* P, long ldp, long M, int N, float scale, void* stream);

int cl_qsample(const float* z, const float* noise, const long* t, const float* sqrt_ac, const float* sqrt_1mac,
               float* out, int B, long per_sample, void* stream);
int cl_qsample_blend(const float* x0, const float* noise, const long* t, const float* sqrt_ac, const float* sqrt_1mac,
                     int T, const float* mask, int mask_per_batch, int mask_per_channel, const float* x, float* out,
                     int B, int C, long HW, void* stream);
int cl_posterior_sample_pair(const float* mom_a, const float* e_a, float* out_a, const float* mom_b, const float* e_b,
                             float* out_b, int B, long per_sample, float scale, void* stream);
int cl_mse_loss(const float* eps, const float* target, float* d_eps, float* loss, long n, float gscale, void* stream);
int cl_p_losses_mse(const float* eps, const float* target, float* d_eps, const long* t, const float* lvlb, float* out,
                    float* per_sample, float* scratch, int B, long per_sample_elems, float gscale, float w_simple,
                    float w_elbo, void* stream);
int cl_zero(void* p, long nbytes, void* stream);
int cl_ddim_step(const float* x, const float* e_c, const float* e_u, const float* noise, const float* coef,
                 int index, float scale, float* x_prev, float* pred_x0, long n, void* stream);
int cl_adamw(float* p, const float* g, float* m, float* v, long n, float lr, float beta1, float beta2,
             float eps, float weight_decay, int step, float grad_scale, void* stream);

int cl_tick(int* counter, void* stream);
int cl_adamw_dev(float* p, const float* g, float* m, float* v, long n, const float* hyper, int* step, void* stream);
long cl_grad_norm_scratch_floats(int nbuf);
int cl_grad_norm(const float* const* bufs, const long* counts, int nbuf, const float* hyper, const float* max_norm, float* out,
                 float* scratch, void* stream);
int cl_adamw_dev_clip(float* p, const float* g, float* m, float* v, long n, const float* hyper, int* step, const float* clip,
                      void* stream);
int cl_ddim_set_t(const long* table, const int* cursor, int S, long* ts, int n, void* stream);
int cl_ddim_step_dev(const float* x, const float* e_c, const float* e_u, const float* noise, const float* coef,
                     const int* cursor, int S, float scale, float* x_prev, float* pred_x0, long n, void* stream);

int cl_dpmpp_step(const float* x, const float* e_c, const float* e_u, const float* coef, int index, int S, float scale,
                  float* hist, float* x_next, float* pred_x0, long n, void* stream);
int cl_dpmpp_step_dev(const float* x, const float* e_c, const float* e_u, const float* coef, const int* cursor, int S,
                      float scale, float* hist, float* x_next, float* pred_x0, long n, void* stream);
int cl_dpm_set_t(const float* coef, const int* cursor, int S, float* ts, int n, void* stream);

int cl_plms_step(const float* x, const float* e_c, const float* e_u, const float* coef, int iter, int S, int phase,
                 float scale, float* hist, float* x_out, float* pred_x0, long n, void* stream);
int cl_plms_step_dev(const float* x, const float* e_c, const float* e_u, const float* coef, const int* cursor, int S,
                     float scale, float* hist, float* x_out, float* pred_x0, long n, void* stream);

#ifdef __cplusplus
}
#endif
#endif
```

Baseline: 241.3 images/s.

## Add short-KV attention forward/backward kernels that stage all keys once per block

Adds a specialised attention path for cross-attention with a short key/value sequence (Nkv up to 96, dh 40/80, as with SD1.5 text context of 77 tokens). Each workgroup loads the whole K and V into LDS once, then walks several 64-row query blocks without any online-softmax rescaling. The backward fuses the delta computation and writes dK/dV partials into a float workspace slab that is reduced afterwards. This cuts the repeated K/V tiling and the masked 64-wide padding overhead of the generic kernels, at the cost of extra workspace memory and a reduction step.

```diff
diff --git a/ctrlora_amd/build.py b/ctrlora_amd/build.py
--- a/ctrlora_amd/build.py
+++ b/ctrlora_amd/build.py
@@ -10,7 +10,7 @@
 CSRC = os.path.join(HERE, "csrc")
 OBJ = os.path.join(ROOT, "build", "obj")
 LIB = os.path.join(HERE, "libctrlora_hip.so")
-SOURCES = ["gemm.hip", "gemm_xs.hip", "gemm_w4.hip", "wgrad.hip", "norm.hip", "norm_coop.hip", "elementwise.hip", "attention_fwd.hip", "attention_bwd.hip", "attention_tr.hip", "attention_fwd40.hip", "attention_causal.hip", "capi.hip"]
+SOURCES = ["gemm.hip", "gemm_xs.hip", "gemm_w4.hip", "wgrad.hip", "norm.hip", "norm_coop.hip", "elementwise.hip", "attention_fwd.hip", "attention_bwd.hip", "attention_tr.hip", "attention_sk.hip", "attention_fwd40.hip", "attention_causal.hip", "capi.hip"]
 FLAGS = ["--offload-arch=gfx950", "-O3", "-std=c++17", "-fPIC", "-Wno-unused-value"]
 
 
diff --git a/ctrlora_amd/csrc/attention.h b/ctrlora_amd/csrc/attention.h
--- a/ctrlora_amd/csrc/attention.h
+++ b/ctrlora_amd/csrc/attention.h
@@ -39,7 +39,13 @@
 int attn_fwd_tr(const AttnFwdArgs& a, const void* V, long ldv, hipStream_t st);
 int attn_fwd_ip(const AttnFwdArgs& a, const AttnIpArgs& ip, int dtype, hipStream_t st);
 int attn_fwd_tr_ip(const AttnFwdArgs& a, const void* V, long ldv, const AttnIpArgs& ip, hipStream_t st);
-int attn_bwd_tr(const AttnBwdArgs& a, hipStream_t st);
+int attn_bwd_tr(const AttnBwdArgs& a, hipStream_t st, void* kv_ws = nullptr, long kv_ws_bytes = 0);
+extern int g_attn_shortkv;
+bool attn_sk_rule(int N, int Nkv, int dh, bool fwd);
+long attn_sk_kv_ws_bytes(int B, int H, int N, int Nkv, int dh);
+bool attn_sk_bwd_applies(const AttnBwdArgs& a, const void* kv_ws, long kv_ws_bytes);
+int attn_sk_fwd(const AttnFwdArgs& a, const void* V, long ldv, hipStream_t st);
+int attn_sk_bwd(const AttnBwdArgs& a, void* kv_ws, hipStream_t st);
 extern int g_attn_fuse_delta;
 extern int g_attn_variant_dkv4;
 extern int g_attn_variant;
@@ -50,7 +56,7 @@
                     int N, int dh, float scale, hipStream_t st);
 
 enum { ATTN_FAM_TR = 1, ATTN_FAM_TR_IP = 2, ATTN_FAM_HYB = 3, ATTN_FAM_FWD40 = 4, ATTN_FAM_FOLD = 5, ATTN_FAM_TRANSPOSED = 6,
-       ATTN_FAM_CAUSAL = 7 };
+       ATTN_FAM_CAUSAL = 7, ATTN_FAM_SHORT = 8 };
 enum { ATTN_BIT_TAIL = 1, ATTN_BIT_TQ = 2, ATTN_BIT_TK = 4, ATTN_BIT_PRIO = 8 };
 struct AttnLaunchRec {
   int kind;
diff --git a/ctrlora_amd/csrc/attention_sk.hip b/ctrlora_amd/csrc/attention_sk.hip
--- /dev/null
+++ b/ctrlora_amd/csrc/attention_sk.hip
@@ -0,0 +1,505 @@
+#include <cstdlib>
+#include "attn_common.h"
+#include "attn_tr_util.h"
+
+namespace cl {
+namespace {
+
+constexpr int SK_TARGET_WG = 1024;
+constexpr int SK_TARGET_WG_DKV = 512;
+
+template <int DH, int NS> struct SkGeo {
+  using G = Geo<DH>;
+  static constexpr int KR = 32 * NS;
+  static constexpr int KV = KR * G::ROWB;
+  static constexpr int QT = 64 * G::ROWB;
+  static constexpr int PROW = 64 * NS + 16;
+  static constexpr int PB = 64 * PROW;
+  static constexpr int LDS_FWD = 2 * KV + 64;
+  static constexpr int LDS_BWD = 2 * KV + 64;
+  static constexpr int LDS_BWD_DKV = 2 * KV + 2 * QT + 2 * PB + 64;
+};
+
+template <int DH, int KR>
+__device__ __forceinline__ void sk_stage(char* dst, const char* ksrc, long ldk_bytes, const char* vsrc, long ldv_bytes, int nrows, int tid) {
+  using G = Geo<DH>;
+  constexpr int TOT = KR * G::CPRP, NIT = (TOT + 255) / 256;
+  uint4 kk[NIT], vv[NIT];
+#pragma unroll
+  for (int it = 0; it < NIT; ++it) {
+    const int i = tid + it * 256, r = i / G::CPRP, c = i - r * G::CPRP;
+    const long rr = min(r, nrows - 1);
+    const bool in = i < TOT && c < G::CPR;
+    kk[it] = in ? *reinterpret_cast<const uint4*>(ksrc + rr * ldk_bytes + c * 16) : make_uint4(0u, 0u, 0u, 0u);
+    vv[it] = in ? *reinterpret_cast<const uint4*>(vsrc + rr * ldv_bytes + c * 16) : make_uint4(0u, 0u, 0u, 0u);
+  }
+#pragma unroll
+  for (int it = 0; it < NIT; ++it) {
+    const int i = tid + it * 256, r = i / G::CPRP, c = i - r * G::CPRP;
+    if (i < TOT) {
+      *reinterpret_cast<uint4*>(dst + r * G::ROWB + c * 16) = kk[it];
+      *reinterpret_cast<uint4*>(dst + KR * G::ROWB + r * G::ROWB + c * 16) = vv[it];
+    }
+  }
+}
+
+}
+
+template <int DH, int NS>
+__global__ __launch_bounds__(256, 4) void attn_sk_fwd_kernel(AttnFwdArgs p, const void* __restrict__ V, long ldv, int bps) {
+  using G = Geo<DH>;
+  using SG = SkGeo<DH, NS>;
+  constexpr int CPR = G::CPR, KSTEPS = G::KSTEPS, DN = G::DN, ROWB = G::ROWB, NF = 2 * NS, KV = SG::KV;
+  extern __shared__ __attribute__((aligned(16))) char smem[];
+
+  const int tid = threadIdx.x, lane = tid & 63;
+  const int wave = __builtin_amdgcn_readfirstlane(tid >> 6);
+  const int g = lane >> 4, lq = lane & 15;
+  const int bh = blockIdx.y, b = bh / p.H, h = bh - b * p.H;
+  const int nb = p.N >> 6;
+  const int blk0 = blockIdx.x * bps, blk1 = min(blk0 + bps, nb);
+  const float sl2 = p.q_prescaled ? 1.0f : p.scale * 1.4426950408889634f;
+
+  const long row0 = (long)b * p.N + blk0 * 64 + wave * 16 + lq;
+  const char* qrow = (const char*)p.Q + (row0 * p.ldq + (long)h * DH) * 2;
+  char* orow = (char*)p.O + (row0 * p.ldo + (long)h * DH) * 2 + 8 * g;
+  float* lrow = p.LSE ? p.LSE + (long)bh * p.lse_stride + blk0 * 64 + wave * 16 + lq : nullptr;
+  const int qstep = 64 * (int)p.ldq * 2, ostep = 64 * (int)p.ldo * 2;
+  asm volatile("" : "+v"(qrow), "+v"(orow), "+v"(lrow));
+  auto load_q = [&](const char* qp, u32x4_t (&q)[KSTEPS]) {
+#pragma unroll
+    for (int ks = 0; ks < KSTEPS; ++ks) {
+      const int c = 4 * ks + g;
+      q[ks] = (c < CPR) ? *reinterpret_cast<const u32x4_t*>(qp + c * 16) : u32x4_t{0u, 0u, 0u, 0u};
+    }
+  };
+  u32x4_t qf[KSTEPS];
+  load_q(qrow, qf);
+  sk_stage<DH, SG::KR>(smem, (const char*)p.K + ((long)b * p.Nkv * p.ldk + (long)h * DH) * 2, p.ldk * 2,
+                       (const char*)V + ((long)b * p.Nkv * ldv + (long)h * DH) * 2, ldv * 2, p.Nkv, tid);
+  __syncthreads();
+
+  const uint32_t lds0 = (uint32_t)(uintptr_t)smem;
+  uint32_t krow[KSTEPS];
+#pragma unroll
+  for (int ks = 0; ks < KSTEPS; ++ks) krow[ks] = lds0 + lq * ROWB + min(4 * ks + g, CPR - 1) * 16;
+  const uint32_t tb = lds0 + KV + (4 * g + ((lane >> 2) & 3)) * ROWB + (lane & 3) * 8;
+
+  for (int blk = blk0; blk < blk1; ++blk) {
+    u32x4_t qn[KSTEPS];
+    if (blk + 1 < blk1) load_q(qrow + qstep, qn);
+    else {
+#pragma unroll
+      for (int ks = 0; ks < KSTEPS; ++ks) qn[ks] = qf[ks];
+    }
+    f32x4_t st[NF];
+    static_for<0, NF>([&](auto KF_) {
+      constexpr int kf = decltype(KF_)::value;
+      st[kf] = f32x4_t{0.f, 0.f, 0.f, 0.f};
+      if (kf * 16 < p.Nkv) {
+        u32x4_t ka[KSTEPS];
+#pragma unroll
+        for (int ks = 0; ks < KSTEPS; ++ks) ka[ks] = lds_read_b128_off<kf * 16 * ROWB>(krow[ks]);
+        lds_wait();
+#pragma unroll
+        for (int ks = 0; ks < KSTEPS; ++ks) Mma<bf16_t>::run(ka[ks], qf[ks], st[kf]);
+      }
+    });
+    float mx = -INFINITY;
+#pragma unroll
+    for (int kf = 0; kf < NF; ++kf)
+      if (kf * 16 < p.Nkv) {
+        if (kf * 16 + 16 > p.Nkv) {
+#pragma unroll
+          for (int r = 0; r < 4; ++r)
+            if (kf * 16 + 4 * g + r >= p.Nkv) st[kf][r] = -INFINITY;
+        }
+        mx = fmaxf(fmaxf(mx, fmaxf(st[kf][0], st[kf][1])), fmaxf(st[kf][2], st[kf][3]));
+      }
+    mx = fmaxf(mx, __shfl_xor(mx, 16, 64));
+    mx = fmaxf(mx, __shfl_xor(mx, 32, 64));
+    const float m = mx * sl2;
+    f32x2_t l2 = {0.f, 0.f};
+#pragma unroll
+    for (int kf = 0; kf < NF; ++kf)
+      if (kf * 16 < p.Nkv) {
+#pragma unroll
+        for (int h2 = 0; h2 < 2; ++h2) {
+          const f32x2_t x = f32x2_t{st[kf][2 * h2], st[kf][2 * h2 + 1]} * sl2 - m;
+          const f32x2_t e = {__builtin_amdgcn_exp2f(x.x), __builtin_amdgcn_exp2f(x.y)};
+          st[kf][2 * h2] = e.x; st[kf][2 * h2 + 1] = e.y;
+          l2 += e;
+        }
+      } else {
+        st[kf] = f32x4_t{0.f, 0.f, 0.f, 0.f};
+      }
+    float l = l2.x + l2.y;
+    l += __shfl_xor(l, 16, 64);
+    l += __shfl_xor(l, 32, 64);
+    u32x4_t pb[NS];
+#pragma unroll
+    for (int s = 0; s < NS; ++s) pb[s] = PFrag<bf16_t>::make(&st[2 * s]);
+    f32x4_t ot[DN];
+    static_for<0, DN>([&](auto I_) {
+      constexpr int i = decltype(I_)::value;
+      u32x4_t va[NS];
+      static_for<0, NS>([&](auto S_) { constexpr int s = decltype(S_)::value; va[s] = tr_frag_off<ROWB, s, i * 32>(tb); });
+      lds_wait();
+      ot[i] = f32x4_t{0.f, 0.f, 0.f, 0.f};
+#pragma unroll
+      for (int s = 0; s < NS; ++s) Mma<bf16_t>::run(va[s], pb[s], ot[i]);
+    });
+    const float inv = 1.0f / l;
+#pragma unroll
+    for (int i = 0; i < DN; ++i) {
+      const int d0 = i * 16 + 4 * g;
+      if (d0 < DH) {
+        const f32x2_t lo = f32x2_t{ot[i][0], ot[i][1]} * inv, hi = f32x2_t{ot[i][2], ot[i][3]} * inv;
+        float v[4] = {lo.x, lo.y, hi.x, hi.y};
+        store4(reinterpret_cast<bf16_t*>(orow + i * 32), v);
+      }
+    }
+    if (lrow && g == 0) *lrow = m + __builtin_amdgcn_logf(l);
+    qrow += qstep; orow += ostep;
+    if (lrow) lrow += 64;
+#pragma unroll
+    for (int ks = 0; ks < KSTEPS; ++ks) qf[ks] = qn[ks];
+  }
+}
+
+template <int DH, int NS, bool DKV>
+__global__ __launch_bounds__(256, DKV ? 2 : (DH <= 40 ? 4 : 3)) void attn_sk_bwd_kernel(AttnBwdArgs p, float* __restrict__ slab, int bps) {
+  using G = Geo<DH>;
+  using SG = SkGeo<DH, NS>;
+  constexpr int CPR = G::CPR, KSTEPS = G::KSTEPS, DN = G::DN, ROWB = G::ROWB, NF = 2 * NS, KV = SG::KV, QT = SG::QT, PROW = SG::PROW,
+                PB = SG::PB;
+  extern __shared__ __attribute__((aligned(16))) char smem[];
+  char* const qimg = smem + 2 * KV;
+
+  const int tid = threadIdx.x, lane = tid & 63;
+  const int wave = __builtin_amdgcn_readfirstlane(tid >> 6);
+  const int g = lane >> 4, lq = lane & 15;
+  const int bh = blockIdx.y, b = bh / p.H, h = bh - b * p.H;
+  const int nb = p.N >> 6;
+  const int blk0 = blockIdx.x * bps, blk1 = min(blk0 + bps, nb);
+  const float sl2 = p.q_prescaled ? 1.0f : p.scale * 1.4426950408889634f;
+
+  if constexpr (DKV && G::CPRP > G::CPR) {
+    if (tid < 128) *reinterpret_cast<uint4*>(qimg + tid * ROWB + CPR * 16) = make_uint4(0u, 0u, 0u, 0u);
+  }
+
+  const long row0 = (long)b * p.N + blk0 * 64 + wave * 16 + lq;
+  const char* qrow = (const char*)p.Q + (row0 * p.ldq + (long)h * DH) * 2;
+  const char* dorow = (const char*)p.dO + (row0 * p.lddo + (long)h * DH) * 2;
+  const char* orow = (const char*)p.O + (row0 * p.ldo + (long)h * DH) * 2;
+  char* dqrow = (char*)p.dQ + (row0 * p.lddq + (long)h * DH) * 2 + 8 * g;
+  const float* lrow = p.LSE + (long)bh * p.lse_stride + blk0 * 64 + wave * 16 + lq;
+  float* drow = p.Delta + (long)bh * p.lse_stride + blk0 * 64 + wave * 16 + lq;
+  const int qstep = 64 * (int)p.ldq * 2, dostep = 64 * (int)p.lddo * 2, ostep = 64 * (int)p.ldo * 2, dqstep = 64 * (int)p.lddq * 2;
+  asm volatile("" : "+v"(qrow), "+v"(dorow), "+v"(orow), "+v"(dqrow), "+v"(lrow), "+v"(drow));
+  char* qr = qimg + (wave * 16 + lq) * ROWB;
+  char* pr = qimg + 2 * QT + (wave * 16 + lq) * PROW + 8 * g;
+  float* sl = DKV ? slab + (((long)bh * gridDim.x + blockIdx.x) * 2 + (wave & 1)) * (long)p.Nkv * DH : nullptr;
+  asm volatile("" : "+v"(qr), "+v"(pr), "+v"(sl));
+  auto load_rows = [&](int ahead, u32x4_t (&q)[KSTEPS], u32x4_t (&d)[KSTEPS], u32x4_t (&o)[KSTEPS], float& ls) {
+    const char* qp = qrow + ahead * qstep;
+    const char* dp = dorow + ahead * dostep;
+    const char* op = orow + ahead * ostep;
+#pragma unroll
+    for (int ks = 0; ks < KSTEPS; ++ks) {
+      const int c = 4 * ks + g;
+      const bool in = c < CPR;
+      q[ks] = in ? *reinterpret_cast<const u32x4_t*>(qp + c * 16) : u32x4_t{0u, 0u, 0u, 0u};
+      d[ks] = in ? *reinterpret_cast<const u32x4_t*>(dp + c * 16) : u32x4_t{0u, 0u, 0u, 0u};
+      o[ks] = in ? *reinterpret_cast<const u32x4_t*>(op + c * 16) : u32x4_t{0u, 0u, 0u, 0u};
+    }
+    ls = lrow[ahead * 64];
+  };
+  u32x4_t qb[KSTEPS], ob[KSTEPS], ov[KSTEPS];
+  float lse_q;
+  load_rows(0, qb, ob, ov, lse_q);
+  sk_stage<DH, SG::KR>(smem, (const char*)p.K + ((long)b * p.Nkv * p.ldk + (long)h * DH) * 2, p.ldk * 2,
+                       (const char*)p.V + ((long)b * p.Nkv * p.ldv + (long)h * DH) * 2, p.ldv * 2, p.Nkv, tid);
+
+  const int which = wave & 1, half = wave >> 1;
+  f32x4_t acc[DKV ? NS : 1][DKV ? DN : 1];
+#pragma unroll
+  for (int j = 0; j < (DKV ? NS : 1); ++j)
+#pragma unroll
+    for (int i = 0; i < (DKV ? DN : 1); ++i) acc[j][i] = f32x4_t{0.f, 0.f, 0.f, 0.f};
+
+  const uint32_t lds0 = (uint32_t)(uintptr_t)smem;
+  uint32_t krow[KSTEPS];
+#pragma unroll
+  for (int ks = 0; ks < KSTEPS; ++ks) krow[ks] = lds0 + lq * ROWB + min(4 * ks + g, CPR - 1) * 16;
+  const uint32_t trl = 4 * g + ((lane >> 2) & 3), trc = (lane & 3) * 8;
+  const uint32_t tbk = lds0 + trl * ROWB + trc;
+  const uint32_t tbx = lds0 + 2 * KV + (which ? 0 : QT) + trl * ROWB + trc;
+  const uint32_t tbw = lds0 + 2 * KV + 2 * QT + (which ? PB : 0) + trl * PROW + trc + half * NS * 32;
+  __syncthreads();
+
+  for (int blk = blk0; blk < blk1; ++blk) {
+    float dlt = 0.f;
+#pragma unroll
+    for (int ks = 0; ks < KSTEPS; ++ks)
+#pragma unroll
+      for (int j = 0; j < 4; ++j) {
+        dlt += __uint_as_float(ov[ks][j] << 16) * __uint_as_float(ob[ks][j] << 16);
+        dlt += __uint_as_float(ov[ks][j] & 0xffff0000u) * __uint_as_float(ob[ks][j] & 0xffff0000u);
+      }
+    dlt += __shfl_xor(dlt, 16, 64);
+    dlt += __shfl_xor(dlt, 32, 64);
+    if (g == 0) *drow = dlt;
+    u32x4_t qn[KSTEPS], on[KSTEPS], ovn[KSTEPS];
+    float lse_n = 0.f;
+    if (blk + 1 < blk1) load_rows(1, qn, on, ovn, lse_n);
+    else {
+#pragma unroll
+      for (int ks = 0; ks < KSTEPS; ++ks) { qn[ks] = qb[ks]; on[ks] = ob[ks]; ovn[ks] = ov[ks]; }
+    }
+    if constexpr (DKV) {
+#pragma unroll
+      for (int ks = 0; ks < KSTEPS; ++ks) {
+        const int c = 4 * ks + g;
+        if (c < CPR) {
+          *reinterpret_cast<u32x4_t*>(qr + c * 16) = qb[ks];
+          *reinterpret_cast<u32x4_t*>(qr + QT + c * 16) = ob[ks];
+        }
+      }
+    }
+    f32x4_t pt[DKV ? NF : 1], dst[NF];
+    static_for<0, NF>([&](auto KF_) {
+      constexpr int kf = decltype(KF_)::value;
+      if constexpr (DKV) pt[kf] = f32x4_t{0.f, 0.f, 0.f, 0.f};
+      dst[kf] = f32x4_t{0.f, 0.f, 0.f, 0.f};
+      if (kf * 16 < p.Nkv) {
+        u32x4_t ka[KSTEPS], va[KSTEPS];
+#pragma unroll
+        for (int ks = 0; ks < KSTEPS; ++ks) {
+          ka[ks] = lds_read_b128_off<kf * 16 * ROWB>(krow[ks]);
+          va[ks] = lds_read_b128_off<KV + kf * 16 * ROWB>(krow[ks]);
+        }
+        lds_wait();
+        f32x4_t sc = {0.f, 0.f, 0.f, 0.f}, dp = {0.f, 0.f, 0.f, 0.f};
+#pragma unroll
+        for (int ks = 0; ks < KSTEPS; ++ks) { Mma<bf16_t>::run(ka[ks], qb[ks], sc); Mma<bf16_t>::run(va[ks], ob[ks], dp); }
+#pragma unroll
+        for (int h2 = 0; h2 < 2; ++h2) {
+          const f32x2_t x = f32x2_t{sc[2 * h2], sc[2 * h2 + 1]} * sl2 - lse_q;
+          const f32x2_t pr = {__builtin_amdgcn_exp2f(x.x), __builtin_amdgcn_exp2f(x.y)};
+          const f32x2_t dsv = pr * (f32x2_t{dp[2 * h2], dp[2 * h2 + 1]} - dlt);
+          if constexpr (DKV) { pt[kf][2 * h2] = pr.x; pt[kf][2 * h2 + 1] = pr.y; }
+          dst[kf][2 * h2] = dsv.x; dst[kf][2 * h2 + 1] = dsv.y;
+        }
+        if (kf * 16 + 16 > p.Nkv) {
+#pragma unroll
+          for (int r = 0; r < 4; ++r)
+            if (kf * 16 + 4 * g + r >= p.Nkv) {
+              if constexpr (DKV) pt[kf][r] = 0.f;
+              dst[kf][r] = 0.f;
+            }
+        }
+      }
+    });
+    u32x4_t sb[NS], pbk[DKV ? NS : 1];
+#pragma unroll
+    for (int s = 0; s < NS; ++s) {
+      sb[s] = PFrag<bf16_t>::make(&dst[2 * s]);
+      if constexpr (DKV) pbk[s] = PFrag<bf16_t>::make(&pt[2 * s]);
+    }
+    static_for<0, DN>([&](auto I_) {
+      constexpr int i = decltype(I_)::value;
+      u32x4_t kc[NS];
+      static_for<0, NS>([&](auto S_) { constexpr int s = decltype(S_)::value; kc[s] = tr_frag_off<ROWB, s, i * 32>(tbk); });
+      lds_wait();
+      f32x4_t dq = {0.f, 0.f, 0.f, 0.f};
+#pragma unroll
+      for (int s = 0; s < NS; ++s) Mma<bf16_t>::run(kc[s], sb[s], dq);
+      const int d0 = i * 16 + 4 * g;
+      if (d0 < DH) {
+        const f32x2_t lo = f32x2_t{dq[0], dq[1]} * p.scale, hi = f32x2_t{dq[2], dq[3]} * p.scale;
+        float a[4] = {lo.x, lo.y, hi.x, hi.y};
+        store4(reinterpret_cast<bf16_t*>(dqrow + i * 32), a);
+      }
+    });
+    if constexpr (DKV) {
+#pragma unroll
+      for (int s = 0; s < NS; ++s) {
+        *reinterpret_cast<uint2*>(pr + s * 64) = make_uint2(pbk[s].x, pbk[s].y);
+        *reinterpret_cast<uint2*>(pr + s * 64 + 32) = make_uint2(pbk[s].z, pbk[s].w);
+        *reinterpret_cast<uint2*>(pr + PB + s * 64) = make_uint2(sb[s].x, sb[s].y);
+        *reinterpret_cast<uint2*>(pr + PB + s * 64 + 32) = make_uint2(sb[s].z, sb[s].w);
+      }
+      __syncthreads();
+      static_for<0, 2>([&](auto QS_) {
+        constexpr int qs = decltype(QS_)::value;
+        u32x4_t wb[NS];
+        static_for<0, NS>([&](auto J_) { constexpr int j = decltype(J_)::value; wb[j] = tr_frag_off<PROW, qs, j * 32>(tbw); });
+        if constexpr (2 * NS + 2 * DN > 12) lds_wait();
+        u32x4_t xa[DN];
+        static_for<0, DN>([&](auto I_) { constexpr int i = decltype(I_)::value; xa[i] = tr_frag_off<ROWB, qs, i * 32>(tbx); });
+        lds_wait();
+#pragma unroll
+        for (int i = 0; i < DN; ++i)
+#pragma unroll
+          for (int j = 0; j < NS; ++j) Mma<bf16_t>::run(xa[i], wb[j], acc[j][i]);
+      });
+      __syncthreads();
+    }
+#pragma unroll
+    for (int ks = 0; ks < KSTEPS; ++ks) { qb[ks] = qn[ks]; ob[ks] = on[ks]; ov[ks] = ovn[ks]; }
+    lse_q = lse_n;
+    qrow += qstep; dorow += dostep; orow += ostep; dqrow += dqstep; lrow += 64; drow += 64;
+  }
+
+  if constexpr (DKV) {
+#pragma unroll
+    for (int j = 0; j < NS; ++j) {
+      const int key = (half * NS + j) * 16 + lq;
+      if (key < p.Nkv) {
+#pragma unroll
+        for (int i = 0; i < DN; ++i) {
+          const int d0 = i * 16 + 4 * g;
+          if (d0 < DH) *reinterpret_cast<float4*>(sl + (long)key * DH + d0) = make_float4(acc[j][i][0], acc[j][i][1], acc[j][i][2], acc[j][i][3]);
+        }
+      }
+    }
+  }
+}
+
+__global__ __launch_bounds__(256) void attn_sk_finish_kernel(const float* __restrict__ slab, bf16_t* __restrict__ dK, long lddk,
+                                                             bf16_t* __restrict__ dV, long lddv, int H, int Nkv, int dh, int nsplit,
+                                                             float kscale, long total) {
+  const long idx = (long)blockIdx.x * 256 + threadIdx.x;
+  if (idx >= total) return;
+  const int d4 = dh / 4;
+  const int c = (int)(idx % d4);
+  long t = idx / d4;
+  const int key = (int)(t % Nkv); t /= Nkv;
+  const int which = (int)(t & 1);
+  const long bh = t >> 1;
+  const long per = (long)Nkv * dh;
+  const float* src = slab + (bh * nsplit * 2 + which) * per + (long)key * dh + c * 4;
+  float4 s = *reinterpret_cast<const float4*>(src);
+  for (int i = 1; i < nsplit; ++i) {
+    const float4 v = *reinterpret_cast<const float4*>(src + (long)i * 2 * per);
+    s.x += v.x; s.y += v.y; s.z += v.z; s.w += v.w;
+  }
+  const long b = bh / H, h = bh - b * H;
+  const float f = which ? kscale : 1.0f;
+  float o[4] = {s.x * f, s.y * f, s.z * f, s.w * f};
+  bf16_t* dst = which ? dK + (b * Nkv + key) * lddk + h * dh + c * 4 : dV + (b * Nkv + key) * lddv + h * dh + c * 4;
+  store4(dst, o);
+}
+
+namespace {
+
+template <typename K> int sk_set_lds(K kern, int bytes) {
+  if (bytes > 65536 &&
+      hipFuncSetAttribute(reinterpret_cast<const void*>(kern), hipFuncAttributeMaxDynamicSharedMemorySize, bytes) != hipSuccess)
+    return CL_ELAUNCH;
+  return CL_OK;
+}
+
+bool sk_shape(int N, int Nkv, int dh) {
+  return Nkv >= 1 && Nkv <= 96 && N >= 256 && N % 64 == 0 && (dh == 40 || dh == 80);
+}
+
+void sk_split(int BH, int nb, int target, int* bps, int* nsplit) {
+  int s = (target + BH - 1) / BH;
+  s = s < 1 ? 1 : (s > nb ? nb : s);
+  *bps = (nb + s - 1) / s;
+  *nsplit = (nb + *bps - 1) / *bps;
+}
+
+bool sk_on() {
+  if (g_attn_shortkv < 0) {
+    const char* e = std::getenv("CTRLORA_ATTN_SHORTKV");
+    g_attn_shortkv = (e && e[0] == '0' && e[1] == 0) ? 0 : 1;
+  }
+  return g_attn_shortkv != 0;
+}
+
+template <int DH, int NS>
+int sk_launch_fwd(const AttnFwdArgs& a, const void* V, long ldv, hipStream_t st) {
+  int bps, ns;
+  sk_split(a.B * a.H, a.N / 64, SK_TARGET_WG, &bps, &ns);
+  using SG = SkGeo<DH, NS>;
+  hipLaunchKernelGGL((attn_sk_fwd_kernel<DH, NS>), dim3(ns, a.B * a.H), dim3(256), SG::LDS_FWD, st, a, V, ldv, bps);
+  attn_rec(1, ATTN_FAM_SHORT, CL_BF16, DH);
+  g_attn_last.fwd_frags = 1; g_attn_last.grid_fwd = ns * a.B * a.H; g_attn_last.dkv_frags = ns; g_attn_last.tile = 32 * NS;
+  CL_CHECK_LAUNCH();
+  return CL_OK;
+}
+
+template <int DH, int NS>
+int sk_launch_bwd(const AttnBwdArgs& a, void* kv_ws, hipStream_t st) {
+  using SG = SkGeo<DH, NS>;
+  const int BH = a.B * a.H;
+  int bps, ns;
+  attn_rec(2, ATTN_FAM_SHORT, CL_BF16, DH);
+  g_attn_last.dq_frags = 1; g_attn_last.tile = 32 * NS;
+  if (a.dK) {
+    static bool done = false;
+    if (!done) { if (sk_set_lds(&attn_sk_bwd_kernel<DH, NS, true>, SG::LDS_BWD_DKV)) return CL_ELAUNCH; done = true; }
+    sk_split(BH, a.N / 64, SK_TARGET_WG_DKV, &bps, &ns);
+    hipLaunchKernelGGL((attn_sk_bwd_kernel<DH, NS, true>), dim3(ns, BH), dim3(256), SG::LDS_BWD_DKV, st, a, (float*)kv_ws, bps);
+    const long total = (long)BH * 2 * a.Nkv * (DH / 4);
+    const float kscale = a.q_prescaled ? 0.6931471805599453f : a.scale;
+    hipLaunchKernelGGL(attn_sk_finish_kernel, dim3((unsigned)((total + 255) / 256)), dim3(256), 0, st, (const float*)kv_ws,
+                       (bf16_t*)a.dK, a.lddk, (bf16_t*)a.dV, a.lddv, a.H, a.Nkv, DH, ns, kscale, total);
+    g_attn_last.dkv_ran = 1; g_attn_last.grid_dq = (int)((total + 255) / 256);
+  } else {
+    sk_split(BH, a.N / 64, SK_TARGET_WG, &bps, &ns);
+    hipLaunchKernelGGL((attn_sk_bwd_kernel<DH, NS, false>), dim3(ns, BH), dim3(256), SG::LDS_BWD, st, a, (float*)nullptr, bps);
+  }
+  g_attn_last.dkv_frags = ns; g_attn_last.grid_dkv = ns * BH;
+  CL_CHECK_LAUNCH();
+  return CL_OK;
+}
+
+}
+
+int g_attn_shortkv = -1;
+
+long attn_sk_kv_ws_bytes(int B, int H, int N, int Nkv, int dh) {
+  if (B < 1 || H < 1 || !sk_shape(N, Nkv, dh)) return 0;
+  int bps, ns;
+  sk_split(B * H, N / 64, SK_TARGET_WG_DKV, &bps, &ns);
+  return (long)B * H * ns * 2 * Nkv * dh * 4;
+}
+
+bool attn_sk_rule(int N, int Nkv, int dh, bool fwd) { return sk_on() && sk_shape(N, Nkv, dh) && (!fwd || dh == 40); }
+
+bool attn_sk_bwd_applies(const AttnBwdArgs& a, const void* kv_ws, long kv_ws_bytes) {
+  if (!attn_sk_rule(a.N, a.Nkv, a.DH, false)) return false;
+  if (!a.dK) return true;
+  return kv_ws && !(reinterpret_cast<uintptr_t>(kv_ws) & 15) && kv_ws_bytes >= attn_sk_kv_ws_bytes(a.B, a.H, a.N, a.Nkv, a.DH);
+}
+
+#define SK_DISPATCH(FN, ...)                                             \
+  do {                                                                   \
+    const int ns_ = (a.Nkv + 31) / 32;                                   \
+    switch (a.DH * 4 + ns_) {                                            \
+      case 40 * 4 + 1: return FN<40, 1>(__VA_ARGS__);                    \
+      case 40 * 4 + 2: return FN<40, 2>(__VA_ARGS__);                    \
+      case 40 * 4 + 3: return FN<40, 3>(__VA_ARGS__);                    \
+      case 80 * 4 + 1: return FN<80, 1>(__VA_ARGS__);                    \
+      case 80 * 4 + 2: return FN<80, 2>(__VA_ARGS__);                    \
+      case 80 * 4 + 3: return FN<80, 3>(__VA_ARGS__);                    \
+      default: return CL_EINVAL;                                         \
+    }                                                                    \
+  } while (0)
+
+int attn_sk_fwd(const AttnFwdArgs& a, const void* V, long ldv, hipStream_t st) {
+  if (a.DH != 40) return CL_EINVAL;
+  switch ((a.Nkv + 31) / 32) {
+    case 1: return sk_launch_fwd<40, 1>(a, V, ldv, st);
+    case 2: return sk_launch_fwd<40, 2>(a, V, ldv, st);
+    case 3: return sk_launch_fwd<40, 3>(a, V, ldv, st);
+    default: return CL_EINVAL;
+  }
+}
+int attn_sk_bwd(const AttnBwdArgs& a, void* kv_ws, hipStream_t st) { SK_DISPATCH(sk_launch_bwd, a, kv_ws, st); }
+
+}
diff --git a/ctrlora_amd/csrc/attention_tr.hip b/ctrlora_amd/csrc/attention_tr.hip
--- a/ctrlora_amd/csrc/attention_tr.hip
+++ b/ctrlora_amd/csrc/attention_tr.hip
@@ -1225,6 +1225,7 @@
   attn_rec_begin();
   if ((a.ldq * 2) % 16 || (a.ldk * 2) % 16 || (ldv * 2) % 16 || (a.ldo * 2) % 16 || a.Nkv < 1 || a.N < 1) return CL_EINVAL;
   if (a.LSE && (a.lse_stride % 64 || a.lse_stride < a.N)) return CL_EINVAL;
+  if (attn_sk_rule(a.N, a.Nkv, a.DH, true)) return attn_sk_fwd(a, V, ldv, st);
   if (g_attn_variant == 0 && attn_fwd40_applies(a)) return attn_fwd40(a, V, ldv, st);
   switch (a.DH) {
     case 8: return launch_fwd_tr_t<8>(a, V, ldv, st);
@@ -1376,13 +1377,14 @@
   return tk ? launch_bwd_tr<DH, false, true>(a, st) : launch_bwd_tr<DH, false, false>(a, st);
 }
 
-int attn_bwd_tr(const AttnBwdArgs& a, hipStream_t st) {
+int attn_bwd_tr(const AttnBwdArgs& a, hipStream_t st, void* kv_ws, long kv_ws_bytes) {
   attn_rec_begin();
   if ((a.ldq * 2) % 16 || (a.ldk * 2) % 16 || (a.ldv * 2) % 16 || (a.lddo * 2) % 16 || (a.ldo * 2) % 16) return CL_EINVAL;
   if ((a.lddq * 2) % 16 || a.lse_stride % 64 || a.lse_stride < a.N) return CL_EINVAL;
   if ((a.dK == nullptr) != (a.dV == nullptr)) return CL_EINVAL;
   if (a.row_ws && (reinterpret_cast<uintptr_t>(a.row_ws) & 15)) return CL_EINVAL;
   if (a.dK && ((a.lddk * 2) % 16 || (a.lddv * 2) % 16)) return CL_EINVAL;
+  if (attn_sk_bwd_applies(a, kv_ws, kv_ws_bytes)) return attn_sk_bwd(a, kv_ws, st);
   switch (a.DH) {
     case 8: return launch_bwd_tr_t<8>(a, st);
     case 16: return launch_bwd_tr_t<16>(a, st);
diff --git a/ctrlora_amd/csrc/capi.hip b/ctrlora_amd/csrc/capi.hip
--- a/ctrlora_amd/csrc/capi.hip
+++ b/ctrlora_amd/csrc/capi.hip
@@ -48,6 +48,11 @@
   }
 }
 int cl_debug_attention_fuse_delta(int on) { g_attn_fuse_delta = on ? 1 : 0; return CL_OK; }
+int cl_debug_attention_shortkv(int on) { g_attn_shortkv = on ? 1 : 0; return CL_OK; }
+int cl_debug_attention_shortkv_rule(int dtype, int B, int H, int N, int Nkv, int dh, int want_dkv, long kv_ws_bytes) {
+  if (dtype != CL_BF16 || !attn_sk_rule(N, Nkv, dh, want_dkv < 0)) return 0;
+  return (want_dkv <= 0 || (kv_ws_bytes > 0 && kv_ws_bytes >= attn_sk_kv_ws_bytes(B, H, N, Nkv, dh))) ? 1 : 0;
+}
 int cl_debug_attention_last_launch(int* out16) {
   static_assert(sizeof(AttnLaunchRec) == 16 * sizeof(int), "cl_debug_attention_last_launch: sixteen ints");
   if (!out16) return CL_EINVAL;
@@ -311,6 +316,20 @@
                         const void* O, long ldo, const void* dO, long lddo, const float* LSE, float* Delta,
                         int lse_stride, void* dQ, long lddq, void* dK, long lddk, void* dV, long lddv, int B, int H,
                         int N, int Nkv, int dh, float scale, int flags, void* row_ws, void* stream) {
+  void* ws = nullptr;
+  long ws_bytes = 0;
+  gemm_get_workspace_for(S(stream), &ws, &ws_bytes);
+  return cl_attention_bwd_v3(dtype, Q, ldq, K, ldk, V, ldv, O, ldo, dO, lddo, LSE, Delta, lse_stride, dQ, lddq, dK, lddk, dV, lddv, B, H,
+                             N, Nkv, dh, scale, flags, row_ws, ws, ws_bytes, stream);
+}
+
+long cl_attention_bwd_kv_ws_bytes(int B, int H, int N, int Nkv, int dh) { return attn_sk_kv_ws_bytes(B, H, N, Nkv, dh); }
+
+int cl_attention_bwd_v3(int dtype, const void* Q, long ldq, const void* K, long ldk, const void* V, long ldv,
+                        const void* O, long ldo, const void* dO, long lddo, const float* LSE, float* Delta,
+                        int lse_stride, void* dQ, long lddq, void* dK, long lddk, void* dV, long lddv, int B, int H,
+                        int N, int Nkv, int dh, float scale, int flags, void* row_ws, void* kv_ws, long kv_ws_bytes,
+                        void* stream) {
   attn_rec_begin();
   if (dtype != CL_BF16 || (flags & ~CL_ATTN_Q_PRESCALED)) return CL_EINVAL;
   AttnBwdArgs a{}; a.Q = Q; a.ldq = ldq; a.K = K; a.ldk = ldk; a.V = V; a.ldv = ldv; a.O = O; a.ldo = ldo;
@@ -318,7 +337,7 @@
   a.dK = dK; a.lddk = lddk; a.dV = dV; a.lddv = lddv; a.B = B; a.H = H; a.N = N; a.Nkv = Nkv; a.DH = dh; a.scale = scale;
   a.q_prescaled = (flags & CL_ATTN_Q_PRESCALED) ? 1 : 0;
   a.row_ws = row_ws;
-  return attn_bwd_tr(a, S(stream));
+  return attn_bwd_tr(a, S(stream), kv_ws, kv_ws_bytes);
 }
 
 int cl_geglu_fwd(int dtype, const void* h, long ldh, void* out, long ldo, long M, int F, void* stream) { return geglu_fwd(dtype, h, ldh, out, ldo, M, F, S(stream)); }
diff --git a/ctrlora_amd/csrc/debug_hooks.h b/ctrlora_amd/csrc/debug_hooks.h
--- a/ctrlora_amd/csrc/debug_hooks.h
+++ b/ctrlora_amd/csrc/debug_hooks.h
@@ -4,6 +4,8 @@
 #endif
 int cl_debug_attention_variant(int variant);
 int cl_debug_attention_fuse_delta(int on);
+int cl_debug_attention_shortkv(int on);
+int cl_debug_attention_shortkv_rule(int dtype, int B, int H, int N, int Nkv, int dh, int want_dkv, long kv_ws_bytes);
 int cl_debug_attention_last_launch(int* out16);
 int cl_debug_groupnorm_form(int three_pass, int one_pass);
 int cl_debug_groupnorm_group(int mode);
diff --git a/ctrlora_amd/hip.py b/ctrlora_amd/hip.py
--- a/ctrlora_amd/hip.py
+++ b/ctrlora_amd/hip.py
@@ -79,6 +79,9 @@
     "cl_attention_fwd_ip": [_I, _P, _L, _P, _L, _P, _L, _P, _L, _P, _L, _P, _L, _I, _I, _I, _I, _I, _I, _F, _F, _I, _P],
     "cl_attention_bwd_v2": [_I, _P, _L, _P, _L, _P, _L, _P, _L, _P, _L, _P, _P, _I, _P, _L, _P, _L, _P, _L,
                             _I, _I, _I, _I, _I, _F, _I, _P, _P],
+    "cl_attention_bwd_v3": [_I, _P, _L, _P, _L, _P, _L, _P, _L, _P, _L, _P, _P, _I, _P, _L, _P, _L, _P, _L,
+                            _I, _I, _I, _I, _I, _F, _I, _P, _P, _L, _P],
+    "cl_attention_bwd_kv_ws_bytes": [_I, _I, _I, _I, _I],
     "cl_attention_causal_fwd": [_I, _P, _L, _P, _L, _P, _L, _P, _L, _I, _I, _I, _I, _F, _P],
     "cl_geglu_fwd": [_I, _P, _L, _P, _L, _L, _I, _P],
     "cl_geglu_bwd": [_I, _P, _L, _P, _L, _P, _L, _L, _I, _P],
@@ -121,12 +124,14 @@
     "cl_grad_norm": [_P, _P, _I, _P, _P, _P, _P, _P],
     "cl_adamw_dev_clip": [_P, _P, _P, _P, _L, _P, _P, _P, _P],
 }
-_LONG_RESULT = ("cl_groupnorm_ws_floats", "cl_grad_norm_scratch_floats")
+_LONG_RESULT = ("cl_groupnorm_ws_floats", "cl_grad_norm_scratch_floats", "cl_attention_bwd_kv_ws_bytes")
 EXPORTED = tuple(_SIGS.keys())
 _DEBUG_SIGS = {
     "cl_debug_attention_variant": [_I],
     "cl_debug_attention_fuse_delta": [_I],
     "cl_debug_attention_last_launch": [_P],
+    "cl_debug_attention_shortkv": [_I],
+    "cl_debug_attention_shortkv_rule": [_I, _I, _I, _I, _I, _I, _I, _L],
     "cl_debug_groupnorm_form": [_I, _I],
     "cl_debug_groupnorm_group": [_I],
     "cl_debug_norm_last_launch": [_P],
@@ -461,12 +466,33 @@
     return o
 
 
-def attention_bwd_v2(q, k, v, o, do, lse, delta, dq, dk, dv, B, H, N, Nkv, dh, scale, q_prescaled=False, row_ws=None):
+def attention_kv_ws_bytes(B, H, N, Nkv, dh):
+    if B < 1 or H < 1 or not (1 <= Nkv <= 96 and N >= 256 and N % 64 == 0 and dh in (40, 80)):
+        return 0
+    nb = N // 64
+    s = max(1, min(nb, -(-512 // (B * H))))
+    bps = -(-nb // s)
+    return B * H * -(-nb // bps) * 2 * Nkv * dh * 4
+
+
+KV_WS_REGISTERED = "registered"
+
+
+def attention_bwd_v2(q, k, v, o, do, lse, delta, dq, dk, dv, B, H, N, Nkv, dh, scale, q_prescaled=False, row_ws=None, kv_ws=None):
     assert row_ws is None or row_ws.numel() * row_ws.element_size() >= B * H * lse.shape[-1] * 32
-    _chk(lib().cl_attention_bwd_v2(dt(q), q.data_ptr(), ld(q), k.data_ptr(), ld(k), v.data_ptr(), ld(v), o.data_ptr(),
+    if isinstance(kv_ws, str):
+        assert kv_ws == KV_WS_REGISTERED
+        _chk(lib().cl_attention_bwd_v2(dt(q), q.data_ptr(), ld(q), k.data_ptr(), ld(k), v.data_ptr(), ld(v), o.data_ptr(),
+                                       ld(o), do.data_ptr(), ld(do), lse.data_ptr(), delta.data_ptr(), lse.shape[-1],
+                                       dq.data_ptr(), ld(dq), ptr(dk), ld(dk), ptr(dv), ld(dv), B, H, N, Nkv, dh, scale,
+                                       ATTN_Q_PRESCALED if q_prescaled else 0, ptr(row_ws), stream()), "cl_attention_bwd_v2")
+        return
+    kv_bytes = 0 if kv_ws is None else kv_ws.numel() * kv_ws.element_size()
+    _chk(lib().cl_attention_bwd_v3(dt(q), q.data_ptr(), ld(q), k.data_ptr(), ld(k), v.data_ptr(), ld(v), o.data_ptr(),
                                    ld(o), do.data_ptr(), ld(do), lse.data_ptr(), delta.data_ptr(), lse.shape[-1],
                                    dq.data_ptr(), ld(dq), ptr(dk), ld(dk), ptr(dv), ld(dv), B, H, N, Nkv, dh, scale,
-                                   ATTN_Q_PRESCALED if q_prescaled else 0, ptr(row_ws), stream()), "cl_attention_bwd_v2")
+                                   ATTN_Q_PRESCALED if q_prescaled else 0, ptr(row_ws), ptr(kv_ws), kv_bytes, stream()),
+         "cl_attention_bwd_v3")
 
 
 
@@ -504,7 +530,7 @@
     if dt(q) == BF16:
         row_ws = torch.empty(lse.numel() * 8, dtype=torch.float32, device=q.device) if (q_prescaled and dh == 40) else None
         return attention_bwd_v2(q, k, v, o, do, lse, delta, dq, dk, dv, B, H, N, Nkv, dh, scale, q_prescaled=q_prescaled,
-                                row_ws=row_ws)
+                                row_ws=row_ws, kv_ws=KV_WS_REGISTERED)
     assert not q_prescaled, "the fp32 kernels scale the scores themselves"
     inner, npad, kpad = H * dh, (N + 63) // 64 * 64, (Nkv + 63) // 64 * 64
     qt = _transposed(q, B, N, inner, npad)
diff --git a/include/ctrlora_hip.h b/include/ctrlora_hip.h
--- a/include/ctrlora_hip.h
+++ b/include/ctrlora_hip.h
@@ -128,6 +128,12 @@
                         const void* O, long ldo, const void* dO, long lddo, const float* LSE, float* Delta,
                         int lse_stride, void* dQ, long lddq, void* dK, long lddk, void* dV, long lddv,
                         int B, int H, int N, int Nkv, int dh, float scale, int flags, void* row_ws, void* stream);
+int cl_attention_bwd_v3(int dtype, const void* Q, long ldq, const void* K, long ldk, const void* V, long ldv,
+                        const void* O, long ldo, const void* dO, long lddo, const float* LSE, float* Delta,
+                        int lse_stride, void* dQ, long lddq, void* dK, long lddk, void* dV, long lddv,
+                        int B, int H, int N, int Nkv, int dh, float scale, int flags, void* row_ws, void* kv_ws,
+                        long kv_ws_bytes, void* stream);
+long cl_attention_bwd_kv_ws_bytes(int B, int H, int N, int Nkv, int dh);
 int cl_attention_fwd_ip(int dtype, const void* Q, long ldq, const void* K, long ldk, const void* V, long ldv,
                         const void* Kip, long ldkip, const void* Vip, long ldvip, void* O, long ldo, int B, int H,
                         int N, int Nkv, int Nip, int dh, float scale, float ip_scale, int flags, void* stream);
```

Result: no change. 242.8 images/s, median of 6 (+0.6%).
